# RobinBruneau/RNb-NeuS2

Measured on AMD Instinct MI355X. Metric: training rays/s + ms/step, normals-only SDF 64x800^2, higher is better.
Workload: dtype f16 storage / f32 accumulate

## Files before the change

rnb-neus2_amd/csrc/common.cuh:

```cuda
#pragma once
#include <hip/hip_runtime.h>
#include <stdint.h>
#include "../../include/rnb_neus2.h"

namespace rnb {

typedef _Float16 half_t;
typedef _Float16 h2 __attribute__((ext_vector_type(2)));
typedef _Float16 h4 __attribute__((ext_vector_type(4)));
typedef _Float16 h8 __attribute__((ext_vector_type(8)));
typedef float f4 __attribute__((ext_vector_type(4)));

constexpr uint32_t GRIDSIZE = RNB_GRIDSIZE;
constexpr uint32_t GRID_CELLS = GRIDSIZE * GRIDSIZE * GRIDSIZE;
constexpr uint32_t N_CASCADES = RNB_CASCADES;
constexpr float LOSS_SCALE = 128.f;
constexpr uint32_t N_MAX_RANDOM_SAMPLES_PER_RAY = 8;
constexpr float SQRT3 = 1.73205080757f;
constexpr float STEPSIZE = SQRT3 / 1024;
constexpr float MIN_CONE_STEPSIZE = STEPSIZE;
constexpr float MAX_CONE_STEPSIZE = STEPSIZE * (1 << (N_CASCADES - 1)) * 1024 / GRIDSIZE;
constexpr float MIN_OPTICAL_THICKNESS = 0.1f;

struct GridMeta {
// ... 220 lines not shown
}

template <bool PAIR = false>
__device__ __forceinline__ void level_issue(const LevelMeta* __restrict__ lm, const uint32_t* __restrict__ grid, const uint32_t level, const float x, const float y, const float z, uint32_t (&v)[8]) {
	const uint4 raw = reinterpret_cast<const uint4*>(lm + level)[0], raw2 = reinterpret_cast<const uint4*>(lm + level)[1];
	const uint32_t off = __builtin_amdgcn_readfirstlane(raw.x), hashmap_size = __builtin_amdgcn_readfirstlane(raw.y);
	const float scale = __uint_as_float(__builtin_amdgcn_readfirstlane(raw.w));
	const uint32_t my = __builtin_amdgcn_readfirstlane(raw2.x), mz = __builtin_amdgcn_readfirstlane(raw2.y);
	const bool dense = __builtin_amdgcn_readfirstlane(raw2.z) != 0u, pow2 = __builtin_amdgcn_readfirstlane(raw2.w) != 0u;
	const uint32_t* __restrict__ g = grid + off;
	float pos[3];
	uint32_t pg[3];
	pos_fract(x, scale, &pos[0], &pg[0]);
	pos_fract(y, scale, &pos[1], &pg[1]);
	pos_fract(z, scale, &pos[2], &pg[2]);
	const uint32_t ty0 = pg[1] * my, ty1 = ty0 + my, tz0 = pg[2] * mz, tz1 = tz0 + mz;
#pragma unroll
	for (uint32_t yz = 0; yz < 4; ++yz) {
		const uint32_t ty = (yz & 1u) ? ty1 : ty0, tz = (yz >> 1) ? tz1 : tz0;
		const uint32_t d0 = pg[0] + ty + tz, h = ty ^ tz;
		uint32_t e0 = (PAIR || dense) ? d0 : (pg[0] ^ h), e1 = (PAIR || dense) ? d0 + 1u : ((pg[0] + 1u) ^ h);
		const uint32_t w0 = e0 >= hashmap_size ? e0 - hashmap_size : e0, w1 = e1 >= hashmap_size ? e1 - hashmap_size : e1;
		e0 = pow2 ? (e0 & (hashmap_size - 1u)) : w0;
		e1 = pow2 ? (e1 & (hashmap_size - 1u)) : w1;
		if (PAIR) {
			const U2 p = *reinterpret_cast<const U2*>(g + e0);
			v[yz * 2 + 0] = p.x;
			v[yz * 2 + 1] = e1 == e0 + 1u ? p.y : g[0];
		} else {
			v[yz * 2 + 0] = g[e0];
			v[yz * 2 + 1] = g[e1];
		}
	}
}
template <bool GRAD>
__device__ __forceinline__ void level_consume(const LevelMeta* __restrict__ lm, const uint32_t level, const float x, const float y, const float z, const uint32_t (&v)[8],
                                              half_t& f0, half_t& f1, float dy0[3], float dy1[3]) {
	const float scale = __uint_as_float(__builtin_amdgcn_readfirstlane(reinterpret_cast<const uint32_t*>(lm + level)[3]));
	float pos[3];
	uint32_t pg[3];
	pos_fract(x, scale, &pos[0], &pg[0]);
	pos_fract(y, scale, &pos[1], &pg[1]);
	pos_fract(z, scale, &pos[2], &pg[2]);
	half_t r0 = (half_t)0.f, r1 = (half_t)0.f;
#pragma unroll
	for (uint32_t idx = 0; idx < 8; ++idx) {
		float weight = 1;
#pragma unroll
		for (uint32_t d = 0; d < 3; ++d) {
			if ((idx & (1u << d)) == 0) weight *= 1 - pos[d];
			else weight *= pos[d];
		}
		const h2 val = unpack_h2(v[idx]);
		r0 = r0 + f2h(weight * h2f(val[0]));
		r1 = r1 + f2h(weight * h2f(val[1]));
	}
	f0 = r0;
	f1 = r1;
	if (GRAD) {
#pragma unroll
		for (uint32_t gd = 0; gd < 3; ++gd) {
			float a0 = 0.f, a1 = 0.f;
#pragma unroll
			for (uint32_t idx = 0; idx < 4; ++idx) {
				float weight = scale;
				uint32_t corner = 0;
#pragma unroll
				for (uint32_t ngd = 0; ngd < 2; ++ngd) {
					const uint32_t d = ngd >= gd ? (ngd + 1) : ngd;
					if ((idx & (1u << ngd)) == 0) weight *= 1 - pos[d];
					else { weight *= pos[d]; corner |= (1u << d); }
				}
				const h2 vl = unpack_h2(v[corner]);
				const h2 vr = unpack_h2(v[corner | (1u << gd)]);
				a0 += weight * (h2f(vr[0]) - h2f(vl[0])) * 1.0f;
				a1 += weight * (h2f(vr[1]) - h2f(vl[1])) * 1.0f;
			}
			dy0[gd] = a0;
			dy1[gd] = a1;
		}
	}
}

struct Vec3 { float x, y, z; };
__device__ __forceinline__ Vec3 v3(float x, float y, float z) { return {x, y, z}; }
__device__ __forceinline__ Vec3 operator+(Vec3 a, Vec3 b) { return {a.x + b.x, a.y + b.y, a.z + b.z}; }
__device__ __forceinline__ Vec3 operator-(Vec3 a, Vec3 b) { return {a.x - b.x, a.y - b.y, a.z - b.z}; }
__device__ __forceinline__ Vec3 operator*(float s, Vec3 a) { return {s * a.x, s * a.y, s * a.z}; }
__device__ __forceinline__ float esum3(float x0, float x1, float x2) { return x0 + (x1 + x2); }
__device__ __forceinline__ float esum4(float x0, float x1, float x2, float x3) { return (x0 + x1) + (x2 + x3); }
__device__ __forceinline__ float dot(Vec3 a, Vec3 b) { return esum3(a.x * b.x, a.y * b.y, a.z * b.z); }
__device__ __forceinline__ Vec3 normalized(Vec3 a) { float n = sqrtf(dot(a, a)); return {a.x / n, a.y / n, a.z / n}; }

__device__ __forceinline__ int mip_from_pos(const Vec3& pos, uint32_t max_cascade = N_CASCADES - 1) {
	int exponent;
	float maxval = fmaxf(fmaxf(fabsf(pos.x - 0.5f), fabsf(pos.y - 0.5f)), fabsf(pos.z - 0.5f));
	frexpf(maxval, &exponent);
	return min((int)max_cascade, max(0, exponent + 1));
}
__device__ __forceinline__ int mip_from_dt(float dt, const Vec3& pos, uint32_t max_cascade = N_CASCADES - 1) {
	int mip = mip_from_pos(pos, max_cascade);
	dt *= 2 * GRIDSIZE;
	if (dt < 1.f) return mip;
	int exponent;
	frexpf(dt, &exponent);
	return min((int)max_cascade, max(exponent, mip));
}
__device__ __forceinline__ uint32_t cascaded_grid_idx_at(Vec3 pos, uint32_t mip) {
	float mip_scale = scalbnf(1.0f, -(int)mip);
	pos = pos - v3(0.5f, 0.5f, 0.5f);
	pos = mip_scale * pos;
	pos = pos + v3(0.5f, 0.5f, 0.5f);
	int ix = (int)(pos.x * GRIDSIZE), iy = (int)(pos.y * GRIDSIZE), iz = (int)(pos.z * GRIDSIZE);
	return morton3D((uint32_t)min(max(ix, 0), (int)GRIDSIZE - 1), (uint32_t)min(max(iy, 0), (int)GRIDSIZE - 1), (uint32_t)min(max(iz, 0), (int)GRIDSIZE - 1));
}
__device__ __forceinline__ bool density_grid_occupied_at(const Vec3& pos, const uint8_t* __restrict__ bitfield, uint32_t mip) {
	uint32_t idx = cascaded_grid_idx_at(pos, mip);
	return bitfield[idx / 8 + (GRID_CELLS * mip) / 8] & (1 << (idx % 8));
}
__device__ __forceinline__ float calc_dt(float t, float cone_angle) {
	return fminf(fmaxf(t * cone_angle, MIN_CONE_STEPSIZE), MAX_CONE_STEPSIZE);
}
__device__ __forceinline__ float warp_dt(float dt) {
	float max_stepsize = MIN_CONE_STEPSIZE * (1 << (N_CASCADES - 1));
	return (dt - MIN_CONE_STEPSIZE) / (max_stepsize - MIN_CONE_STEPSIZE);
}
__device__ __forceinline__ float unwarp_dt(float dt) {
	float max_stepsize = MIN_CONE_STEPSIZE * (1 << (N_CASCADES - 1));
	return dt * (max_stepsize - MIN_CONE_STEPSIZE) + MIN_CONE_STEPSIZE;
}
__device__ __forceinline__ float sign1(float x) { return copysignf(1.0f, x); }
__device__ __forceinline__ float distance_to_next_voxel(const Vec3& pos, const Vec3& dir, const Vec3& idir, uint32_t res) {
	Vec3 p = (float)res * pos;
	float tx = (floorf(p.x + 0.5f + 0.5f * sign1(dir.x)) - p.x) * idir.x;
	float ty = (floorf(p.y + 0.5f + 0.5f * sign1(dir.y)) - p.y) * idir.y;
	float tz = (floorf(p.z + 0.5f + 0.5f * sign1(dir.z)) - p.z) * idir.z;
	float t = fminf(fminf(tx, ty), tz);
	return fmaxf(t / res, 0.0f);
}
__device__ __forceinline__ float advance_to_next_voxel(float t, float cone_angle, const Vec3& pos, const Vec3& dir, const Vec3& idir, uint32_t res) {
	float t_target = t + distance_to_next_voxel(pos, dir, idir, res);
	do { t += calc_dt(t, cone_angle); } while (t < t_target);
	return t;
}

__device__ __forceinline__ float logistic(float x) { return 1.0f / (1.0f + expf(-x)); }
__device__ __forceinline__ float relu(float v) { return v > 0.0f ? v : 0.0f; }
__device__ __forceinline__ Vec3 warp_direction(const Vec3& d) { return {(d.x + 1.0f) * 0.5f, (d.y + 1.0f) * 0.5f, (d.z + 1.0f) * 0.5f}; }
__device__ __forceinline__ Vec3 unwarp_direction(const Vec3& d) { return {d.x * 2.0f - 1.0f, d.y * 2.0f - 1.0f, d.z * 2.0f - 1.0f}; }
__device__ __forceinline__ float loss_and_gradient(const bool l2, const float (&target)[4], const float (&prediction)[4], float (&grad)[4]) {
	float diff[4];
#pragma unroll
	for (int k = 0; k < 4; ++k) diff[k] = prediction[k] - target[k];
	if (l2) {
#pragma unroll
		for (int k = 0; k < 4; ++k) grad[k] = 2 * diff[k];
		return diff[0] * diff[0] + diff[1] * diff[1] + diff[2] * diff[2] + diff[3] * diff[3];
	}
#pragma unroll
	for (int k = 0; k < 4; ++k) grad[k] = copysignf(1.0f, diff[k]);
	return fabsf(diff[0]) + fabsf(diff[1]) + fabsf(diff[2]) + fabsf(diff[3]);
}

}
```

rnb-neus2_amd/csrc/kernels_net.cuh:

```cuda
#pragma once
#include "mlp.cuh"

namespace rnb {

constexpr int WG = 256;
constexpr int WAVES_PER_WG = 4;


__device__ __forceinline__ void write_sdf_in_row(half_t* __restrict__ tile, const int lane, const float x, const float y, const float z, const half_t (&feat)[28]) {
	half_t row[32];
	row[0] = f2h(x) - (half_t)0.5f;
	row[1] = f2h(y) - (half_t)0.5f;
	row[2] = f2h(z) - (half_t)0.5f;
#pragma unroll
	for (int k = 0; k < 28; ++k) row[3 + k] = feat[k];
	row[31] = (half_t)0.f;
#pragma unroll
	for (int q = 0; q < 4; ++q) {
		h8 v;
#pragma unroll
		for (int j = 0; j < 8; ++j) v[j] = row[q * 8 + j];
		*reinterpret_cast<h8*>(tile + lane * S32 + q * 8) = v;
	}
}

template <bool GRAD>
__device__ __forceinline__ void encode_all_lm(const LevelMeta* __restrict__ lm, const uint32_t n_levels, const uint32_t valid_level, const uint32_t* __restrict__ grid,
                                              const float x, const float y, const float z, half_t (&feat)[28], float (&dydx)[GRAD ? 28 : 1][3]) {
#pragma unroll
	for (uint32_t level = 0; level < 14; ++level) {
		half_t f0 = (half_t)0.f, f1 = (half_t)0.f;
		float d0[3] = {0.f, 0.f, 0.f}, d1[3] = {0.f, 0.f, 0.f};
		if (level < n_levels && level <= valid_level) {
			encode_level_lm<GRAD>(lm, grid, level, x, y, z, f0, f1, d0, d1);
		}
		feat[level * 2 + 0] = f0;
		feat[level * 2 + 1] = f1;
		if (GRAD) {
#pragma unroll
			for (int d = 0; d < 3; ++d) { dydx[GRAD ? level * 2 + 0 : 0][d] = d0[d]; dydx[GRAD ? level * 2 + 1 : 0][d] = d1[d]; }
		}
	}
}

template <bool GRAD, int DEPTH, int ND = 0>
__device__ __forceinline__ void encode_all_pipelined(const LevelMeta* __restrict__ lm, const uint32_t n_levels, const uint32_t valid_level, const uint32_t* __restrict__ grid,
                                                     const float x, const float y, const float z, half_t (&feat)[28], float (&dydx)[GRAD ? 28 : 1][3]) {
	const uint32_t n_live = min(n_levels, valid_level + 1u);
	uint32_t v[DEPTH][8];
	const uint32_t last = n_live ? n_live - 1u : 0u;
#pragma unroll
	for (uint32_t l = 0; l < (uint32_t)DEPTH; ++l) { if (l < (uint32_t)ND) level_issue<true>(lm, grid, min(l, last), x, y, z, v[l]); else level_issue<false>(lm, grid, min(l, last), x, y, z, v[l]); }
#pragma unroll
	for (uint32_t level = 0; level < 14; ++level) {
		half_t f0, f1;
		float d0[3], d1[3];
		const bool live = level < n_live;
		level_consume<GRAD>(lm, min(level, last), x, y, z, v[level % DEPTH], f0, f1, d0, d1);
		if (level + DEPTH < 14) { if (level + DEPTH < (uint32_t)ND) level_issue<true>(lm, grid, min(level + (uint32_t)DEPTH, last), x, y, z, v[level % DEPTH]); else level_issue<false>(lm, grid, min(level + (uint32_t)DEPTH, last), x, y, z, v[level % DEPTH]); }
		feat[level * 2 + 0] = live ? f0 : (half_t)0.f;
		feat[level * 2 + 1] = live ? f1 : (half_t)0.f;
		if (GRAD) {
#pragma unroll
			for (int d = 0; d < 3; ++d) { dydx[GRAD ? level * 2 + 0 : 0][d] = live ? d0[d] : 0.f; dydx[GRAD ? level * 2 + 1 : 0][d] = live ? d1[d] : 0.f; }
		}
	}
}

__device__ __forceinline__ half_t sdf_to_density(half_t sdf, half_t variance) {
	const half_t s = f2h(expf(h2f(variance * (half_t)10.0f)));
	const half_t sig = f2h(1.0f / (1.0f + expf(-h2f(sdf * s))));
	return (s * sig) * ((half_t)1.0f - sig);
}

struct PointArgs {
	const float* xyz;
	uint32_t n;
	half_t* out;
	const uint32_t* splat_idx;
	float* grid_tmp;
	int want_density;
	float sdf_bias;
	const uint32_t* range;
	uint32_t xcd;
};

struct FwdArgs {
	const float* coords;
	const uint32_t* n_ptr;
	uint32_t n_max;
	half_t* out;
	float sdf_bias;
	const uint32_t* idx;
	const half_t* wimg;
	half_t* cin_out;
};

__device__ __forceinline__ void copy_weight_image(half_t* __restrict__ dst, const half_t* __restrict__ src, const int n_halfs, const int tid, const int nthreads) {
	for (int i = tid * 8; i < n_halfs; i += nthreads * 8) *reinterpret_cast<h8*>(dst + i) = *reinterpret_cast<const h8*>(src + i);
}

constexpr int PQ2_WAVE_HALFS = TILE * S32 + TILE;
constexpr size_t LDS_POINT2 = (size_t)(W_S0T + WAVES_PER_WG * PQ2_WAVE_HALFS) * sizeof(half_t);
__device__ __forceinline__ void poison_lds(char* smem_raw, const size_t bytes, const int tid, const int nthreads) {
#ifdef RNB_POISON_LDS
	uint32_t* w = reinterpret_cast<uint32_t*>(smem_raw);
	for (uint32_t q = (uint32_t)tid; q < (uint32_t)(bytes / 4); q += (uint32_t)nthreads) w[q] = 0x7e007e00u;
	__syncthreads();
#else
	(void)smem_raw; (void)bytes; (void)tid; (void)nthreads;
#endif
}

template <bool EMU, int PIPE_DEPTH = 0, int ND = 0>
__device__ __forceinline__ void point_query_chained_body(const GridMeta& G, const NetW& net, const PointArgs& a, const half_t* __restrict__ wimg, char* smem_raw, LevelMeta* lm) {
	poison_lds(smem_raw, LDS_POINT2, threadIdx.x, WG);
	half_t* wts = reinterpret_cast<half_t*>(smem_raw);
	fill_level_meta(lm, G, threadIdx.x);
	const uint32_t n_levels = G.n_levels, valid_level = G.valid_level;
	if (wimg) copy_weight_image(wts, wimg, W_S0T, threadIdx.x, WG);
	else {
		for (int i = threadIdx.x; i < 64 * 32; i += WG) { int o = i >> 5, k = i & 31; wts[W_S0 + o * S32 + k] = net.sdf_w0[i]; }
		for (int i = threadIdx.x; i < 16 * 64; i += WG) { int o = i >> 6, q = i & 63; wts[W_S1 + o * S64 + q] = net.sdf_w1[o * 64 + chain_logical(q)]; }
	}
	__syncthreads();
	const int lane = threadIdx.x & 63, wave = threadIdx.x >> 6;
	half_t* X = wts + W_S0T + wave * PQ2_WAVE_HALFS;
	half_t* Z = X + TILE * S32;
	const half_t variance = net.variance[0];
	const half_t bias = f2h(a.sdf_bias);
	uint32_t s_first = 0, s_end = a.n;
	if (a.range) { s_first = a.range[0]; s_end = min(a.range[1], a.n); }
	const uint32_t n_tiles = (s_end - s_first + TILE - 1) / TILE;
	const int r16 = lane & 15, hq = lane >> 4;
	const bool by_xcd = a.xcd != 0u && (gridDim.x & 7u) == 0u;
	const uint32_t t8 = by_xcd ? (n_tiles + 7u) / 8u : n_tiles, t_base = by_xcd ? (blockIdx.x & 7u) * t8 : 0u, t_stop = min(n_tiles, t_base + t8);
	const uint32_t t_stride = (by_xcd ? gridDim.x / 8u : gridDim.x) * WAVES_PER_WG;
	for (uint32_t tile = t_base + (by_xcd ? blockIdx.x / 8u : blockIdx.x) * WAVES_PER_WG + wave; tile < t_stop; tile += t_stride) {
		const uint32_t s = s_first + tile * TILE + lane;
		const bool valid = s < s_end;
		float x = 0.5f, y = 0.5f, z = 0.5f;
		if (valid) { x = a.xyz[(size_t)s * 3 + 0]; y = a.xyz[(size_t)s * 3 + 1]; z = a.xyz[(size_t)s * 3 + 2]; }
		uint32_t cell = 0;
		if (valid && a.splat_idx) cell = a.splat_idx[s];
		half_t feat[28];
		float dummy[1][3];
		if (PIPE_DEPTH) encode_all_pipelined<false, PIPE_DEPTH ? PIPE_DEPTH : 1, ND>(lm, n_levels, valid_level, net.grid, x, y, z, feat, dummy);
		else encode_all_lm<false>(lm, n_levels, valid_level, net.grid, x, y, z, feat, dummy);
		write_sdf_in_row(X, lane, x, y, z, feat);
		wave_lds_sync();
		h8 bz[4][2];
		{
			f4 acc[4][4];
			zero_acc<4>(acc);
			mfma_layer<4, 1, EMU ? EMU_NATURAL : EMU_OFF>(wts + W_S0, S32, X, S32, acc, lane);
			chain_pack<true>(acc, bz);
		}
		f4 acc_so[1][4];
		zero_acc<1>(acc_so);
		mfma_layer_regs<1, 2, EMU ? EMU_CHAINED : EMU_OFF>(wts + W_S1, S64, bz, acc_so, lane);
		if (hq == 0) {
#pragma unroll
			for (int nt = 0; nt < 4; ++nt) Z[16 * nt + r16] = f2h(acc_so[0][nt][0]);
		}
		wave_lds_sync();
		half_t v = Z[lane] + bias;
		if (a.want_density) v = sdf_to_density(v, variance);
		if (valid) {
			if (a.out) a.out[s] = v;
			if (a.splat_idx) atomicMax(reinterpret_cast<uint32_t*>(a.grid_tmp) + cell, __float_as_uint(h2f(v)));
		}
		wave_lds_sync();
	}
}
__global__ __launch_bounds__(WG, 4) void k_point_query_chained(const GridMeta G, const NetW net, const PointArgs a, const half_t* __restrict__ wimg) {
	extern __shared__ __attribute__((aligned(16))) char smem_raw[];
	__shared__ LevelMeta lm[RNB_MAX_LEVELS];
	point_query_chained_body<false>(G, net, a, wimg, smem_raw, lm);
}
template <int DEPTH, int ND = 0>
__global__ __launch_bounds__(WG, 3) void k_point_query_chained_pipe(const GridMeta G, const NetW net, const PointArgs a, const half_t* __restrict__ wimg) {
	extern __shared__ __attribute__((aligned(16))) char smem_raw[];
	__shared__ LevelMeta lm[RNB_MAX_LEVELS];
	point_query_chained_body<false, DEPTH, ND>(G, net, a, wimg, smem_raw, lm);
}
__global__ __launch_bounds__(WG, 2) void k_point_query_chained_emul(const GridMeta G, const NetW net, const PointArgs a, const half_t* __restrict__ wimg) {
	extern __shared__ __attribute__((aligned(16))) char smem_raw[];
	__shared__ LevelMeta lm[RNB_MAX_LEVELS];
	point_query_chained_body<true>(G, net, a, wimg, smem_raw, lm);
}
template <int DEPTH, int ND = 0>
__global__ __launch_bounds__(WG, 2) void k_point_query_chained_emul_pipe(const GridMeta G, const NetW net, const PointArgs a, const half_t* __restrict__ wimg) {
	extern __shared__ __attribute__((aligned(16))) char smem_raw[];
	__shared__ LevelMeta lm[RNB_MAX_LEVELS];
	point_query_chained_body<true, DEPTH, ND>(G, net, a, wimg, smem_raw, lm);
}

constexpr int FWD2_WAVE_HALFS = TILE * S32 + TILE * 8 + TILE;
constexpr size_t LDS_FWD2 = (size_t)(W_FWD_END + WAVES_PER_WG * FWD2_WAVE_HALFS) * sizeof(half_t);

template <bool EMU, int PIPE_DEPTH = 0, int ND = 0>
__device__ __forceinline__ void forward_chained_body(const GridMeta& G, const NetW& net, const FwdArgs& a, char* smem_raw, LevelMeta* lm) {
	poison_lds(smem_raw, LDS_FWD2, threadIdx.x, WG);
	half_t* wts = reinterpret_cast<half_t*>(smem_raw);
	fill_level_meta(lm, G, threadIdx.x);
	const uint32_t n_levels = G.n_levels, valid_level = G.valid_level;
	if (a.wimg) copy_weight_image(wts, a.wimg, W_FWD_END, threadIdx.x, WG);
	else load_weights_chained(wts, net, threadIdx.x, WG);
	__syncthreads();
	const int lane = threadIdx.x & 63, wave = threadIdx.x >> 6;
	half_t* X = wts + W_FWD_END + wave * FWD2_WAVE_HALFS;
	half_t* Y = X + TILE * S32;
	half_t* Z = Y + TILE * 8;
	const half_t variance = net.variance[0];
	const half_t bias = f2h(a.sdf_bias);
	uint32_t n = a.n_max;
	if (a.n_ptr) n = min(*a.n_ptr, a.n_max);
	const uint32_t n_tiles = (n + TILE - 1) / TILE;
	const int r16 = lane & 15, hq = lane >> 4;
	for (uint32_t tile = blockIdx.x * WAVES_PER_WG + wave; tile < n_tiles; tile += gridDim.x * WAVES_PER_WG) {
		const uint32_t q_in = tile * TILE + lane;
		const bool valid = q_in < n;
		uint32_t s = q_in;
		if (a.idx && valid) s = a.idx[q_in];
		float c[7] = {0.5f, 0.5f, 0.5f, 0.f, 0.f, 0.f, 0.f};
		if (valid) {
#pragma unroll
			for (int q = 0; q < 7; ++q) c[q] = a.coords[(size_t)s * 7 + q];
		}
		half_t feat[28];
		float dydx[28][3];
		if (PIPE_DEPTH) encode_all_pipelined<true, PIPE_DEPTH ? PIPE_DEPTH : 1, ND>(lm, n_levels, valid_level, net.grid, c[0], c[1], c[2], feat, dydx);
		else encode_all_lm<true>(lm, n_levels, valid_level, net.grid, c[0], c[1], c[2], feat, dydx);
		write_sdf_in_row(X, lane, c[0], c[1], c[2], feat);
		wave_lds_sync();
		h8 bz[4][2];
		{
			f4 acc[4][4];
			zero_acc<4>(acc);
			mfma_layer<4, 1, EMU ? EMU_NATURAL : EMU_OFF>(wts + W_S0, S32, X, S32, acc, lane);
			chain_pack<true>(acc, bz);
		}
		f4 acc_so[1][4];
		zero_acc<1>(acc_so);
		mfma_layer_regs<1, 2, EMU ? EMU_CHAINED : EMU_OFF>(wts + W_S1, S64, bz, acc_so, lane);
		{
#pragma unroll
			for (int ks = 0; ks < 2; ++ks) {
				const h8 w1 = *reinterpret_cast<const h8*>(wts + W_S1 + 0 * S64 + 32 * ks + 8 * hq);
#pragma unroll
				for (int nt = 0; nt < 4; ++nt)
#pragma unroll
					for (int j = 0; j < 8; ++j) bz[nt][ks][j] = (bz[nt][ks][j] > (half_t)0.f) ? w1[j] : (half_t)0.f;
			}
		}
		wave_lds_sync();
		{
			f4 acc[2][4];
			zero_acc<2>(acc);
			mfma_layer_regs<2, 2, EMU ? EMU_CHAINED : EMU_OFF>(wts + W_S0T, S64, bz, acc, lane);
			store_acc<2, false>(acc, X, S32, 0, lane);
		}
		wave_lds_sync();
		float grad[3] = {0.f, 0.f, 0.f};
		{
			half_t din[32];
#pragma unroll
			for (int q = 0; q < 4; ++q) {
				const h8 v = *reinterpret_cast<const h8*>(X + lane * S32 + q * 8);
#pragma unroll
				for (int j = 0; j < 8; ++j) din[q * 8 + j] = v[j];
			}
#pragma unroll
			for (int k = 0; k < 28; ++k) {
				const float dl = h2f(din[3 + k]);
#pragma unroll
				for (int d = 0; d < 3; ++d) grad[d] += dl * dydx[k][d];
			}
#pragma unroll
			for (int d = 0; d < 3; ++d) grad[d] += h2f(din[d]);
		}
		{
			const h8 v = {f2h(c[0]), f2h(c[1]), f2h(c[2]), f2h(grad[0]), f2h(grad[1]), f2h(grad[2]), (half_t)0.f, (half_t)0.f};
			*reinterpret_cast<h8*>(Y + lane * 8) = v;
			if (hq == 0) {
#pragma unroll
				for (int nt = 0; nt < 4; ++nt) Z[16 * nt + r16] = f2h(acc_so[0][nt][0]);
			}
		}
		wave_lds_sync();
		const half_t sdf0 = Z[lane];
		if (a.cin_out) {
			if (valid) {
				h8* row = reinterpret_cast<h8*>(a.cin_out + (size_t)s * 32);
				row[2] = *reinterpret_cast<const h8*>(Y + lane * 8);
				row[3] = h8{(half_t)0.f, (half_t)0.f, (half_t)0.f, (half_t)0.f, (half_t)0.f, (half_t)0.f, (half_t)0.f, (half_t)0.f};
			}
#pragma unroll
			for (int nt = 0; nt < 4; ++nt) {
				const uint32_t s_nt = (uint32_t)__shfl((int)s, 16 * nt + r16, 64);
				const bool v_nt = __shfl((int)valid, 16 * nt + r16, 64) != 0;
				const h4 o = {f2h(acc_so[0][nt][0]), f2h(acc_so[0][nt][1]), f2h(acc_so[0][nt][2]), f2h(acc_so[0][nt][3])};
				if (v_nt) *reinterpret_cast<h4*>(a.cin_out + (size_t)s_nt * 32 + 4 * hq) = o;
			}
		}
		h8 bh[4][2];
		{
			h8 bin[4][1];
#pragma unroll
			for (int nt = 0; nt < 4; ++nt) {
				h4 o = {(half_t)0.f, (half_t)0.f, (half_t)0.f, (half_t)0.f};
				if (hq < 2) o = *reinterpret_cast<const h4*>(Y + (16 * nt + r16) * 8 + 4 * hq);
#pragma unroll
				for (int j = 0; j < 4; ++j) { bin[nt][0][j] = f2h(acc_so[0][nt][j]); bin[nt][0][4 + j] = o[j]; }
			}
			f4 acc[4][4];
			zero_acc<4>(acc);
			mfma_layer_regs<4, 1, EMU ? EMU_CHAINED : EMU_OFF>(wts + W_C0, S32, bin, acc, lane);
			chain_pack<true>(acc, bh);
		}
		{
			f4 acc[4][4];
			zero_acc<4>(acc);
			mfma_layer_regs<4, 2, EMU ? EMU_CHAINED : EMU_OFF>(wts + W_C1, S64, bh, acc, lane);
			chain_pack<true>(acc, bh);
		}
		{
			f4 acc[1][4];
			zero_acc<1>(acc);
			mfma_layer_regs<1, 2, EMU ? EMU_CHAINED : EMU_OFF>(wts + W_C2, S64, bh, acc, lane);
			store_acc<1, false>(acc, X, S32, 0, lane);
		}
		wave_lds_sync();
		{
			h8 o0 = *reinterpret_cast<const h8*>(X + lane * S32 + 0);
			h8 o1 = *reinterpret_cast<const h8*>(X + lane * S32 + 8);
			o0[3] = sdf0 + bias;
			o0[4] = f2h(grad[0]); o0[5] = f2h(grad[1]); o0[6] = f2h(grad[2]);
			o0[7] = variance;
			o1[0] = f2h(c[4]); o1[1] = f2h(c[5]); o1[2] = f2h(c[6]);
			if (valid) {
				h8* dst = reinterpret_cast<h8*>(a.out + (size_t)s * 16);
				dst[0] = o0;
				dst[1] = o1;
			}
		}
		wave_lds_sync();
	}
}
__global__ __launch_bounds__(WG, 2) void k_forward_chained(const GridMeta G, const NetW net, const FwdArgs a) {
	extern __shared__ __attribute__((aligned(16))) char smem_raw[];
	__shared__ LevelMeta lm[RNB_MAX_LEVELS];
	forward_chained_body<false>(G, net, a, smem_raw, lm);
}
template <int DEPTH, int ND = 0>
__global__ __launch_bounds__(WG, 2) void k_forward_chained_pipe(const GridMeta G, const NetW net, const FwdArgs a) {
	extern __shared__ __attribute__((aligned(16))) char smem_raw[];
	__shared__ LevelMeta lm[RNB_MAX_LEVELS];
	forward_chained_body<false, DEPTH, ND>(G, net, a, smem_raw, lm);
}
__global__ __launch_bounds__(WG, 2) void k_forward_chained_emul(const GridMeta G, const NetW net, const FwdArgs a) {
	extern __shared__ __attribute__((aligned(16))) char smem_raw[];
	__shared__ LevelMeta lm[RNB_MAX_LEVELS];
	forward_chained_body<true>(G, net, a, smem_raw, lm);
}
template <int DEPTH, int ND = 0>
__global__ __launch_bounds__(WG, 2) void k_forward_chained_emul_pipe(const GridMeta G, const NetW net, const FwdArgs a) {
	extern __shared__ __attribute__((aligned(16))) char smem_raw[];
	__shared__ LevelMeta lm[RNB_MAX_LEVELS];
	forward_chained_body<true, DEPTH, ND>(G, net, a, smem_raw, lm);
}


struct TrainScratch {
	half_t *h2, *h1, *cin, *z1, *sdfin, *dz1;
	half_t *dr, *dh2, *dh1, *dso, *dz, *ddin, *front;
	uint32_t* g12;
	float* srec;
	float* var_partial;
};

struct TrainArgs {
	const float* coords;
	const half_t* dout;
	uint32_t B;
	uint32_t B_global;
	float sdf_bias;
	uint32_t skip_rgb;
	const half_t* wimg;
	float *dw_w0, *dw_w0b, *dw_w1, *dw_w1b;
	const half_t* dcin;
	TrainScratch t;
};

__device__ __forceinline__ void fm_store(const half_t* __restrict__ tile, const int stride, const int width, half_t* __restrict__ dst, const uint32_t B, const uint32_t s) {
	const half_t* row = tile + (s & 63) * stride;
	for (int f = 0; f < width; f += 8) {
		const h8 v = *reinterpret_cast<const h8*>(row + f);
#pragma unroll
		for (int j = 0; j < 8; ++j) dst[(size_t)(f + j) * B + s] = v[j];
	}
}

__global__ __launch_bounds__(WG, 1) void k_fwd_bwd(const GridMeta G, const NetW net, const TrainArgs a) {
	extern __shared__ __attribute__((aligned(16))) char smem_raw[];
	half_t* wts = reinterpret_cast<half_t*>(smem_raw);
	__shared__ LevelMeta lm[RNB_MAX_LEVELS];
	fill_level_meta(lm, G, threadIdx.x);
	const uint32_t n_levels = G.n_levels, valid_level = G.valid_level;
	if (a.wimg) copy_weight_image(wts, a.wimg, W_TRAIN_END, threadIdx.x, WG);
	else load_weights<true>(wts, net, threadIdx.x, WG);
	__syncthreads();
	const int lane = threadIdx.x & 63, wave = threadIdx.x >> 6;
	half_t* tA = wts + W_TRAIN_END + wave * 3 * ACT_TILE_HALFS;
	half_t* tB = tA + ACT_TILE_HALFS;
	half_t* tC = tB + ACT_TILE_HALFS;
	const int r16 = lane & 15, hq = lane >> 4;
	const uint32_t B = a.B;
	const uint32_t n_tiles = B / TILE;
	const TrainScratch& T = a.t;
	float var_sum = 0.f;
	for (uint32_t tile = blockIdx.x * WAVES_PER_WG + wave; tile < n_tiles; tile += gridDim.x * WAVES_PER_WG) {
		const uint32_t s = tile * TILE + lane;
		float c[7];
#pragma unroll
		for (int q = 0; q < 7; ++q) c[q] = a.coords[(size_t)s * 7 + q];
		half_t dout[16];
		{
			const h8* src = reinterpret_cast<const h8*>(a.dout + (size_t)s * 16);
			const h8 d0 = src[0], d1 = src[1];
#pragma unroll
			for (int j = 0; j < 8; ++j) { dout[j] = d0[j]; dout[8 + j] = d1[j]; }
		}
		half_t feat[28];
		float dydx[28][3];
		encode_all_lm<true>(lm, n_levels, valid_level, net.grid, c[0], c[1], c[2], feat, dydx);
		write_sdf_in_row(tA, lane, c[0], c[1], c[2], feat);
		wave_lds_sync();
		fm_store(tA, S32, 32, T.sdfin, B, s);
		uint64_t m_z1;
		{
			f4 acc[4][4];
			zero_acc<4>(acc);
			mfma_layer<4, 1>(wts + W_S0, S32, tA, S32, acc, lane);
			m_z1 = store_acc<4, true>(acc, tB, S64, 0, lane);
		}
		wave_lds_sync();
		fm_store(tB, S64, 64, T.z1, B, s);
		{
			f4 acc[1][4];
			zero_acc<1>(acc);
			mfma_layer<1, 2>(wts + W_S1, S64, tB, S64, acc, lane);
			store_acc<1, false>(acc, tC, S32, 0, lane);
		}
		wave_lds_sync();
#pragma unroll
		for (int mt = 0; mt < 4; ++mt) {
			const h4 w1 = *reinterpret_cast<const h4*>(wts + W_S1 + 0 * S64 + 16 * mt + 4 * hq);
#pragma unroll
			for (int nt = 0; nt < 4; ++nt) {
				h4 v;
#pragma unroll
				for (int r = 0; r < 4; ++r) v[r] = ((m_z1 >> ((mt * 4 + nt) * 4 + r)) & 1ull) ? w1[r] : (half_t)0.f;
				*reinterpret_cast<h4*>(tA + (16 * nt + r16) * S64 + 16 * mt + 4 * hq) = v;
			}
		}
		wave_lds_sync();
		fm_store(tA, S64, 64, T.dz1, B, s);
		{
			f4 acc[2][4];
			zero_acc<2>(acc);
			mfma_layer<2, 2>(wts + W_S0T, S64, tA, S64, acc, lane);
			store_acc<2, false>(acc, tB, S32, 0, lane);
		}
// ... 153 lines not shown
			}
			dd[31] = (half_t)0.f;
#pragma unroll
			for (int q = 0; q < 4; ++q) {
				h8 v;
#pragma unroll
				for (int j = 0; j < 8; ++j) v[j] = dd[q * 8 + j];
				*reinterpret_cast<h8*>(tC + lane * S32 + q * 8) = v;
			}
		}
		wave_lds_sync();
		fm_store(tC, S32, 32, T.ddin, B, s);
		{
			f4 acc[4][4];
			zero_acc<4>(acc);
			mfma_layer<4, 1>(wts + W_S0, S32, tC, S32, acc, lane);
			wave_lds_sync();
			store_acc_masked<4>(acc, m_z1, tB, S64, 0, lane);
		}
		wave_lds_sync();
		fm_store(tB, S64, 64, T.front, B, s);
		wave_lds_sync();
		(void)m_h2;
	}
#pragma unroll
	for (int off = 32; off > 0; off >>= 1) var_sum += __shfl_down(var_sum, off, 64);
	if (lane == 0) T.var_partial[blockIdx.x * WAVES_PER_WG + wave] = var_sum;
}

constexpr int SW_S0 = 0;
constexpr int SW_S0T = SW_S0 + 64 * S32;
constexpr int SW_W1 = SW_S0T + 32 * S64;
constexpr int SW_W1N = SW_W1 + 64;
constexpr int SW_END = SW_W1N + 64;
constexpr int SW_END_PADDED = (SW_END + 7) / 8 * 8;
constexpr int FBS_WAVE_HALFS = 2 * TILE * S32 + TILE;
constexpr size_t LDS_FBS = (size_t)(SW_END + WAVES_PER_WG * FBS_WAVE_HALFS) * sizeof(half_t);
constexpr int SW_W1T = SW_END_PADDED;
constexpr int SWF_END = SW_W1T + 64 * S32;
constexpr int SO_STRIDE = 24;
constexpr int FBS_FULL_WAVE_HALFS = FBS_WAVE_HALFS + TILE * SO_STRIDE;
constexpr size_t LDS_FBS_FULL = (size_t)(SWF_END + WAVES_PER_WG * FBS_FULL_WAVE_HALFS) * sizeof(half_t);
__host__ __device__ constexpr int fbs_logical(int p) { return p < 28 ? 3 + p : (p < 31 ? p - 28 : 31); }
__host__ __device__ constexpr int fbs_logical_h(int p) { return p < 13 ? 3 + p : (p < 16 ? p - 13 : p); }
__host__ __device__ constexpr int fbs_feature_slot_h(int q) { return q < 13 ? q : q + 3; }

__device__ inline void load_weights_fbs(half_t* __restrict__ w, const NetW& net, const int tid, const int nthreads, const bool half_order = false) {
	for (int i = tid; i < 64 * 32; i += nthreads) { const int o = i >> 5, p = i & 31; w[SW_S0 + o * S32 + p] = net.sdf_w0[o * 32 + (half_order ? fbs_logical_h(p) : fbs_logical(p))]; }
	for (int i = tid; i < 32 * 64; i += nthreads) { const int q = i >> 6, p = i & 63; w[SW_S0T + q * S64 + p] = net.sdf_w0[chain_logical(p) * 32 + fbs_logical(q)]; }
	for (int i = tid; i < 64; i += nthreads) { w[SW_W1 + i] = net.sdf_w1[chain_logical(i)]; w[SW_W1N + i] = net.sdf_w1[i]; }
	for (int i = SW_END + tid; i < SW_END_PADDED; i += nthreads) w[i] = (half_t)0.f;
}
__device__ inline void load_weights_fbs_full(half_t* __restrict__ w, const NetW& net, const int tid, const int nthreads, const bool half_order = false) {
	load_weights_fbs(w, net, tid, nthreads, half_order);
	for (int i = tid; i < 64 * 32; i += nthreads) { const int u = i >> 5, o = i & 31; w[SW_W1T + u * S32 + o] = o < 16 ? net.sdf_w1[o * 64 + u] : (half_t)0.f; }
}

__device__ inline void load_weights_rgb(half_t* __restrict__ w, const NetW& net, const int tid, const int nthreads);
constexpr uint32_t WIMG_WGS = 16;
__global__ __launch_bounds__(WG) void k_prepare_weight_images(const NetW net, half_t* __restrict__ img_fwd, half_t* __restrict__ img_fbs, half_t* __restrict__ img_train, half_t* __restrict__ img_rgb, const int half_order) {
	const int tid = blockIdx.x * WG + threadIdx.x, nthreads = gridDim.x * WG;
	if (blockIdx.y == 0) load_weights_chained(img_fwd, net, tid, nthreads);
	else if (blockIdx.y == 1) load_weights_fbs_full(img_fbs, net, tid, nthreads, half_order != 0);
	else if (blockIdx.y == 2) load_weights<true>(img_train, net, tid, nthreads);
	else load_weights_rgb(img_rgb, net, tid, nthreads);
}

template <typename T>
__device__ __forceinline__ void st32(T* __restrict__ base, const uint32_t idx, const T v) { *reinterpret_cast<T*>(reinterpret_cast<char*>(base) + idx * (uint32_t)sizeof(T)) = v; }

__device__ __forceinline__ void export_frags(const h8 (&b)[4][2], half_t* __restrict__ dst, const uint32_t B, const uint32_t tile, const int lane) {
	const uint32_t r16 = lane & 15, hq = lane >> 4;
	const uint32_t lane_off = 4u * hq * B + tile * TILE + r16 * 4u;
#pragma unroll
	for (uint32_t ks = 0; ks < 2; ++ks)
#pragma unroll
		for (uint32_t j = 0; j < 8; ++j) {
			const uint32_t row_off = (16u * (2u * ks + (j >> 2)) + (j & 3u)) * B;
			const h4 v = {b[0][ks][j], b[1][ks][j], b[2][ks][j], b[3][ks][j]};
			*reinterpret_cast<h4*>(reinterpret_cast<char*>(dst) + (row_off + lane_off) * 2u) = v;
		}
}

template <bool FULL, bool EMU = false, bool SLICED = false>
__device__ __forceinline__ void fwd_bwd_sdf_body(const GridMeta& G, const NetW& net, const TrainArgs& a, char* smem_raw, LevelMeta* lm) {
	poison_lds(smem_raw, FULL ? LDS_FBS_FULL : LDS_FBS, threadIdx.x, WG);
	half_t* wts = reinterpret_cast<half_t*>(smem_raw);
	constexpr int W_END = FULL ? SWF_END : SW_END;
	fill_level_meta(lm, G, threadIdx.x);
	const uint32_t n_live = min(G.n_levels, G.valid_level + 1u);
	if (a.wimg) copy_weight_image(wts, a.wimg, W_END, threadIdx.x, WG);
	else if (FULL) load_weights_fbs_full(wts, net, threadIdx.x, WG, EMU);
	else load_weights_fbs(wts, net, threadIdx.x, WG, EMU);
	__syncthreads();
	const int lane = threadIdx.x & 63, wave = threadIdx.x >> 6;
	constexpr int WAVE_HALFS = FULL ? FBS_FULL_WAVE_HALFS : FBS_WAVE_HALFS;
	half_t* X = wts + W_END + wave * WAVE_HALFS;
	half_t* D = X + TILE * S32;
	half_t* Z = D + TILE * S32;
	half_t* SO = Z + TILE;
	const int r16 = lane & 15, hq = lane >> 4;
	const uint32_t B = a.B;
	const uint32_t n_tiles = B / TILE;
	const TrainScratch& T = a.t;
	float var_sum = 0.f;
	f4 acc_w0[4][2], acc_w0b[4][2];
	float acc_w1[4] = {0.f, 0.f, 0.f, 0.f}, acc_w1b[4] = {0.f, 0.f, 0.f, 0.f};
	f4 acc_w1f[FULL ? 4 : 1];
#pragma unroll
	for (int nt = 0; nt < (FULL ? 4 : 1); ++nt) acc_w1f[nt] = f4{0.f, 0.f, 0.f, 0.f};
#pragma unroll
	for (int mo = 0; mo < 4; ++mo)
#pragma unroll
		for (int ni = 0; ni < 2; ++ni) { acc_w0[mo][ni] = f4{0.f, 0.f, 0.f, 0.f}; acc_w0b[mo][ni] = f4{0.f, 0.f, 0.f, 0.f}; }
	for (uint32_t tile = blockIdx.x * WAVES_PER_WG + wave; tile < n_tiles; tile += gridDim.x * WAVES_PER_WG) {
		const uint32_t s = tile * TILE + lane;
		float c[3];
#pragma unroll
		for (int q = 0; q < 3; ++q) c[q] = a.coords[(size_t)s * 7 + q];
		half_t dout[16];
		{
			const h8* src = reinterpret_cast<const h8*>(a.dout + (size_t)s * 16);
			const h8 d0 = src[0], d1 = src[1];
#pragma unroll
			for (int j = 0; j < 8; ++j) { dout[j] = d0[j]; dout[8 + j] = d1[j]; }
		}
		float dn[3];
		{
			h8 a2 = {(half_t)0.f, (half_t)0.f, (half_t)0.f, (half_t)0.f, (half_t)0.f, (half_t)0.f, (half_t)0.f, (half_t)0.f};
			if (FULL) {
				const h8* row = reinterpret_cast<const h8*>(a.dcin + (size_t)s * 32);
				a2 = row[2];
				h8 o0 = row[0];
				o0[0] = o0[0] + dout[3];
				*reinterpret_cast<h8*>(SO + lane * SO_STRIDE) = o0;
				*reinterpret_cast<h8*>(SO + lane * SO_STRIDE + 8) = row[1];
			}
#pragma unroll
			for (int d = 0; d < 3; ++d) {
				float v = FULL ? h2f(a2[3 + d]) : 0.f;
				v += h2f(dout[4 + d]) / (float)a.B_global;
				v += h2f(dout[8 + d]);
				dn[d] = v;
			}
		}
		reinterpret_cast<f4*>(T.srec)[(size_t)s * 2 + 0] = f4{c[0], c[1], c[2], dn[0]};
		reinterpret_cast<f4*>(T.srec)[(size_t)s * 2 + 1] = f4{dn[1], dn[2], 0.f, 0.f};
		uint32_t* Xrow = reinterpret_cast<uint32_t*>(X + lane * S32);
		uint32_t* Drow = reinterpret_cast<uint32_t*>(D + lane * S32);
#pragma unroll 1
		for (uint32_t level = 0; level < 14; ++level) {
			half_t f0 = (half_t)0.f, f1 = (half_t)0.f;
			float d0[3] = {0.f, 0.f, 0.f}, d1[3] = {0.f, 0.f, 0.f};
			if (level < n_live) encode_level_lm<true>(lm, net.grid, level, c[0], c[1], c[2], f0, f1, d0, d1);
			float r0 = 0.f, r1 = 0.f;
#pragma unroll
			for (int d = 0; d < 3; ++d) { r0 += d0[d] * dn[d]; r1 += d1[d] * dn[d]; }
			const half_t e0 = f2h(r0), e1 = f2h(r1);
			if (EMU) {
				const uint32_t q0 = 2u * level, q1 = q0 + 1u, p0 = q0 < 13u ? q0 : q0 + 3u, p1 = q1 < 13u ? q1 : q1 + 3u;
				X[lane * S32 + p0] = f0; X[lane * S32 + p1] = f1;
				D[lane * S32 + p0] = e0; D[lane * S32 + p1] = e1;
			} else {
				Xrow[level] = pack_h2(f0, f1);
				Drow[level] = pack_h2(e0, e1);
			}
		}
		{
			const half_t px = f2h(c[0]) - (half_t)0.5f, py = f2h(c[1]) - (half_t)0.5f, pz = f2h(c[2]) - (half_t)0.5f;
			const half_t n0 = f2h(dn[0]), n1 = f2h(dn[1]), n2 = f2h(dn[2]);
			if (EMU) {
				half_t* xr = X + lane * S32; half_t* dr = D + lane * S32;
				xr[13] = px; xr[14] = py; xr[15] = pz; xr[31] = (half_t)0.f;
				dr[13] = n0; dr[14] = n1; dr[15] = n2; dr[31] = (half_t)0.f;
			} else {
				Xrow[14] = pack_h2(px, py); Xrow[15] = pack_h2(pz, (half_t)0.f);
				Drow[14] = pack_h2(n0, n1); Drow[15] = pack_h2(n2, (half_t)0.f);
			}
		}
		Z[lane] = dout[3];
		var_sum += h2f(dout[7]);
		wave_lds_sync();
		auto load_fso = [&](const int nt) {
			h8 v = {(half_t)0.f, (half_t)0.f, (half_t)0.f, (half_t)0.f, (half_t)0.f, (half_t)0.f, (half_t)0.f, (half_t)0.f};
			if (hq < 2) v = *reinterpret_cast<const h8*>(SO + (16 * nt + r16) * SO_STRIDE + 8 * hq);
			return v;
		};
		if (SLICED) {
			static_assert(!SLICED || EMU, "the sliced weight gradients belong to the half mode");
			if (!FULL) st32(T.dso, s, dout[3]);
		}
		{
			h8 fso[4];
			if (FULL) {
#pragma unroll
				for (int nt = 0; nt < 4; ++nt) fso[nt] = load_fso(nt);
			}
			h8 ain[4], add[4];
			h4 d3v[4];
#pragma unroll
			for (int mt = 0; mt < 4; ++mt) {
				ain[mt] = *reinterpret_cast<const h8*>(X + (16 * mt + r16) * S32 + 8 * hq);
				add[mt] = *reinterpret_cast<const h8*>(D + (16 * mt + r16) * S32 + 8 * hq);
				d3v[mt] = *reinterpret_cast<const h4*>(Z + 16 * mt + 4 * hq);
			}
			const f4 zero4 = {0.f, 0.f, 0.f, 0.f};
			h8 a_so[2];
			if (FULL) {
				h8 idf;
#pragma unroll
				for (int j = 0; j < 8; ++j) idf[j] = (8 * hq + j == r16) ? (half_t)1.f : (half_t)0.f;
#pragma unroll
				for (int ks = 0; ks < 2; ++ks)
#pragma unroll
					for (int h = 0; h < 2; ++h) {
						const f4 t = __builtin_amdgcn_mfma_f32_16x16x32_f16(fso[2 * ks + h], idf, zero4, 0, 0, 0);
#pragma unroll
						for (int r = 0; r < 4; ++r) a_so[ks][4 * h + r] = f2h(t[r]);
					}
				if (SLICED) {
#pragma unroll
					for (int ks = 0; ks < 2; ++ks)
#pragma unroll
						for (int h = 0; h < 2; ++h) {
							const uint32_t off = (uint32_t)r16 * B + tile * TILE + 16u * (2 * ks + h) + 4u * hq;
							st32(reinterpret_cast<h4*>(T.dso), off / 4u, h4{a_so[ks][4 * h], a_so[ks][4 * h + 1], a_so[ks][4 * h + 2], a_so[ks][4 * h + 3]});
						}
				}
			}
			h8 b_in[2][2], b_dd[2][2];
#pragma unroll
			for (int n2 = 0; n2 < 2; ++n2) {
				h8 idf;
#pragma unroll
				for (int j = 0; j < 8; ++j) idf[j] = (8 * hq + j == 16 * n2 + r16) ? (half_t)1.f : (half_t)0.f;
#pragma unroll
				for (int ks = 0; ks < 2; ++ks)
#pragma unroll
					for (int h = 0; h < 2; ++h) {
						const f4 ti = __builtin_amdgcn_mfma_f32_16x16x32_f16(ain[2 * ks + h], idf, zero4, 0, 0, 0);
						const f4 td = __builtin_amdgcn_mfma_f32_16x16x32_f16(add[2 * ks + h], idf, zero4, 0, 0, 0);
#pragma unroll
						for (int r = 0; r < 4; ++r) { b_in[n2][ks][4 * h + r] = f2h(ti[r]); b_dd[n2][ks][4 * h + r] = f2h(td[r]); }
					}
			}
			if (SLICED) {
#pragma unroll
				for (int n2 = 0; n2 < 2; ++n2) {
// ... 113 lines not shown
			}
		}
#pragma unroll
		for (int ks = 0; ks < 2; ++ks) {
			const h8 w1 = *reinterpret_cast<const h8*>(wts + SW_W1 + 32 * ks + 8 * hq);
#pragma unroll
			for (int nt = 0; nt < 4; ++nt)
#pragma unroll
				for (int j = 0; j < 8; ++j) {
					const bool on = bz[nt][ks][j] > (half_t)0.f;
					bz[nt][ks][j] = on ? w1[j] : (half_t)0.f;
					bdz[nt][ks][j] = on ? (FULL ? bdz[nt][ks][j] : f2h(h2f(w1[j]) * h2f(d3[nt]))) : (half_t)0.f;
				}
		}
		wave_lds_sync();
		{
			f4 acc[2][4];
			zero_acc<2>(acc);
			mfma_layer_regs<2, 2, EMU ? EMU_CHAINED : EMU_OFF>(wts + SW_S0T, S64, bz, acc, lane);
			store_acc<2, false>(acc, X, S32, 0, lane);
		}
		wave_lds_sync();
#pragma unroll
		for (uint32_t l = 0; l < 14; ++l) st32(T.g12, (l * B + s) * 2u + 1u, Xrow[l]);
		wave_lds_sync();
		{
			f4 acc[2][4];
			zero_acc<2>(acc);
			mfma_layer_regs<2, 2, EMU ? EMU_CHAINED : EMU_OFF>(wts + SW_S0T, S64, bdz, acc, lane);
			store_acc<2, false>(acc, X, S32, 0, lane);
		}
		wave_lds_sync();
#pragma unroll
		for (uint32_t l = 0; l < 14; ++l) st32(T.g12, (l * B + s) * 2u + 0u, Xrow[l]);
		wave_lds_sync();
	}
#pragma unroll
	for (int off = 32; off > 0; off >>= 1) var_sum += __shfl_down(var_sum, off, 64);
	if (lane == 0) T.var_partial[blockIdx.x * WAVES_PER_WG + wave] = var_sum;
	if (SLICED) return;
	float* red = reinterpret_cast<float*>(wts + W_END);
	static_assert((size_t)WAVES_PER_WG * FBS_WAVE_HALFS * sizeof(half_t) >= (size_t)WAVES_PER_WG * 64 * 32 * sizeof(float), "staging area of the weight-gradient partials");
	constexpr int N = 64 * 32;
	for (int pass = 0; pass < 2; ++pass) {
		__syncthreads();
#pragma unroll
		for (int mo = 0; mo < 4; ++mo)
#pragma unroll
			for (int ni = 0; ni < 2; ++ni)
#pragma unroll
				for (int r = 0; r < 4; ++r) red[wave * N + (16 * mo + 4 * hq + r) * 32 + (EMU ? fbs_logical_h(16 * ni + r16) : fbs_logical(16 * ni + r16))] = pass ? acc_w0b[mo][ni][r] : acc_w0[mo][ni][r];
		__syncthreads();
		float* dst = (pass ? a.dw_w0b : a.dw_w0) + (size_t)blockIdx.x * N;
		for (int q = threadIdx.x; q < N; q += WG) dst[q] = ((red[q] + red[N + q]) + red[2 * N + q]) + red[3 * N + q];
	}
	if (FULL) {
		__syncthreads();
#pragma unroll
		for (int nt = 0; nt < 4; ++nt)
#pragma unroll
			for (int r = 0; r < 4; ++r) red[wave * (16 * 64) + (4 * hq + r) * 64 + 16 * nt + r16] = acc_w1f[nt][r];
		__syncthreads();
		float* dst = a.dw_w1 + (size_t)blockIdx.x * (16 * 64);
		for (int q = threadIdx.x; q < 16 * 64; q += WG) dst[q] = ((red[q] + red[16 * 64 + q]) + red[2 * 16 * 64 + q]) + red[3 * 16 * 64 + q];
	}
	for (int pass = FULL ? 1 : 0; pass < 2; ++pass) {
		__syncthreads();
#pragma unroll
		for (int nt = 0; nt < 4; ++nt) red[(wave * 4 + hq) * 64 + 16 * nt + r16] = pass ? acc_w1b[nt] : acc_w1[nt];
		__syncthreads();
		float* dst = (pass ? a.dw_w1b : a.dw_w1) + (size_t)blockIdx.x * (16 * 64);
		for (int q = threadIdx.x; q < 16 * 64; q += WG) {
			float v = 0.f;
			if (q < 64) for (int g = 0; g < 16; ++g) v += red[g * 64 + q];
			dst[q] = v;
		}
	}
}

__global__ __launch_bounds__(WG, 2) void k_fwd_bwd_sdf(const GridMeta G, const NetW net, const TrainArgs a) {
	extern __shared__ __attribute__((aligned(16))) char smem_raw[];
	__shared__ LevelMeta lm[RNB_MAX_LEVELS];
	fwd_bwd_sdf_body<false>(G, net, a, smem_raw, lm);
}
__global__ __launch_bounds__(WG, 2) void k_fwd_bwd_sdf_full(const GridMeta G, const NetW net, const TrainArgs a) {
	extern __shared__ __attribute__((aligned(16))) char smem_raw[];
	__shared__ LevelMeta lm[RNB_MAX_LEVELS];
	fwd_bwd_sdf_body<true>(G, net, a, smem_raw, lm);
}
__global__ __launch_bounds__(WG, 2) void k_fwd_bwd_sdf_h(const GridMeta G, const NetW net, const TrainArgs a) {
	extern __shared__ __attribute__((aligned(16))) char smem_raw[];
	__shared__ LevelMeta lm[RNB_MAX_LEVELS];
	fwd_bwd_sdf_body<false, true>(G, net, a, smem_raw, lm);
}
__global__ __launch_bounds__(WG, 2) void k_fwd_bwd_sdf_hs(const GridMeta G, const NetW net, const TrainArgs a) {
	extern __shared__ __attribute__((aligned(16))) char smem_raw[];
	__shared__ LevelMeta lm[RNB_MAX_LEVELS];
	fwd_bwd_sdf_body<false, true, true>(G, net, a, smem_raw, lm);
}
__global__ __launch_bounds__(WG, 2) void k_fwd_bwd_sdf_full_hs(const GridMeta G, const NetW net, const TrainArgs a) {
	extern __shared__ __attribute__((aligned(16))) char smem_raw[];
	__shared__ LevelMeta lm[RNB_MAX_LEVELS];
	fwd_bwd_sdf_body<true, true, true>(G, net, a, smem_raw, lm);
}
__global__ __launch_bounds__(WG, 2) void k_fwd_bwd_sdf_full_h(const GridMeta G, const NetW net, const TrainArgs a) {
	extern __shared__ __attribute__((aligned(16))) char smem_raw[];
	__shared__ LevelMeta lm[RNB_MAX_LEVELS];
	fwd_bwd_sdf_body<true, true>(G, net, a, smem_raw, lm);
}

constexpr int RW_C0 = 0;
constexpr int RW_C1 = RW_C0 + 64 * S32;
constexpr int RW_C1T = RW_C1 + 64 * S64;
constexpr int RW_C0T = RW_C1T + 64 * S64;
constexpr int RW_C2T = RW_C0T + 32 * S64;
constexpr int RW_END = RW_C2T + 64 * S32;
static_assert(RW_END % 8 == 0, "16-byte copies of the image");
constexpr size_t LDS_RGB = std::max((size_t)RW_END * sizeof(half_t), (size_t)WAVES_PER_WG * 64 * 64 * sizeof(float));

__device__ inline void load_weights_rgb(half_t* __restrict__ w, const NetW& net, const int tid, const int nthreads) {
	auto col = [](int c) { return c < 16 ? c : c + 16; };
	for (int i = tid; i < 64 * 32; i += nthreads) {
		const int o = i >> 5, c = i & 31;
		w[RW_C0 + o * S32 + c] = net.rgb_w0[o * 48 + col(c)];
		w[RW_C2T + o * S32 + c] = c < 16 ? net.rgb_w2[c * 64 + o] : (half_t)0.f;
	}
	for (int i = tid; i < 64 * 64; i += nthreads) {
		const int o = i >> 6, p = i & 63;
		w[RW_C1 + o * S64 + p] = net.rgb_w1[o * 64 + chain_logical(p)];
		w[RW_C1T + o * S64 + p] = net.rgb_w1[chain_logical(p) * 64 + o];
	}
	for (int i = tid; i < 32 * 64; i += nthreads) { const int c = i >> 6, p = i & 63; w[RW_C0T + c * S64 + p] = net.rgb_w0[chain_logical(p) * 48 + col(c)]; }
}

struct RgbArgs {
	const half_t* cin;
	const uint32_t* src_slot;
	const half_t* dout;
	half_t* dcin;
	uint32_t B;
	const half_t* wimg;
	float *dw_c0, *dw_c1, *dw_c2;
	TrainScratch t;
};

template <int KS>
__device__ __forceinline__ void transpose_frags(const h8 (&in)[4][KS], h8 (&out)[2 * KS][2], const int r16, const int hq) {
	const f4 zero4 = {0.f, 0.f, 0.f, 0.f};
#pragma unroll
	for (int n2 = 0; n2 < 2; ++n2) {
		h8 idf;
#pragma unroll
		for (int j = 0; j < 8; ++j) idf[j] = (8 * hq + j == 16 * n2 + r16) ? (half_t)1.f : (half_t)0.f;
#pragma unroll
		for (int ks = 0; ks < KS; ++ks)
#pragma unroll
			for (int ms = 0; ms < 4; ++ms) {
				const f4 t = __builtin_amdgcn_mfma_f32_16x16x32_f16(in[ms][ks], idf, zero4, 0, 0, 0);
#pragma unroll
				for (int r = 0; r < 4; r += 2) {
					out[2 * ks + n2][ms >> 1][4 * (ms & 1) + r] = f2h(t[r]);
					out[2 * ks + n2][ms >> 1][4 * (ms & 1) + r + 1] = f2h(t[r + 1]);
				}
			}
	}
}
// ... 1200 lines not shown
```

rnb-neus2_amd/csrc/rnb_neus2_hip.hip:

```cpp
#include "kernels_net.cuh"
#include "kernels_ray.cuh"
#include "kernels_mesh.cuh"
#include "kernels_render.cuh"
#include "kernels_mesh_sparse.cuh"
#include "kernels_mesh_clean.cuh"
#include "kernels_mesh_simplify.cuh"
#include "../host/mesh.hpp"

#include <hip/hip_ext.h>

#include <algorithm>
#include <atomic>
#include <chrono>
#include <cmath>
#include <cstdio>
#include <cstdlib>
#include <cstring>
#include <functional>
#include <limits>
#include <new>
#include <stdexcept>
#include <random>
#include <string>
#include <vector>
// ... 69 lines not shown
			float ms = 0.f;
			if (hipEventElapsedTime(&ms, ev[i - 1], ev[i]) == hipSuccess) {
				total_ms[ids[i]] += ms; ++launches[ids[i]];
				if (ids[i] == P_SCATTER_LDS || ids[i] == P_SCATTER_RL || ids[i] == P_SCATTER_QUAD) { total_ms[P_SCATTER] += ms; if (ids[i] == P_SCATTER_QUAD) ++launches[P_SCATTER]; }
			}
		}
		n = 0;
	}
	void reset() { for (int i = 0; i < P_COUNT; ++i) { total_ms[i] = 0; launches[i] = 0; units[i] = 0; } n = 0; }
	void destroy() { for (auto e : ev) (void)hipEventDestroy(e); ev.clear(); ids.clear(); n = 0; }
};

static inline uint32_t ilog2(uint32_t v) { uint32_t r = 0; while (v > 1) { v >>= 1; ++r; } return r; }

struct rnb_ctx {
	rnb_config cfg;
	Profiler prof;
	GridMeta grid;
	uint64_t n_grid_params = 0, n_params = 0;
	uint32_t n_dense_lead = 0;
	uint64_t off_sdf = 0, off_rgb = 0, off_grid = 0, off_var = 0;
	SceneAabb aabb;
	int n_cus = 256;

	DevBuf<float> params_fp32, grads, adam_m, adam_v;
	DevBuf<half_t> params_fp16, params_ema;
	DevBuf<half_t> grads16;
	bool half_acc() const { return cfg.accumulate == RNB_ACCUM_HALF; }
	DevBuf<unsigned long long> grads_fixed;
	bool fixed_acc() const { return cfg.deterministic != 0; }
	size_t grad_elem() const { return half_acc() ? sizeof(half_t) : sizeof(float); }
	char* grad_ptr(uint64_t i) const { return half_acc() ? reinterpret_cast<char*>(grads16.p + i) : reinterpret_cast<char*>(grads.p + i); }
	DevBuf<uint32_t> adam_steps;
	DevBuf<float> opt_rec;
	bool opt_plain_current = true, opt_rec_current = false;
	DevBuf<float> adam_lr_table;
	float lr_table_beta1 = -1.f, lr_table_beta2 = -1.f;
	DevBuf<float> density_grid, density_grid_tmp, density_grid_tmp_alt, density_mean;
	bool tmp_alt_clear = false;
	rnb_grid_exchange_fn grid_exchange = nullptr;
	void* grid_exchange_user = nullptr;
	bool bitfield_foreign = false;
	DevBuf<double> mean_partial, loss_sums;
	DevBuf<uint8_t> bitfield;
	DevBuf<unsigned long long> march_stats;
	DevBuf<uint32_t> coarse_bits, coarse_count;
	bool coarse_valid = false;
	uint32_t* host_coarse = nullptr;
	uint32_t* host_coarse_dev = nullptr;
	DevBuf<float> grid_sample_pos;
	DevBuf<uint32_t> grid_sample_idx;
	uint32_t n_grid_samples = 0;
	struct { bool valid = false; uint32_t ema_step = 0, n_uniform = 0, n_nonuniform = 0; uint64_t rng_state = 0, rng_inc = 0; } gs_pre;
	bool last_update_sorted = false;
	struct { bool pending = false; uint32_t n_uniform = 0, n_nonuniform = 0; } gs_todo;
	DevBuf<float> gs_sorted_pos, gs_stage_pos, gs_eval_pos;
	DevBuf<uint32_t> gs_sorted_idx, gs_stage_idx, gs_eval_idx, gs_hist, gs_range;
	hipEvent_t ev_grid = nullptr, ev_gs = nullptr;

	uint32_t n_views = 0;
	DevBuf<ViewDev> views;
	DevBuf<uint16_t> pixels;
	float light_dirs[9];

	DevBuf<uint32_t> ray_indices, numsteps, counters;
	DevBuf<float> rays, coords, coords_compacted, loss;
	float *ek_loss = nullptr, *mask_loss = nullptr;
	DevBuf<half_t> mlp_out, dloss_dout;
	DevBuf<double> wg_partial;
	bool loss_reduced = false;
	DevBuf<float> ray_grad; DevBuf<uint32_t> ray_of, slot_of;
	DevBuf<float> chain_rec;
	DevBuf<float> ray_setup, ray_dunnorm, ray_t;
	DevBuf<double> loss_partial;
	DevBuf<uint32_t> ray_steps, ray_base, ray_slot, ncomp, cbase, scan_tiles;
	DevBuf<uint32_t> ray_base1, idx1, idx2, fwd_counts;
	DevBuf<unsigned long long> scan_words;
	uint32_t scan_ticket = 0;
	DevBuf<half_t> wimg_fwd, wimg_fbs, wimg_train, wimg_rgb;
	DevBuf<half_t> cin_eval, dcin, rgb_out_scratch;
	DevBuf<uint32_t> src_slot;
	bool cin_flow = false;
	bool rgb_split() const { return !cfg.apply_no_albedo && !knobs.fwd_bwd_generic; }
	bool wimg_valid = false;
	DevBuf<float> ray_const;
	DevBuf<uint32_t> unfinished;
	uint32_t fwd_k1 = 48;
	bool fwd_k1_fixed = false;
	bool gen_split = false;
	uint32_t gen_k1 = 0, cur_k1 = 0;
	struct Knobs {
		bool march_narrow = false, fwd_bwd_generic = false, loss_wave_per_ray = false;
		int scatter_wg_per_cu = -1;
		uint32_t fbs_wg_per_cu = 2;
		bool march_running_sums = false;
		bool march_late = false;
		uint32_t march_narrow_from = 18432;
		bool dp_order = false;
		bool scan_chain = true;
		uint32_t march_wave_per_ray_below = 4096;
		int scatter_order = -1;
		bool scatter_c_side = false;
		bool unsafe_skip_joins = false;
		bool join_fold = false;
		bool defer_tail = true;
		bool poll_loss = true;
		bool fused_update = true;
		bool loss_scan_fused_always = false;
		bool loss_scan_fused = true;
		bool loss_flat = true;
		bool loss_chain_records = true;
		int ray_const_dense = 2;
		int march_write_split = -1;
		bool scatter_plain = false;
		int dbg_scatter_lo = -1, dbg_scatter_hi = -1;
		bool scatter_c_early = false;
		int scatter_rl_staged = -1;
		bool march_skip_narrow = false;
		uint32_t march_narrow_wgs = 128;
		int march_wgs = 1024;
		int march_skip = 1;
		bool dw_late = false;
		int march_bbox = 1;
		int march_prio = 0;
		int scatter_prio = 0;
		bool scatter_share = true;
		int scatter_kmin = 0, scatter_rl_upto = 0;
		bool scatter_anyorder = true;
		int encode_depth = 4;
		int march_write_wg = 256;
		bool chain_plain = true;
		bool point_xcd = true;
		bool dw_sliced = true;
		bool encode_pair = false;
		bool grid_presort = true;
	} knobs;
	DevBuf<RayLoss> ray_loss;
	DevBuf<McTable> mc_table;
	uint32_t render_cap = 0;
	DevBuf<RenderRay> render_rays[2];
	DevBuf<uint32_t> render_keep, render_scan, render_counts;
	DevBuf<float> render_res, render_coords;
	DevBuf<half_t> render_out;
	DevBuf<half_t> fm;
	DevBuf<uint32_t> g12;
	DevBuf<float> srec, var_partial, dw_partial;
	TrainScratch ts;
	uint32_t dw_nwg = 0, dw_chunk = 0;
	uint32_t fwd_grid = 0;
	bool grads_clean = true;

	Pcg32 rng, density_grid_rng, trainer_rng;
	uint32_t density_grid_ema_step = 0;
	uint32_t training_step = 0, valid_level = 0, rays_per_batch = 0;
	uint32_t measured_batch_size = 0, measured_batch_size_before_compaction = 0, n_rays_total = 0;
	uint32_t optimizer_step_count = 0;
	float lr_factor = 1.f;
	uint32_t cur_n_rays = 0, cur_n_rays_total = 0, local_measured_before = 0, cur_step = 0;
	bool grid_updated = false;
	float prep_ms = 0.f;
	std::chrono::steady_clock::time_point step_start;

	hipStream_t s_march = nullptr, s_dw = nullptr, s_adam = nullptr;
	bool tail_pending = false;
	bool join_pending = false;
	hipEvent_t ev_join = nullptr;
	hipEvent_t ev_loss = nullptr, ev_march = nullptr, ev_fb = nullptr, ev_dw = nullptr, ev_adam = nullptr, ev_tail = nullptr, ev_march_rest = nullptr, ev_all = nullptr, ev_sc[4] = {nullptr, nullptr, nullptr, nullptr};
	struct { bool valid = false, exchanged = false, dp = false, sharded = false, all_final_recorded = false, dw_joined = true, c_early = false; uint64_t split[2] = {0, 0}, split_mid = 0; int order = 0;
	         bool c_side = false; hipEvent_t c_after = nullptr; std::function<void(hipStream_t, hipEvent_t)> c_launch; } sc;
	struct ScatterGroups { uint32_t e_c = 0, l_fine = 0, Ks[RNB_MAX_LEVELS] = {}; uint64_t k_log2 = 0; } sg;
	hipStream_t backward_stream = nullptr;
	hipStream_t step_stream = nullptr;
	uint64_t dp_split = 0, dp_mid = 0;
	uint64_t param_capacity = 0;
	bool dp_order() const { return cfg.world_size > 1 || knobs.dp_order; }
	struct { bool begun = false, early_done = false; AdamArgs args; } opt;
	struct { bool valid = false, loss_cleared = false; uint32_t n_rays = 0, n_rays_total = 0, max_inference = 0, k1 = 0; bool split = false, march_joined = false; } pre;
	struct Readback { double sums[3]; uint32_t counters[4]; uint32_t fwd[2]; uint32_t seq, pad; }* host_rb = nullptr;
	uint32_t rb_seq = 0;
	bool loss_polled = true;
	bool poll_loss() const { return overlap() && !dp_order() && knobs.poll_loss; }
	void* host_rb_dev = nullptr;
	bool overlap() const { return cfg.overlap != 0 && !prof.on && s_march != nullptr; }

	NetW net(bool inference) const {
		const half_t* p = inference ? params_ema.p : params_fp16.p;
		NetW n;
		n.sdf_w0 = p + off_sdf;
		n.sdf_w1 = n.sdf_w0 + 64 * 32;
		n.rgb_w0 = p + off_rgb;
		n.rgb_w1 = n.rgb_w0 + 64 * 48;
		n.rgb_w2 = n.rgb_w1 + 64 * 64;
		n.grid = reinterpret_cast<const uint32_t*>(p + off_grid);
		n.variance = p + off_var;
		return n;
	}
	GridMeta meta() const { GridMeta g = grid; g.valid_level = valid_level; return g; }
};

static void discard_premarch(rnb_ctx* c);
static bool prep_due(uint32_t step) {
	const uint32_t n_prep_to_skip = std::min(std::max(step / 16u, 1u), 16u);
	return step % n_prep_to_skip == 0;
}
static void flush_c_side(rnb_ctx* c, hipStream_t s) {
	if (!c->sc.c_side) return;
	c->sc.c_side = false;
	c->sc.c_launch(s, nullptr);
}
static void join_tail_host(rnb_ctx* c) {
	if (c->join_pending) { (void)hipEventSynchronize(c->ev_join); c->join_pending = false; }
	if (c->tail_pending) { (void)hipEventSynchronize(c->ev_tail); c->tail_pending = false; }
}

static int check_scan_errors(rnb_ctx* c) {
	const bool rays = c->host_coarse[5] != 0, compact = c->host_coarse[6] != 0;
	if (!rays && !compact) return RNB_OK;
// ... 191 lines not shown
	HIP_TRY(hipGetLastError());
	HIP_TRY(hipEventRecord(c->ev_gs, s));
	c->gs_pre.valid = true; c->gs_pre.ema_step = c->density_grid_ema_step; c->gs_pre.n_uniform = n_uniform; c->gs_pre.n_nonuniform = n_nonuniform;
	return RNB_OK;
}

int update_density_grid_front(rnb_ctx* c, hipStream_t s, uint32_t n_uniform, uint32_t n_nonuniform, bool shard) {
	const uint32_t n_elements = GRID_CELLS * (c->aabb.max_cascade + 1);
	const uint32_t n_samples = n_uniform + n_nonuniform;
	c->prof.mark(s, P_NONE);
	if (c->training_step == 0) {
		c->density_grid_ema_step = 0;
		HIP_TRY(hipMemsetAsync(c->density_grid.p, 0, sizeof(float) * n_elements, s));
		c->gs_pre.valid = false;
	}
	const bool sorted = c->gs_pre.valid && c->gs_pre.ema_step == c->density_grid_ema_step && c->gs_pre.n_uniform == n_uniform && c->gs_pre.n_nonuniform == n_nonuniform &&
	                    c->gs_pre.rng_state == c->density_grid_rng.state && c->gs_pre.rng_inc == c->density_grid_rng.inc;
	c->gs_pre.valid = false;
	c->last_update_sorted = sorted;
	if (sorted && c->tmp_alt_clear) std::swap(c->density_grid_tmp, c->density_grid_tmp_alt);
	else HIP_TRY(hipMemsetAsync(c->density_grid_tmp.p, 0, sizeof(float) * n_elements, s));
	c->tmp_alt_clear = false;
	if (sorted) {
		HIP_TRY(hipStreamWaitEvent(s, c->ev_gs, 0));
		std::swap(c->grid_sample_pos, c->gs_stage_pos);
		std::swap(c->grid_sample_idx, c->gs_stage_idx);
		std::swap(c->gs_sorted_pos, c->gs_eval_pos);
		std::swap(c->gs_sorted_idx, c->gs_eval_idx);
		c->density_grid_rng.advance();
		c->density_grid_rng.advance();
	} else {
		int rc = launch_grid_samples(c, s, c->density_grid_rng, c->density_grid_ema_step, n_uniform, n_nonuniform, c->grid_sample_pos.p, c->grid_sample_idx.p, nullptr, 0);
		if (rc != RNB_OK) return rc;
	}
	c->prof.mark(s, P_GRID_SAMPLES);
	c->n_grid_samples = n_samples;
	int rc;
	const uint64_t W = shard ? c->cfg.world_size : 1u, r = shard ? c->cfg.rank : 0u;
	if (sorted) {
		rc = launch_point_query(c, s, c->gs_eval_pos.p, n_samples, nullptr, c->gs_eval_idx.p, c->density_grid_tmp.p, 1, false, W > 1 ? c->gs_range.p : nullptr);
	} else {
		const uint32_t lo = (uint32_t)((uint64_t)n_samples * r / W), hi = (uint32_t)((uint64_t)n_samples * (r + 1) / W);
		rc = launch_point_query(c, s, c->grid_sample_pos.p + (size_t)lo * 3, hi - lo, nullptr, c->grid_sample_idx.p + lo, c->density_grid_tmp.p, 1, false);
	}
	if (rc != RNB_OK) return rc;
	c->prof.mark(s, P_POINT_QUERY);
	c->prof.units[P_POINT_QUERY] += n_samples / W;
	c->gs_todo.n_uniform = n_uniform; c->gs_todo.n_nonuniform = n_nonuniform;
	return RNB_OK;
}

int update_density_grid_back(rnb_ctx* c, hipStream_t s) {
	const uint32_t n_elements = GRID_CELLS * (c->aabb.max_cascade + 1);
	int rc;
	if (c->knobs.fused_update) hipLaunchKernelGGL(k_ema_mean, dim3(n_elements / 2048), dim3(256), 0, s, n_elements, c->cfg.density_grid_decay, c->density_grid.p, c->density_grid_tmp.p, c->mean_partial.p);
	else hipLaunchKernelGGL(k_ema_grid, dim3((n_elements + 127) / 128), dim3(128), 0, s, n_elements, c->cfg.density_grid_decay, c->density_grid.p, c->density_grid_tmp.p);
	HIP_TRY(hipGetLastError());
	++c->density_grid_ema_step;
	rc = update_bitfield(c, s, !c->overlap(), c->knobs.fused_update);
	c->prof.mark(s, P_EMA_BITFIELD);
	c->gs_todo.pending = true;
	return rc;
}

int training_prep_front(rnb_ctx* c, hipStream_t s, bool shard) {
	const uint32_t n_cascades = c->aabb.max_cascade + 1;
	if (c->training_step < 256) return update_density_grid_front(c, s, GRID_CELLS * n_cascades, 0, shard);
	return update_density_grid_front(c, s, GRID_CELLS / 4 * n_cascades, GRID_CELLS / 4 * n_cascades, shard);
}
int training_prep(rnb_ctx* c, hipStream_t s) {
	const bool shard = c->grid_exchange != nullptr && c->dp_order();
	int rc = training_prep_front(c, s, shard);
	if (rc != RNB_OK) return rc;
	if (shard) {
		const int xrc = c->grid_exchange(c->grid_exchange_user, c->density_grid_tmp.p, (uint64_t)GRID_CELLS * (c->aabb.max_cascade + 1), (void*)s);
		if (xrc != 0) return fail(RNB_ERR_INVALID, "the occupancy grid exchange (rnb_set_grid_exchange) failed");
	}
	return update_density_grid_back(c, s);
}

static int ensure_rgb_buffers(rnb_ctx* c) {
	if (c->cin_eval.p) return RNB_OK;
	const size_t B = c->cfg.target_batch_size;
	if (c->cin_eval.alloc(B * 16 * 32) != hipSuccess || c->dcin.alloc(B * 32) != hipSuccess || c->rgb_out_scratch.alloc(B * 16) != hipSuccess || c->src_slot.alloc(B) != hipSuccess)
		return fail(RNB_ERR_NOMEM, "hipMalloc failed for the colour-MLP training buffers");
	return RNB_OK;
}

int launch_forward(rnb_ctx* c, hipStream_t s, const float* coords, const uint32_t* n_ptr, uint32_t n_max, half_t* out, bool inference, const uint32_t* idx = nullptr, half_t* cin_out = nullptr) {
	if (n_max == 0) return RNB_OK;
	join_tail_host(c);
	FwdArgs a;
	a.coords = coords; a.n_ptr = n_ptr; a.n_max = n_max; a.out = out; a.sdf_bias = c->cfg.sdf_bias; a.idx = idx; a.cin_out = cin_out;
	a.wimg = (!inference && c->wimg_valid) ? c->wimg_fwd.p : nullptr;
	const uint32_t n_tiles = (n_max + TILE - 1) / TILE;
	const uint32_t grid = std::min<uint32_t>((n_tiles + WAVES_PER_WG - 1) / WAVES_PER_WG, (uint32_t)c->n_cus * 2);
	if (c->half_acc() && c->knobs.encode_depth) hipLaunchKernelGGL(k_forward_chained_emul_pipe<4>, dim3(grid), dim3(WG), LDS_FWD2, s, c->meta(), c->net(inference), a);
	else if (c->half_acc()) hipLaunchKernelGGL(k_forward_chained_emul, dim3(grid), dim3(WG), LDS_FWD2, s, c->meta(), c->net(inference), a);
	else if (c->knobs.encode_depth == 2) hipLaunchKernelGGL(k_forward_chained_pipe<2>, dim3(grid), dim3(WG), LDS_FWD2, s, c->meta(), c->net(inference), a);
	else if (c->knobs.encode_depth == 4 && c->knobs.encode_pair && c->n_dense_lead >= 5) hipLaunchKernelGGL((k_forward_chained_pipe<4, 5>), dim3(grid), dim3(WG), LDS_FWD2, s, c->meta(), c->net(inference), a);
	else if (c->knobs.encode_depth == 4) hipLaunchKernelGGL(k_forward_chained_pipe<4>, dim3(grid), dim3(WG), LDS_FWD2, s, c->meta(), c->net(inference), a);
	else if (c->knobs.encode_depth == 7) hipLaunchKernelGGL(k_forward_chained_pipe<7>, dim3(grid), dim3(WG), LDS_FWD2, s, c->meta(), c->net(inference), a);
	else hipLaunchKernelGGL(k_forward_chained, dim3(grid), dim3(WG), LDS_FWD2, s, c->meta(), c->net(inference), a);
	HIP_TRY(hipGetLastError());
	return RNB_OK;
}

static LossFlags loss_flags(const rnb_ctx* c) {
	LossFlags F;
	F.apply_L2 = c->cfg.apply_L2; F.apply_rgbplus = c->cfg.apply_rgbplus; F.apply_no_albedo = c->cfg.apply_no_albedo; F.apply_light_opti = c->cfg.apply_light_opti;
	F.apply_relu = c->cfg.apply_relu; F.apply_bce = c->cfg.apply_bce; F.snap = c->cfg.snap_to_pixel_centers;
	F.mask_loss_weight = c->cfg.mask_loss_weight; F.ek_loss_weight = c->cfg.ek_loss_weight;
	return F;
}

static uint32_t k1_for(const rnb_ctx* c, uint32_t n_rays) {
	if (c->fwd_k1 == 0 || c->fwd_k1_fixed) return c->fwd_k1;
	const float k = 8.f + 3.f * (float)c->cfg.target_batch_size / (float)std::max(1u, n_rays);
	const uint32_t k8 = (uint32_t)std::min(48.f, std::max(16.f, k) + 4.f) / 8u * 8u;
	return std::min(c->fwd_k1, std::max(16u, k8));
}

static bool lattice_is_linear() {
	const volatile float C = STEPSIZE;
	for (int e = -1; e <= 3; ++e) {
		const float base = std::ldexp(0.5f, e), ulp = std::ldexp(1.0f, e - 1 - 23);
		const volatile float d0 = (base + C) - base;
		for (const float t : {base, base + ulp, base + 2 * ulp, base + 3 * ulp, std::ldexp(1.0f, e) - 64 * d0, std::ldexp(1.0f, e) - 64 * d0 + ulp}) {
			const volatile float sum = t + C;
			if (sum - t != d0) return false;
		}
	}
	return true;
}

MarchArgs march_args(rnb_ctx* c, uint32_t n_rays, uint32_t n_rays_total, uint32_t max_samples) {
	MarchArgs a;
	static const bool linear = lattice_is_linear();
	a.lattice_ok = (linear && !c->knobs.march_running_sums) ? 1u : 0u;
	a.n_rays = n_rays;
	a.n_rays_global = n_rays * c->cfg.world_size;
	a.ray_offset = c->cfg.rank * n_rays;
	a.n_rays_total = n_rays_total;
	a.max_samples = max_samples;
	a.n_images = c->n_views;
	a.snap = c->cfg.snap_to_pixel_centers;
	a.rng = c->rng;
	a.A = c->aabb;
	a.views = c->views.p;
	a.bitfield = c->bitfield.p; a.coarse = c->coarse_bits.p;
	{
		const uint32_t seen = *reinterpret_cast<volatile uint32_t*>(c->host_coarse);
		const uint32_t budget = seen == 0xffffffffu ? 0u : (seen + seen / 8 + 64 + 63) / 64 * 64;
		a.n_blocks_lds = seen <= COARSE_MAX_BLOCKS ? std::min(budget, COARSE_MAX_BLOCKS) : 0u;
	}
	a.setup = c->ray_setup.p; a.ray_t = c->ray_t.p; a.d_unnorm = c->ray_dunnorm.p; a.steps = c->ray_steps.p; a.base = c->ray_base.p; a.slot = c->ray_slot.p;
	a.ray_indices = c->ray_indices.p; a.rays = c->rays.p; a.numsteps = c->numsteps.p; a.coords = c->coords.p; a.counters = c->counters.p;
	a.base1 = c->ray_base1.p; a.idx1 = c->idx1.p; a.k1 = k1_for(c, n_rays);
	a.F = loss_flags(c);
	for (int k = 0; k < 9; ++k) a.light_dirs[k] = c->light_dirs[k];
	a.ray_const = c->ray_const.p;
	a.part = 0;
	a.stats = c->march_stats.p;
	a.prio = (uint32_t)c->knobs.march_prio;
	a.use_bbox = (uint32_t)c->knobs.march_bbox;
	return a;
}

int generate_training_samples(rnb_ctx* c, hipStream_t s, uint32_t n_rays, uint32_t n_rays_total, uint32_t max_samples, hipEvent_t done = nullptr, hipEvent_t wait_before_write = nullptr, hipEvent_t rest_done = nullptr, hipEvent_t wait_before_scans = nullptr) {
	if (!c->coarse_valid) { const int rc0 = rebuild_coarse(c, s); if (rc0 != RNB_OK) return rc0; }
	MarchArgs a = march_args(c, n_rays, n_rays_total, max_samples);
	c->gen_k1 = a.k1;
	const uint32_t blocks = (n_rays + 127) / 128;
	c->prof.mark(s, P_NONE);
	const bool sc = c->aabb.cone_angle == 0.f && c->aabb.max_cascade == 0;
	const size_t march_lds = sc ? (size_t)(2 * COARSE_WORDS + 2 * a.n_blocks_lds) * sizeof(uint32_t) : 0;
	if (c->knobs.march_narrow || n_rays >= c->knobs.march_narrow_from) {
		if (sc && c->knobs.march_skip && c->knobs.march_skip_narrow && a.lattice_ok) {
			if (c->knobs.march_skip == 2) a.lattice_ok |= 2u;
			hipLaunchKernelGGL(k_march_count_skip_narrow, dim3(blocks), dim3(128), march_lds + COARSE_WORDS * sizeof(uint32_t), s, a);
			a.lattice_ok &= 1u;
		} else if (sc && c->knobs.march_bbox >= 2 && a.lattice_ok) {
			if (c->knobs.march_skip == 2) a.lattice_ok |= 2u;
			hipLaunchKernelGGL(k_march_count_bbox, dim3(blocks), dim3(128), march_lds, s, a);
			a.lattice_ok &= 1u;
		} else if (sc) hipLaunchKernelGGL(k_march_count<true>, dim3((n_rays + c->knobs.march_narrow_wgs - 1) / c->knobs.march_narrow_wgs), dim3(c->knobs.march_narrow_wgs), march_lds, s, a);
		else hipLaunchKernelGGL(k_march_count<false>, dim3(blocks), dim3(128), 0, s, a);
	} else if (sc && n_rays <= c->knobs.march_wave_per_ray_below) {
		hipLaunchKernelGGL((k_march_count_wide<64, true, 256>), dim3((n_rays + 3) / 4), dim3(256), march_lds, s, a);
	} else {
		const dim3 grid((n_rays + 15) / 16);
		if (sc && c->knobs.march_skip && a.lattice_ok) {
			if (c->knobs.march_skip == 2) a.lattice_ok |= 2u;
			if (c->knobs.march_wgs == 512) hipLaunchKernelGGL((k_march_count_skip<512>), dim3((n_rays + 31) / 32), dim3(512), march_lds + COARSE_WORDS * sizeof(uint32_t), s, a);
			else if (c->knobs.march_wgs == 1024) hipLaunchKernelGGL((k_march_count_skip<1024>), dim3((n_rays + 63) / 64), dim3(1024), march_lds + COARSE_WORDS * sizeof(uint32_t), s, a);
			else hipLaunchKernelGGL((k_march_count_skip<256>), grid, dim3(256), march_lds + COARSE_WORDS * sizeof(uint32_t), s, a);
			a.lattice_ok &= 1u;
		} else if (sc) hipLaunchKernelGGL((k_march_count_wide<16, true>), grid, dim3(256), march_lds, s, a);
		else hipLaunchKernelGGL((k_march_count_wide<16, false>), grid, dim3(256), 0, s, a);
	}
	c->prof.mark(s, P_MARCH_COUNT);
	if (wait_before_scans) HIP_TRY(hipStreamWaitEvent(s, wait_before_scans, 0));
	const uint32_t n_scan_tiles = (n_rays + SCAN_TILE - 1) / SCAN_TILE;
	if (c->knobs.scan_chain && n_scan_tiles <= 64) {
		ScanChainArgs q;
		q.n = n_rays; q.max_samples = max_samples; q.k1 = a.k1; q.steps = c->ray_steps.p; q.base = c->ray_base.p; q.slot = c->ray_slot.p; q.base1 = c->ray_base1.p;
		q.counters = c->counters.p; q.fwd_counts = c->fwd_counts.p; q.words = c->scan_words.p; q.words2 = c->scan_words.p + 2 * 64 * 4; q.ticket = ++c->scan_ticket; q.error = c->host_coarse_dev + 5; q.plain = c->knobs.chain_plain ? 1u : 0u;
		hipLaunchKernelGGL(k_scan_rays_chain, dim3(n_scan_tiles), dim3(SCAN_WG), 0, s, q);
	} else if (n_rays >= c->knobs.march_narrow_from) {
		const uint32_t n_tiles = (n_rays + SCAN_TILE - 1) / SCAN_TILE;
		hipLaunchKernelGGL(k_scan_rays_sums, dim3(n_tiles), dim3(SCAN_WG), 0, s, n_rays, c->ray_steps.p, c->scan_tiles.p);
		hipLaunchKernelGGL(k_scan_rays_base, dim3(n_tiles), dim3(SCAN_WG), 0, s, n_rays, max_samples, a.k1, c->ray_steps.p, c->scan_tiles.p, c->ray_base.p, c->scan_tiles.p + 64, c->counters.p);
		hipLaunchKernelGGL(k_scan_rays_slots, dim3(n_tiles), dim3(SCAN_WG), 0, s, n_rays, max_samples, a.k1, c->ray_steps.p, c->ray_base.p, c->scan_tiles.p + 64, c->ray_slot.p, c->ray_base1.p, c->counters.p, c->fwd_counts.p);
	} else
		hipLaunchKernelGGL(k_scan_rays, dim3(1), dim3(1024), 0, s, n_rays, max_samples, c->ray_steps.p, c->ray_base.p, c->ray_slot.p, c->counters.p, a.k1, c->ray_base1.p, c->fwd_counts.p);
	c->prof.mark(s, P_SCAN_RAYS);
	if (wait_before_write) HIP_TRY(hipStreamWaitEvent(s, wait_before_write, 0));
	const bool dense_const = c->knobs.ray_const_dense != 0;
	float* const ray_const = a.ray_const;
	if (dense_const) a.ray_const = nullptr;
	c->gen_split = rest_done != nullptr && a.k1 != 0 && (c->knobs.ray_const_dense == 1 ? false : (c->knobs.march_write_split < 0 ? n_rays < 65536u : c->knobs.march_write_split != 0));
	for (uint32_t part = c->gen_split ? 1u : 0u; part <= (c->gen_split ? 2u : 0u); ++part) {
		a.part = part;
		hipEvent_t ev = part == 2 ? rest_done : done;
		if (dense_const && part != 1) ev = nullptr;
		if (c->knobs.march_write_wg == 1024) {
			if (n_rays >= c->knobs.march_narrow_from) LAUNCH_EV((k_march_write<16, 1024>), dim3((n_rays + 63) / 64), dim3(1024), 0, s, ev, a);
			else LAUNCH_EV((k_march_write<64, 1024>), dim3((n_rays + 15) / 16), dim3(1024), 0, s, ev, a);
		} else if (c->knobs.march_write_wg == 64) {
			if (n_rays >= c->knobs.march_narrow_from) LAUNCH_EV((k_march_write<16, 64>), dim3((n_rays + 3) / 4), dim3(64), 0, s, ev, a);
			else LAUNCH_EV((k_march_write<64, 64>), dim3(n_rays), dim3(64), 0, s, ev, a);
		} else if (c->knobs.march_write_wg == 128) {
			if (n_rays >= c->knobs.march_narrow_from) LAUNCH_EV((k_march_write<16, 128>), dim3((n_rays + 7) / 8), dim3(128), 0, s, ev, a);
			else LAUNCH_EV((k_march_write<64, 128>), dim3((n_rays + 1) / 2), dim3(128), 0, s, ev, a);
		} else if (n_rays >= c->knobs.march_narrow_from) LAUNCH_EV((k_march_write<16, 256>), dim3((n_rays + 15) / 16), dim3(256), 0, s, ev, a);
		else LAUNCH_EV((k_march_write<64, 256>), dim3((n_rays + 3) / 4), dim3(256), 0, s, ev, a);
	}
	if (dense_const) LAUNCH_EV(k_ray_constants, dim3((n_rays + 63) / 64), dim3(64), 0, s, c->gen_split ? rest_done : done, a, ray_const);
	c->prof.mark(s, P_MARCH_WRITE);
	c->prof.units[P_MARCH_COUNT] += n_rays;
	HIP_TRY(hipGetLastError());
	return RNB_OK;
}

int compute_loss(rnb_ctx* c, hipStream_t s, uint32_t n_rays, uint32_t n_rays_total, uint32_t two_round_n_max = 0, bool defer_rollover = false, bool reduce_too = false) {
	LossArgs a;
	a.n_rays = n_rays; a.n_rays_global = n_rays * c->cfg.world_size; a.ray_offset = c->cfg.rank * n_rays; a.n_rays_total = n_rays_total;
	a.n_images = c->n_views; a.B = c->cfg.target_batch_size;
	a.rng = c->rng; a.A = c->aabb;
	a.F = loss_flags(c);
	a.ray_const = two_round_n_max ? c->ray_const.p : nullptr;
	for (int k = 0; k < 9; ++k) a.light_dirs[k] = c->light_dirs[k];
	a.views = c->views.p; a.counters = c->counters.p; a.ray_indices = c->ray_indices.p; a.rays = c->rays.p; a.numsteps = c->numsteps.p;
	a.coords = c->coords.p; a.mlp_out = c->mlp_out.p; a.ray_loss = c->ray_loss.p; a.ncomp = c->ncomp.p; a.cbase = c->cbase.p;
	a.coords_compacted = c->coords_compacted.p; a.dloss = c->dloss_dout.p; a.loss = c->loss.p; a.ek_loss = c->ek_loss; a.mask_loss = c->mask_loss;
	a.src_slot = c->cin_flow ? c->src_slot.p : nullptr;
	a.chain_rec = c->knobs.loss_chain_records ? c->chain_rec.p : nullptr;
	a.ray_grad = c->ray_grad.p; a.ray_of = c->ray_of.p; a.slot_of = c->slot_of.p;
	a.scan_words = nullptr; a.scan_ticket = 0; a.scan_error = nullptr; a.scan_total = nullptr;
	a.wg_partial = c->wg_partial.p; a.red_out = nullptr; a.red_host_out = nullptr; a.red_host_seq = 0;
	c->loss_reduced = false;
	if (!c->pre.loss_cleared && !defer_rollover) HIP_TRY(hipMemsetAsync(c->loss.p, 0, c->loss.bytes(), s));
	c->pre.loss_cleared = false;
	const uint32_t blocks = (n_rays + 3) / 4;
	const bool rows = n_rays >= c->knobs.march_narrow_from && !c->knobs.loss_wave_per_ray;
	const uint32_t blocks_heads = rows ? (n_rays + LOSS1_WG / 16 - 1) / (LOSS1_WG / 16) : (n_rays + LOSS1_WG / 64 - 1) / (LOSS1_WG / 64);
	auto launch_heads = [&]() {
		if (rows) hipLaunchKernelGGL(k_loss_pass1_heads<16>, dim3(blocks_heads), dim3(LOSS1_WG), 0, s, a);
		else hipLaunchKernelGGL(k_loss_pass1_heads<64>, dim3(blocks_heads), dim3(LOSS1_WG), 0, s, a);
	};
	a.cap = 0xffffffffu; a.phase = 0; a.unfinished = c->unfinished.p; a.idx2 = c->idx2.p; a.fwd_counts = c->fwd_counts.p;
	c->prof.mark(s, P_NONE);
	if (two_round_n_max) {
		a.cap = c->cur_k1;
		launch_heads();
		c->prof.mark(s, P_LOSS_PASS1);
		int rc = launch_forward(c, s, c->coords.p, c->fwd_counts.p + 2, two_round_n_max, c->mlp_out.p, false, c->idx2.p, c->cin_flow ? c->cin_eval.p : nullptr);
		if (rc != RNB_OK) return rc;
		c->prof.mark(s, P_FORWARD);
		a.phase = 1;
	}
	if (a.phase) hipLaunchKernelGGL(k_loss_pass1, dim3(std::min(blocks, 1024u)), dim3(256), 0, s, a);
	else launch_heads();
	c->prof.mark(s, P_LOSS_PASS1);
	const bool flat = a.chain_rec && c->knobs.loss_flat;
	if (flat && c->knobs.loss_scan_fused && (n_rays + SCAN_TILE - 1) / SCAN_TILE <= (c->knobs.loss_scan_fused_always ? 64u : 8u)) {
		a.scan_words = c->scan_words.p + 64 * 4; a.scan_ticket = ++c->scan_ticket; a.scan_error = c->host_coarse_dev + 6; a.scan_total = c->counters.p + 1;
	} else if (n_rays >= c->knobs.march_narrow_from && c->knobs.scan_chain && (n_rays + SCAN_TILE - 1) / SCAN_TILE <= 64) {
		hipLaunchKernelGGL(k_scan_compact_chain, dim3((n_rays + SCAN_TILE - 1) / SCAN_TILE), dim3(SCAN_WG), 0, s, n_rays, c->ncomp.p, c->cbase.p, c->counters.p,
		                   c->scan_words.p + 64 * 4, ++c->scan_ticket, c->host_coarse_dev + 6);
	} else if (n_rays >= c->knobs.march_narrow_from) {
		const uint32_t n_tiles = (n_rays + SCAN_TILE - 1) / SCAN_TILE;
		hipLaunchKernelGGL(k_scan_compact_sums, dim3(n_tiles), dim3(SCAN_WG), 0, s, n_rays, c->ncomp.p, c->scan_tiles.p + 256);
		hipLaunchKernelGGL(k_scan_compact_offsets, dim3(n_tiles), dim3(SCAN_WG), 0, s, n_rays, c->ncomp.p, c->scan_tiles.p + 256, c->cbase.p, c->counters.p);
	} else
		hipLaunchKernelGGL(k_scan_compact, dim3(1), dim3(1024), 0, s, n_rays, c->ncomp.p, c->cbase.p, c->counters.p);
	c->prof.mark(s, P_SCAN_COMPACT);
	if (flat) {
		hipLaunchKernelGGL(k_loss_pass2_rays<16>, dim3((n_rays + 15) / 16), dim3(256), 0, s, a);
		hipEvent_t ev = nullptr;
		if (reduce_too) {
			const bool poll = c->poll_loss();
			if (poll) { if (++c->rb_seq == 0) ++c->rb_seq; c->loss_polled = false; }
			a.red_out = c->loss_sums.p; a.red_host_out = reinterpret_cast<double*>(c->host_rb_dev); a.red_host_seq = poll ? c->rb_seq : 0u;
			ev = poll ? nullptr : c->ev_loss;
			c->loss_reduced = true;
		}
		LAUNCH_EV(k_loss_pass2_samples, dim3(1 + (a.B + 255) / 256), dim3(256), 0, s, ev, a);
		c->prof.mark(s, P_LOSS_PASS2);
		HIP_TRY(hipGetLastError());
		return RNB_OK;
	} else if (a.chain_rec) {
		if (rows) hipLaunchKernelGGL((k_loss_pass2<16, true>), dim3((n_rays + 15) / 16), dim3(256), 0, s, a);
		else hipLaunchKernelGGL((k_loss_pass2<64, true>), dim3(blocks), dim3(256), 0, s, a);
	} else {
		if (rows) hipLaunchKernelGGL((k_loss_pass2<16, false>), dim3((n_rays + 15) / 16), dim3(256), 0, s, a);
		else hipLaunchKernelGGL((k_loss_pass2<64, false>), dim3(blocks), dim3(256), 0, s, a);
	}
	if (!defer_rollover) hipLaunchKernelGGL(k_rollover, dim3(1024), dim3(256), 0, s, c->cfg.target_batch_size, c->counters.p, c->dloss_dout.p, c->coords_compacted.p, a.src_slot);
	c->prof.mark(s, P_LOSS_PASS2);
	HIP_TRY(hipGetLastError());
	return RNB_OK;
}

int forward_backward(rnb_ctx* c, hipStream_t s, bool join_dw = true) {
	const uint32_t B = c->cfg.target_batch_size;
	const rnb_ctx::ScatterGroups& sg = c->sg;
	const uint32_t L = c->cfg.n_levels;
	const uint32_t e_c = sg.e_c, l_fine = sg.l_fine;
	join_tail_host(c);
	const bool half = c->half_acc();
	if (!c->grads_clean) HIP_TRY(hipMemsetAsync(c->grad_ptr(0), 0, c->n_params * c->grad_elem(), s));
	c->grads_clean = false;
	c->sc.valid = false; c->sc.exchanged = false; c->sc.sharded = false; c->sc.all_final_recorded = false; c->sc.dw_joined = true; c->sc.c_early = false; c->sc.c_side = false;
	TrainArgs a;
	a.coords = c->coords_compacted.p; a.dout = c->dloss_dout.p; a.B = B; a.B_global = B * c->cfg.world_size; a.sdf_bias = c->cfg.sdf_bias; a.t = c->ts; a.skip_rgb = c->cfg.apply_no_albedo ? 1u : 0u;
	const bool split = c->rgb_split();
	a.wimg = !c->wimg_valid ? nullptr : (!c->knobs.fwd_bwd_generic) ? c->wimg_fbs.p : c->wimg_train.p;
	const bool sdf_only = (a.skip_rgb && !c->knobs.fwd_bwd_generic) || split;
	const uint32_t fb_grid = sdf_only ? std::min<uint32_t>((B / TILE + WAVES_PER_WG - 1) / WAVES_PER_WG, (uint32_t)c->n_cus * c->knobs.fbs_wg_per_cu) : c->fwd_grid;
	const bool sliced = half && sdf_only && c->knobs.dw_sliced;
	const uint32_t n_slices = (B + DW_SLICE - 1) / DW_SLICE;
	const size_t slab = sliced ? (size_t)n_slices : sdf_only ? (size_t)fb_grid : (size_t)c->dw_nwg;
	float* p_rgb2; float* p_rgb1; float* p_rgb0; float* p_sdf1; float* p_sdf0; float* p_sdf0b; float* p_sdf1b;
	{
		float* p = c->dw_partial.p;
		p_rgb2 = p;  p += slab * 16 * 64;
		p_rgb1 = p;  p += slab * 64 * 64;
		p_rgb0 = p;  p += slab * 64 * 32;
		p_sdf1 = p;  p += slab * 16 * 64;
		p_sdf0 = p;  p += slab * 64 * 32;
		p_sdf0b = p; p += slab * 64 * 32;
		p_sdf1b = p; p += slab * 16 * 64;
	}
	a.dw_w0 = p_sdf0; a.dw_w0b = p_sdf0b; a.dw_w1 = p_sdf1; a.dw_w1b = p_sdf1b;
	const bool side_streams = c->overlap();
	c->prof.mark(s, P_NONE);
	hipEvent_t ev_fb = side_streams ? c->ev_fb : nullptr;
	if (split) {
		int rc = ensure_rgb_buffers(c);
		if (rc != RNB_OK) return rc;
		const bool flow = c->cin_flow;
		c->cin_flow = false;
		if (!flow) {
			rc = launch_forward(c, s, c->coords_compacted.p, nullptr, B, c->rgb_out_scratch.p, false, nullptr, c->cin_eval.p);
			if (rc != RNB_OK) return rc;
		}
		RgbArgs r;
		r.cin = c->cin_eval.p; r.src_slot = flow ? c->src_slot.p : nullptr; r.dout = c->dloss_dout.p; r.dcin = c->dcin.p; r.B = B;
		r.wimg = c->wimg_valid ? c->wimg_rgb.p : nullptr;
		r.dw_c0 = p_rgb0; r.dw_c1 = p_rgb1; r.dw_c2 = p_rgb2;
		r.t = c->ts;
		if (half && sliced) hipLaunchKernelGGL(k_rgb_fwd_bwd_hs, dim3(fb_grid), dim3(WG), LDS_RGB, s, c->net(false), r);
		else if (half) hipLaunchKernelGGL(k_rgb_fwd_bwd_h, dim3(fb_grid), dim3(WG), LDS_RGB, s, c->net(false), r);
		else hipLaunchKernelGGL(k_rgb_fwd_bwd, dim3(fb_grid), dim3(WG), LDS_RGB, s, c->net(false), r);
		a.dcin = c->dcin.p;
		if (half && sliced) LAUNCH_EV(k_fwd_bwd_sdf_full_hs, dim3(fb_grid), dim3(WG), LDS_FBS_FULL, s, ev_fb, c->meta(), c->net(false), a);
		else if (half) LAUNCH_EV(k_fwd_bwd_sdf_full_h, dim3(fb_grid), dim3(WG), LDS_FBS_FULL, s, ev_fb, c->meta(), c->net(false), a);
		else LAUNCH_EV(k_fwd_bwd_sdf_full, dim3(fb_grid), dim3(WG), LDS_FBS_FULL, s, ev_fb, c->meta(), c->net(false), a);
	} else if (sdf_only && half && sliced) LAUNCH_EV(k_fwd_bwd_sdf_hs, dim3(fb_grid), dim3(WG), LDS_FBS, s, ev_fb, c->meta(), c->net(false), a);
	else if (sdf_only && half) LAUNCH_EV(k_fwd_bwd_sdf_h, dim3(fb_grid), dim3(WG), LDS_FBS, s, ev_fb, c->meta(), c->net(false), a);
	else if (sdf_only) LAUNCH_EV(k_fwd_bwd_sdf, dim3(fb_grid), dim3(WG), LDS_FBS, s, ev_fb, c->meta(), c->net(false), a);
	else LAUNCH_EV(k_fwd_bwd, dim3(fb_grid), dim3(WG), LDS_TRAIN, s, ev_fb, c->meta(), c->net(false), a);
	c->prof.mark(s, P_FWD_BWD);
	c->prof.units[P_FWD_BWD] += B;
	const TrainScratch& T = c->ts;

	auto launch_dw = [&](hipStream_t sd, hipEvent_t done) {
		const uint32_t nwg = c->dw_nwg, chunk = c->dw_chunk;
		DwAllArgs d;
		d.n = 0; d.nwg = nwg; d.B = B; d.chunk = chunk;
		auto add = [&](uint32_t kind, const half_t* yt, const half_t* xt, float* part) { d.kind[d.n] = kind; d.YT[d.n] = yt; d.XT[d.n] = xt; d.partial[d.n] = part; ++d.n; };
		if (!a.skip_rgb) {
			add(DW_4x4, T.dh2, T.h1, p_rgb1);
			add(DW_4x2, T.dh1, T.cin, p_rgb0);
			add(DW_1x4, T.dr, T.h2, p_rgb2);
		}
		add(DW_4x2, T.dz, T.sdfin, p_sdf0);
		add(DW_4x2, T.dz1, T.ddin, p_sdf0b);
		add(DW_1x4, T.dso, T.z1, p_sdf1);
		add(DW_1x4_ONES, nullptr, T.front, p_sdf1b);
		for (uint32_t q = d.n; q < 7; ++q) { d.kind[q] = DW_1x4; d.YT[q] = nullptr; d.XT[q] = nullptr; d.partial[q] = nullptr; }
		if (!sdf_only) hipLaunchKernelGGL(k_dw_all, dim3(nwg * d.n), dim3(WG), 0, sd, d);
		if (sliced) {
			DwSlicedArgs q;
			q.n = 0; q.B = B; q.n_slices = n_slices;
			uint32_t wgs = 0;
			auto add_sliced = [&](const half_t* yt, const half_t* xt, float* out, uint32_t n_out, uint32_t n_live, uint32_t n_in, uint32_t ones) {
				q.YT[q.n] = yt; q.XT[q.n] = xt; q.out[q.n] = out; q.n_out[q.n] = n_out; q.n_out_live[q.n] = n_live; q.n_in[q.n] = n_in; q.ones[q.n] = ones;
				q.first_wg[q.n] = wgs; wgs += n_slices * ((n_out * n_in / 4 + 255) / 256); ++q.n;
			};
			if (!a.skip_rgb) {
				add_sliced(T.dh2, T.h1, p_rgb1, 64, 64, 64, 0);
				add_sliced(T.dh1, T.cin, p_rgb0, 64, 64, 32, 0);
				add_sliced(T.dr, T.h2, p_rgb2, 16, 3, 64, 0);
			}
			add_sliced(T.dz, T.sdfin, p_sdf0, 64, 64, 32, 0);
			add_sliced(T.dz1, T.ddin, p_sdf0b, 64, 64, 32, 0);
			add_sliced(T.dso, T.z1, p_sdf1, 16, split ? 16 : 1, 64, 0);
			add_sliced(nullptr, T.front, p_sdf1b, 16, 1, 64, 1);
			for (uint32_t g = q.n; g < 7; ++g) { q.YT[g] = nullptr; q.XT[g] = nullptr; q.out[g] = nullptr; q.n_out[g] = 0; q.n_out_live[g] = 0; q.n_in[g] = 4; q.ones[g] = 0; }
			for (uint32_t g = q.n; g < 8; ++g) q.first_wg[g] = wgs;
			hipLaunchKernelGGL(k_dw_sliced, dim3(wgs), dim3(256), 0, sd, q);
		}
		DwFinishArgs f;
		f.partial[0] = p_rgb2; f.partial[1] = p_rgb1; f.partial[2] = p_rgb0; f.partial[3] = p_sdf1; f.partial[4] = p_sdf0; f.partial[5] = p_sdf0b; f.partial[6] = p_sdf1b;
		f.n_partials = (uint32_t)slab; f.sliced = sliced ? 1u : 0u;
		f.var_partial = c->var_partial.p; f.n_var_partials = fb_grid * WAVES_PER_WG;
		f.grads = c->grads.p; f.grads16 = half ? c->grads16.p : nullptr; f.off_sdf = (uint32_t)c->off_sdf; f.off_rgb = (uint32_t)c->off_rgb; f.off_var = (uint32_t)c->off_var; f.skip_rgb = a.skip_rgb;
		const uint32_t n_fin_blocks = (RNB_N_SDF_MLP_PARAMS + (a.skip_rgb ? 0 : RNB_N_RGB_MLP_PARAMS)) / DWF_PARAMS + 1;
		LAUNCH_EV(k_dw_finish, dim3(n_fin_blocks), dim3(DWF_WG), 0, sd, done, f);
	};

	const uint32_t scatter_cap = c->knobs.scatter_wg_per_cu >= 0 ? (uint32_t)c->knobs.scatter_wg_per_cu : ((sdf_only && !split) ? 0u : 2u);
	ScatterArgs sa;
	sa.g12 = T.g12; sa.srec = T.srec; sa.B = B; sa.grid_grad = half ? nullptr : c->grads.p + c->off_grid;
	sa.grid_grad16 = half ? reinterpret_cast<uint32_t*>(c->grads16.p + c->off_grid) : nullptr;
	const bool fixed = c->fixed_acc();
	sa.grid_fixed = fixed ? c->grads_fixed.p : nullptr;
	sa.prio = side_streams ? (uint32_t)c->knobs.scatter_prio : 0u;
	auto narrow = [&](hipStream_t st, hipEvent_t done, uint32_t l0, uint32_t l1) {
		const uint64_t lo = (uint64_t)c->grid.offsets[l0] * 2, hi = (uint64_t)c->grid.offsets[l1] * 2;
		if (hi <= lo) { if (done) (void)hipEventRecord(done, st); return; }
		const uint32_t blocks = (uint32_t)std::min<uint64_t>(2048, ((hi - lo) / 2 + 255) / 256);
		LAUNCH_EV(k_fixed_narrow, dim3(blocks), dim3(256), 0, st, done, c->grads_fixed.p, half ? nullptr : c->grads.p + c->off_grid, half ? c->grads16.p + c->off_grid : nullptr, lo, hi);
	};
	const bool dbg_levels = c->prof.on && c->knobs.dbg_scatter_lo >= 0;
	bool sc_first = true;
	auto sc_flags = [&]() -> uint32_t { const bool any = c->knobs.scatter_anyorder && side_streams && !sc_first; sc_first = false; return any ? (uint32_t)hipExtAnyOrderLaunch : 0u; };
	auto launch_a = [&](hipStream_t st, hipEvent_t done, uint32_t l0, uint32_t l1) {
		if (dbg_levels) { l0 = std::max(l0, (uint32_t)c->knobs.dbg_scatter_lo); l1 = std::max(l0, std::min(l1, (uint32_t)c->knobs.dbg_scatter_hi)); }
		const uint32_t n_vb = (B * 4 + 255) / 256, cap = scatter_cap ? std::max(1u, (uint32_t)c->n_cus * scatter_cap / std::max(1u, l1 - l0)) : n_vb;
		if (l1 > l0 && fixed) {
			LAUNCH_EVF(k_grid_scatter_quad_fixed, dim3(std::min(n_vb, cap), l1 - l0), dim3(256), 0, st, nullptr, sc_flags(), c->meta(), sa, l0, n_vb);
			narrow(st, done, l0, l1);
		} else if (l1 > l0 && half && c->knobs.scatter_plain) LAUNCH_EVF(k_grid_scatter_quad_h_per_addend, dim3(std::min(n_vb, cap), l1 - l0), dim3(256), 0, st, done, sc_flags(), c->meta(), sa, l0, n_vb);
		else if (l1 > l0 && half) LAUNCH_EVF(k_grid_scatter_quad_h, dim3(std::min(n_vb, cap), l1 - l0), dim3(256), 0, st, done, sc_flags(), c->meta(), sa, l0, n_vb);
		else if (l1 > l0) LAUNCH_EVF(k_grid_scatter_quad, dim3(std::min(n_vb, cap), l1 - l0), dim3(256), 0, st, done, sc_flags(), c->meta(), sa, l0, n_vb);
		else if (done) (void)hipEventRecord(done, st);
	};
	auto launch_b = [&](hipStream_t st, hipEvent_t done) {
		uint32_t e_c = sg.e_c, l_fine = sg.l_fine;
		if (dbg_levels) { e_c = std::max(e_c, (uint32_t)c->knobs.dbg_scatter_lo); l_fine = std::min(l_fine, (uint32_t)c->knobs.dbg_scatter_hi); }
		if (l_fine <= e_c) { if (done) (void)hipEventRecord(done, st); return; }
// ... 277 lines not shown
		if (!c->knobs.unsafe_skip_joins) HIP_TRY(hipStreamWaitEvent(s, c->ev_adam, 0));
	} else {
		adam_launch(c, s, 0, c->n_params);
	}
	return optimizer_finish(c, s, images_done);
}

int optimizer_step_shard(rnb_ctx* c, uint32_t part, hipStream_t st) {
	rnb_shard_part parts[RNB_MAX_SHARD_PARTS];
	uint32_t n = 0;
	shard_layout(c, parts, &n);
	if (part >= n) return fail(RNB_ERR_INVALID, "rnb_train_step_apply_shard: no such block");
	const rnb_shard_part& p = parts[part];
	{ const int rc = optimizer_begin(c); if (rc != RNB_OK) return rc; }
	if (!c->sc.dw_joined) HIP_TRY(hipStreamWaitEvent(st, c->ev_dw, 0));
	if (p.own_lo > p.lo) HIP_TRY(hipMemsetAsync(c->grad_ptr(p.lo), 0, (p.own_lo - p.lo) * c->grad_elem(), st));
	if (p.hi > p.own_hi) HIP_TRY(hipMemsetAsync(c->grad_ptr(p.own_hi), 0, (p.hi - p.own_hi) * c->grad_elem(), st));
	adam_launch(c, st, std::min<uint64_t>(p.own_lo, c->n_params), std::min<uint64_t>(p.own_hi, c->n_params));
	HIP_TRY(hipGetLastError());
	return RNB_OK;
}

hipStream_t as_stream(void* s) { return reinterpret_cast<hipStream_t>(s); }

static int update_config_common(rnb_config& dst, const rnb_config* cfg) {
	if (cfg->abi_version != RNB_ABI_VERSION) return fail(RNB_ERR_INVALID, "abi_version mismatch");
	if (cfg->n_levels != dst.n_levels || cfg->log2_hashmap_size != dst.log2_hashmap_size || cfg->base_resolution != dst.base_resolution ||
	    cfg->per_level_scale != dst.per_level_scale || cfg->target_batch_size != dst.target_batch_size || cfg->max_rays_per_batch != dst.max_rays_per_batch ||
	    cfg->aabb_scale != dst.aabb_scale || cfg->seed != dst.seed || cfg->world_size != dst.world_size || cfg->rank != dst.rank || cfg->accumulate != dst.accumulate || cfg->deterministic != dst.deterministic)
		return fail(RNB_ERR_INVALID, "rnb_update_config: geometry fields differ from the context's");
	dst = *cfg;
	return RNB_OK;
}


}

extern "C" {
#define RNB_GUARD                                                                                                   \
	catch (const std::bad_alloc&) { return fail(RNB_ERR_NOMEM, "out of host memory (std::bad_alloc)"); }                \
	catch (const std::exception& e_) { return fail(RNB_ERR_INVALID, std::string("exception: ") + e_.what()); }          \
	catch (...) { return fail(RNB_ERR_INVALID, "unknown exception"); }

const char* rnb_last_error(void) { return g_err.c_str(); }
uint32_t rnb_abi_version(void) { return RNB_ABI_VERSION; }

int rnb_default_config(rnb_config* cfg) try {
	if (!cfg) return fail(RNB_ERR_INVALID, "cfg is null");
	std::memset(cfg, 0, sizeof(*cfg));
	cfg->abi_version = RNB_ABI_VERSION;
	cfg->n_levels = 14; cfg->log2_hashmap_size = 19; cfg->base_resolution = 16;
	cfg->per_level_scale = std::exp(std::log(2048.0f * 1.0f / 16.0f) / (14 - 1));
	cfg->valid_level_scale = 0.02f; cfg->base_valid_level_scale = 0.2f; cfg->base_training_step = 100;
	cfg->sdf_bias = -0.1f;
	cfg->target_batch_size = 1u << 18; cfg->initial_rays_per_batch = 1u << 12; cfg->max_rays_per_batch = 1u << 18;
	cfg->aabb_scale = 1; cfg->seed = 1337;
	cfg->mask_loss_weight = 1.0f; cfg->ek_loss_weight = 0.01f;
	cfg->apply_L2 = 1; cfg->apply_rgbplus = 1; cfg->apply_no_albedo = 0; cfg->apply_light_opti = 0;
	cfg->apply_supernormal = 0; cfg->apply_relu = 0; cfg->apply_bce = 0; cfg->snap_to_pixel_centers = 1;
	cfg->learning_rate = 1e-3f; cfg->beta1 = 0.9f; cfg->beta2 = 0.99f; cfg->epsilon = 1e-15f; cfg->l2_reg = 1e-6f;
	cfg->ema_decay = 0.95f; cfg->lr_decay_start = 20000; cfg->lr_decay_interval = 10000; cfg->lr_decay_base = 0.33f;
	cfg->density_grid_decay = 0.95f;
	cfg->world_size = 1; cfg->rank = 0;
	cfg->overlap = 1;
	return RNB_OK;
} RNB_GUARD

int rnb_destroy(rnb_ctx* c) try {
	if (!c) return RNB_OK;
	if (c->march_stats.p) {
		unsigned long long h[8] = {0, 0, 0, 0, 0, 0, 0, 0};
		(void)hipDeviceSynchronize();
		if (hipMemcpy(h, c->march_stats.p, sizeof(h), hipMemcpyDeviceToHost) == hipSuccess && h[0])
			fprintf(stderr, "k_march_count_skip: %llu wavefronts, %.2f loop iterations each; %llu rays: %.3f skipped at least once, %.3f ended early, %.5f start-overs per ray, %.3f rounds per ray looking for a re-entry cell\n",
			        h[0], (double)h[1] / h[0], h[2], (double)h[3] / h[2], (double)h[6] / h[2], (double)h[4] / h[2], (double)h[5] / h[2]);
		c->march_stats.free();
	}
	c->opt_rec.free(); c->params_fp32.free(); c->grads.free(); c->grads16.free(); c->grads_fixed.free(); c->adam_m.free(); c->adam_v.free(); c->params_fp16.free(); c->params_ema.free(); c->adam_steps.free(); c->adam_lr_table.free();
	c->density_grid.free(); c->density_grid_tmp.free(); c->density_grid_tmp_alt.free(); c->density_mean.free(); c->mean_partial.free(); c->loss_sums.free(); c->bitfield.free(); c->coarse_bits.free(); c->coarse_count.free();
	c->grid_sample_pos.free(); c->grid_sample_idx.free(); c->views.free(); c->pixels.free();
	c->gs_sorted_pos.free(); c->gs_sorted_idx.free(); c->gs_stage_pos.free(); c->gs_stage_idx.free(); c->gs_hist.free(); c->gs_range.free(); c->gs_eval_pos.free(); c->gs_eval_idx.free();
	c->ray_indices.free(); c->numsteps.free(); c->counters.free(); c->rays.free(); c->coords.free(); c->coords_compacted.free();
	c->loss.free(); c->mlp_out.free(); c->chain_rec.free(); c->ray_grad.free(); c->ray_of.free(); c->slot_of.free(); c->wg_partial.free(); c->dloss_dout.free();
	c->wimg_fwd.free(); c->wimg_fbs.free(); c->wimg_train.free(); c->wimg_rgb.free(); c->cin_eval.free(); c->dcin.free(); c->rgb_out_scratch.free(); c->src_slot.free(); c->ray_const.free(); c->ray_base1.free(); c->scan_words.free(); c->idx1.free(); c->idx2.free(); c->fwd_counts.free(); c->unfinished.free();
	c->ray_setup.free(); c->ray_t.free(); c->ray_dunnorm.free(); c->ray_steps.free(); c->ray_base.free(); c->ray_slot.free(); c->ncomp.free(); c->cbase.free(); c->scan_tiles.free(); c->loss_partial.free(); c->ray_loss.free();
	c->render_rays[0].free(); c->render_rays[1].free(); c->render_keep.free(); c->render_scan.free(); c->render_counts.free(); c->render_res.free(); c->render_coords.free(); c->render_out.free();
	c->mc_table.free(); c->fm.free(); c->g12.free(); c->srec.free(); c->var_partial.free(); c->dw_partial.free();
	c->prof.destroy();
	if (c->s_march) { (void)hipStreamSynchronize(c->s_march); (void)hipStreamDestroy(c->s_march); }
	for (hipStream_t st : {c->s_dw, c->s_adam}) if (st) { (void)hipStreamSynchronize(st); (void)hipStreamDestroy(st); }
	for (hipEvent_t e : {c->ev_join, c->ev_loss, c->ev_march, c->ev_fb, c->ev_dw, c->ev_adam, c->ev_tail, c->ev_march_rest, c->ev_all, c->ev_grid, c->ev_gs, c->ev_sc[0], c->ev_sc[1], c->ev_sc[2], c->ev_sc[3]}) if (e) (void)hipEventDestroy(e);
	if (c->host_rb) (void)hipHostFree(c->host_rb);
	if (c->host_coarse) (void)hipHostFree(c->host_coarse);
	delete c;
	return RNB_OK;
} RNB_GUARD

int rnb_create(const rnb_config* cfg, rnb_ctx** out) try {
	if (!cfg || !out) return fail(RNB_ERR_INVALID, "null argument");
	if (cfg->abi_version != RNB_ABI_VERSION) return fail(RNB_ERR_INVALID, "abi_version mismatch");
	if (cfg->n_levels == 0 || cfg->n_levels > 14) return fail(RNB_ERR_INVALID, "n_levels must be in [1,14]");
	if (cfg->base_resolution < 2) return fail(RNB_ERR_INVALID, "base_resolution must be >= 2");
	if (cfg->aabb_scale == 0 || (cfg->aabb_scale & (cfg->aabb_scale - 1)) != 0 || cfg->aabb_scale > 128) return fail(RNB_ERR_INVALID, "aabb_scale must be a power of two <= 128");
	if (cfg->target_batch_size == 0 || cfg->target_batch_size % 128 != 0) return fail(RNB_ERR_INVALID, "target_batch_size must be a positive multiple of 128");
	if (cfg->max_rays_per_batch == 0 || cfg->max_rays_per_batch > (1u << 18)) return fail(RNB_ERR_INVALID, "max_rays_per_batch must be in [1, 2^18]");
	if (cfg->world_size == 0 || cfg->rank >= cfg->world_size) return fail(RNB_ERR_INVALID, "bad rank/world_size");
	if (cfg->accumulate > RNB_ACCUM_HALF) return fail(RNB_ERR_INVALID, "accumulate must be RNB_ACCUM_FP32 or RNB_ACCUM_HALF");
	if (cfg->deterministic > 1) return fail(RNB_ERR_INVALID, "deterministic must be 0 or 1");
	if (cfg->accumulate == RNB_ACCUM_HALF && getenv("RNB_FWD_BWD_GENERIC")) return fail(RNB_ERR_INVALID, "RNB_FWD_BWD_GENERIC (the generic training kernel of rounds 1-3) has no half-accumulate form");
	int dev = 0;
	HIP_TRY(hipGetDevice(&dev));
	hipDeviceProp_t prop;
	HIP_TRY(hipGetDeviceProperties(&prop, dev));
	if (std::string(prop.gcnArchName).find("gfx950") == std::string::npos) return fail(RNB_ERR_DEVICE, std::string("librnb_neus2_hip targets gfx950 (MI355X); found ") + prop.gcnArchName);
	rnb_ctx* c = new rnb_ctx();
#define HIP_TRY_C(expr)                                                                                                  \
	do {                                                                                                                 \
		hipError_t e_ = (expr);                                                                                          \
		if (e_ != hipSuccess) { rnb_destroy(c); return fail(RNB_ERR_DEVICE, std::string(#expr) + ": " + hipGetErrorString(e_)); } \
	} while (0)
	c->cfg = *cfg;
	if (const char* e = getenv("RNB_DETERMINISTIC")) c->cfg.deterministic = atoi(e) != 0 ? 1u : 0u;
	c->n_cus = prop.multiProcessorCount;
	build_grid_tables(c);
	c->off_sdf = 0;
	c->off_rgb = RNB_N_SDF_MLP_PARAMS;
	c->off_grid = c->off_rgb + RNB_N_RGB_MLP_PARAMS;
	c->off_var = c->off_grid + c->n_grid_params;
	c->n_params = c->off_var + RNB_N_VARIANCE_PARAMS;
	c->aabb.mn = 0.5f - 0.5f * std::min(1u << (N_CASCADES - 1), cfg->aabb_scale);
	c->aabb.mx = 0.5f + 0.5f * std::min(1u << (N_CASCADES - 1), cfg->aabb_scale);
	c->aabb.max_cascade = 0;
	while ((1u << c->aabb.max_cascade) < cfg->aabb_scale) ++c->aabb.max_cascade;
	c->aabb.cone_angle = cfg->aabb_scale <= 1 ? 0.0f : (1.0f / 256.0f);
	const uint32_t B = cfg->target_batch_size, maxr = cfg->max_rays_per_batch;
	const uint32_t n_grid = GRID_CELLS * (c->aabb.max_cascade + 1);
#define ALLOC(buf, count)                                                                                              \
	do {                                                                                                               \
		if ((buf).alloc(count) != hipSuccess) { rnb_destroy(c); return fail(RNB_ERR_NOMEM, "hipMalloc failed for " #buf); } \
	} while (0)
	{
		const uint64_t q = 4ull * std::max(1u, cfg->world_size);
		c->param_capacity = (c->n_params + q - 1) / q * q;
	}
#define ALLOC_P(buf)                                                                                                   \
	do {                                                                                                               \
		if ((buf).alloc_padded(c->n_params, c->param_capacity) != hipSuccess) { rnb_destroy(c); return fail(RNB_ERR_NOMEM, "hipMalloc failed for " #buf); } \
	} while (0)
	if (getenv("RNB_MARCH_STATS")) { if (c->march_stats.alloc_padded(8, 8) != hipSuccess) { rnb_destroy(c); return fail(RNB_ERR_NOMEM, "hipMalloc failed"); } }
	ALLOC(c->adam_lr_table, ADAM_LR_TABLE_N);
	ALLOC(c->opt_rec, c->param_capacity * 4);
	if (cfg->accumulate == RNB_ACCUM_HALF) ALLOC_P(c->grads16); else ALLOC_P(c->grads);
	if (c->cfg.deterministic) {
		if (c->grads_fixed.alloc_padded(c->n_grid_params, c->n_grid_params) != hipSuccess) { rnb_destroy(c); return fail(RNB_ERR_NOMEM, "hipMalloc failed for the fixed-point gradient accumulators"); }
	}
	ALLOC_P(c->params_fp32); ALLOC_P(c->adam_m); ALLOC_P(c->adam_v); ALLOC_P(c->params_fp16); ALLOC_P(c->params_ema); ALLOC_P(c->adam_steps);
#undef ALLOC_P
	ALLOC(c->density_grid, n_grid); ALLOC(c->density_grid_tmp, n_grid); ALLOC(c->density_grid_tmp_alt, n_grid); ALLOC(c->density_mean, 1); ALLOC(c->mean_partial, 1024); ALLOC(c->loss_sums, 16);
	ALLOC(c->bitfield, (size_t)GRID_CELLS / 8 * N_CASCADES); ALLOC(c->coarse_bits, COARSE_BUF_WORDS); ALLOC(c->coarse_count, 1);
	ALLOC(c->grid_sample_pos, (size_t)n_grid * 3); ALLOC(c->grid_sample_idx, n_grid);
	ALLOC(c->ray_indices, maxr); ALLOC(c->numsteps, (size_t)maxr * 2); ALLOC(c->counters, 4); ALLOC(c->rays, (size_t)maxr * 6);
	ALLOC(c->coords, (size_t)B * 16 * 7); ALLOC(c->mlp_out, (size_t)B * 16 * 16); ALLOC(c->chain_rec, (size_t)B * 16 * CHAIN_REC_FLOATS); ALLOC(c->ray_grad, (size_t)maxr * 16); ALLOC(c->ray_of, B); ALLOC(c->slot_of, B); ALLOC(c->wg_partial, ((size_t)maxr + 15) / 16 * 3); ALLOC(c->dloss_dout, (size_t)B * 16); ALLOC(c->coords_compacted, (size_t)B * 7);
	ALLOC(c->loss, (size_t)maxr * 3); c->ek_loss = c->loss.p + maxr; c->mask_loss = c->loss.p + (size_t)maxr * 2;
	ALLOC(c->ray_setup, (size_t)maxr * 8); ALLOC(c->ray_t, (size_t)maxr * RNB_MAX_STEPS); ALLOC(c->ray_dunnorm, (size_t)maxr * 3); ALLOC(c->ray_steps, maxr); ALLOC(c->ray_base, maxr); ALLOC(c->ray_slot, maxr);
	ALLOC(c->scan_tiles, 256 + 64); ALLOC(c->loss_partial, 64 * 3);
	ALLOC(c->ncomp, maxr); ALLOC(c->cbase, maxr); ALLOC(c->ray_loss, maxr);
	ALLOC(c->wimg_fwd, W_FWD_END); ALLOC(c->wimg_fbs, SWF_END); ALLOC(c->wimg_train, W_TRAIN_END); ALLOC(c->wimg_rgb, RW_END);
// ... 28 lines not shown
	HIP_TRY_C(hipMemset(c->density_grid.p, 0, c->density_grid.bytes()));
	HIP_TRY_C(hipMemset(c->density_grid_tmp.p, 0, c->density_grid_tmp.bytes()));
	HIP_TRY_C(hipMemset(c->bitfield.p, 0, c->bitfield.bytes()));
	HIP_TRY_C(hipMemset(c->counters.p, 0, c->counters.bytes()));
	HIP_TRY_C(hipMemset(c->density_mean.p, 0, 4));
	HIP_TRY_C(hipMemset(c->coords.p, 0, c->coords.bytes()));
	HIP_TRY_C(hipMemset(c->coords_compacted.p, 0, c->coords_compacted.bytes()));
	HIP_TRY_C(hipMemset(c->dloss_dout.p, 0, c->dloss_dout.bytes()));
	HIP_TRY_C(hipMemset(c->mlp_out.p, 0, c->mlp_out.bytes()));
	int rc = reset_optimizer_state(c);
	if (rc != RNB_OK) { rnb_destroy(c); return rc; }
	HIP_TRY_C(hipFuncSetAttribute(reinterpret_cast<const void*>(k_forward_chained), hipFuncAttributeMaxDynamicSharedMemorySize, (int)LDS_FWD2));
	HIP_TRY_C(hipFuncSetAttribute(reinterpret_cast<const void*>(k_forward_chained_emul), hipFuncAttributeMaxDynamicSharedMemorySize, (int)LDS_FWD2));
	HIP_TRY_C(hipFuncSetAttribute(reinterpret_cast<const void*>(k_forward_chained_emul_pipe<4>), hipFuncAttributeMaxDynamicSharedMemorySize, (int)LDS_FWD2));
	HIP_TRY_C(hipFuncSetAttribute(reinterpret_cast<const void*>(k_forward_chained_pipe<2>), hipFuncAttributeMaxDynamicSharedMemorySize, (int)LDS_FWD2));
	HIP_TRY_C(hipFuncSetAttribute(reinterpret_cast<const void*>(k_forward_chained_pipe<4>), hipFuncAttributeMaxDynamicSharedMemorySize, (int)LDS_FWD2));
	HIP_TRY_C(hipFuncSetAttribute(reinterpret_cast<const void*>(k_forward_chained_pipe<7>), hipFuncAttributeMaxDynamicSharedMemorySize, (int)LDS_FWD2));
	HIP_TRY_C(hipFuncSetAttribute(reinterpret_cast<const void*>(k_forward_chained_pipe<4, 5>), hipFuncAttributeMaxDynamicSharedMemorySize, (int)LDS_FWD2));
	HIP_TRY_C(hipFuncSetAttribute(reinterpret_cast<const void*>(k_fwd_bwd), hipFuncAttributeMaxDynamicSharedMemorySize, (int)LDS_TRAIN));
	HIP_TRY_C(hipFuncSetAttribute(reinterpret_cast<const void*>(k_fwd_bwd_sdf), hipFuncAttributeMaxDynamicSharedMemorySize, (int)LDS_FBS));
	HIP_TRY_C(hipFuncSetAttribute(reinterpret_cast<const void*>(k_fwd_bwd_sdf_full), hipFuncAttributeMaxDynamicSharedMemorySize, (int)LDS_FBS_FULL));
	HIP_TRY_C(hipFuncSetAttribute(reinterpret_cast<const void*>(k_rgb_fwd_bwd), hipFuncAttributeMaxDynamicSharedMemorySize, (int)LDS_RGB));
	HIP_TRY_C(hipFuncSetAttribute(reinterpret_cast<const void*>(k_fwd_bwd_sdf_h), hipFuncAttributeMaxDynamicSharedMemorySize, (int)LDS_FBS));
	HIP_TRY_C(hipFuncSetAttribute(reinterpret_cast<const void*>(k_fwd_bwd_sdf_hs), hipFuncAttributeMaxDynamicSharedMemorySize, (int)LDS_FBS));
	HIP_TRY_C(hipFuncSetAttribute(reinterpret_cast<const void*>(k_fwd_bwd_sdf_full_hs), hipFuncAttributeMaxDynamicSharedMemorySize, (int)LDS_FBS_FULL));
	HIP_TRY_C(hipFuncSetAttribute(reinterpret_cast<const void*>(k_rgb_fwd_bwd_hs), hipFuncAttributeMaxDynamicSharedMemorySize, (int)LDS_RGB));
	HIP_TRY_C(hipFuncSetAttribute(reinterpret_cast<const void*>(k_fwd_bwd_sdf_full_h), hipFuncAttributeMaxDynamicSharedMemorySize, (int)LDS_FBS_FULL));
	HIP_TRY_C(hipFuncSetAttribute(reinterpret_cast<const void*>(k_rgb_fwd_bwd_h), hipFuncAttributeMaxDynamicSharedMemorySize, (int)LDS_RGB));
	HIP_TRY_C(hipFuncSetAttribute(reinterpret_cast<const void*>(k_grid_scatter_lds_h), hipFuncAttributeMaxDynamicSharedMemorySize, 150 * 1024));
	{
		const int march_lds_max = (int)((2 * COARSE_WORDS + 2 * COARSE_MAX_BLOCKS) * sizeof(uint32_t));
		HIP_TRY_C(hipFuncSetAttribute(reinterpret_cast<const void*>(k_march_count<true>), hipFuncAttributeMaxDynamicSharedMemorySize, march_lds_max));
		HIP_TRY_C(hipFuncSetAttribute(reinterpret_cast<const void*>(k_march_count_wide<16, true>), hipFuncAttributeMaxDynamicSharedMemorySize, march_lds_max));
		HIP_TRY_C(hipFuncSetAttribute(reinterpret_cast<const void*>(k_march_count_wide<64, true, 256>), hipFuncAttributeMaxDynamicSharedMemorySize, march_lds_max));
		HIP_TRY_C(hipFuncSetAttribute(reinterpret_cast<const void*>(k_march_count_skip<256>), hipFuncAttributeMaxDynamicSharedMemorySize, march_lds_max + (int)(COARSE_WORDS * sizeof(uint32_t))));
		HIP_TRY_C(hipFuncSetAttribute(reinterpret_cast<const void*>(k_march_count_skip<512>), hipFuncAttributeMaxDynamicSharedMemorySize, march_lds_max + (int)(COARSE_WORDS * sizeof(uint32_t))));
		HIP_TRY_C(hipFuncSetAttribute(reinterpret_cast<const void*>(k_march_count_skip<1024>), hipFuncAttributeMaxDynamicSharedMemorySize, march_lds_max + (int)(COARSE_WORDS * sizeof(uint32_t))));
		HIP_TRY_C(hipFuncSetAttribute(reinterpret_cast<const void*>(k_march_count_skip_narrow), hipFuncAttributeMaxDynamicSharedMemorySize, march_lds_max + (int)(COARSE_WORDS * sizeof(uint32_t))));
		HIP_TRY_C(hipFuncSetAttribute(reinterpret_cast<const void*>(k_march_count_bbox), hipFuncAttributeMaxDynamicSharedMemorySize, march_lds_max));
	}
HIP_TRY_C(hipFuncSetAttribute(reinterpret_cast<const void*>(k_grid_scatter_lds), hipFuncAttributeMaxDynamicSharedMemorySize, 150 * 1024));
	HIP_TRY_C(hipFuncSetAttribute(reinterpret_cast<const void*>(k_grid_scatter_lds_fixed), hipFuncAttributeMaxDynamicSharedMemorySize, 150 * 1024));
	c->rng = Pcg32{cfg->seed};
	c->density_grid_rng = Pcg32{c->rng.next_uint()};
	(void)c->rng.next_uint();
	c->rays_per_batch = std::min(cfg->initial_rays_per_batch, cfg->max_rays_per_batch);
	c->training_step = 0;
	c->valid_level = compute_valid_level(c->cfg, 0);
	build_light_dirs(c);
	if (const char* e = getenv("RNB_FWD_K1")) { c->fwd_k1 = (uint32_t)atoi(e); c->fwd_k1_fixed = true; }
	{
		rnb_ctx::Knobs& k = c->knobs;
		k.march_narrow = getenv("RNB_MARCH_NARROW") != nullptr; k.fwd_bwd_generic = getenv("RNB_FWD_BWD_GENERIC") != nullptr;
		k.loss_wave_per_ray = getenv("RNB_LOSS_WAVE_PER_RAY") != nullptr;
		k.dp_order = getenv("RNB_DP_FORCE_COLLECTIVES") != nullptr;
		k.march_late = getenv("RNB_MARCH_LATE") != nullptr;
		k.march_running_sums = getenv("RNB_MARCH_RUNNING_SUMS") != nullptr;
		if (const char* e = getenv("RNB_MARCH_NARROW_FROM")) k.march_narrow_from = (uint32_t)atoi(e);
		if (const char* e = getenv("RNB_SCATTER_WG_PER_CU")) k.scatter_wg_per_cu = std::max(0, atoi(e));
		if (const char* e = getenv("RNB_FBS_WG_PER_CU")) k.fbs_wg_per_cu = (uint32_t)std::max(1, std::min(2, atoi(e)));
		if (const char* e = getenv("RNB_GRID_PRESORT")) k.grid_presort = atoi(e) != 0;
		if (const char* e = getenv("RNB_FUSED_UPDATE")) k.fused_update = atoi(e) != 0;
		if (const char* e = getenv("RNB_POLL_LOSS")) k.poll_loss = atoi(e) != 0;
		if (const char* e = getenv("RNB_DEFER_TAIL")) k.defer_tail = atoi(e) != 0;
		if (const char* e = getenv("RNB_JOIN_FOLD")) k.join_fold = atoi(e) != 0;
		if (const char* e = getenv("RNB_SCATTER_C_SIDE")) k.scatter_c_side = atoi(e) != 0;
		if (const char* e = getenv("RNB_UNSAFE_SKIP_JOINS")) k.unsafe_skip_joins = atoi(e) != 0;
		if (const char* e = getenv("RNB_MARCH_WAVE_PER_RAY_BELOW")) k.march_wave_per_ray_below = (uint32_t)atoi(e);
		if (const char* e = getenv("RNB_SCATTER_ORDER")) k.scatter_order = std::max(-1, std::min(2, atoi(e)));
		if (const char* e = getenv("RNB_SCAN_CHAIN")) k.scan_chain = atoi(e) != 0;
		if (const char* e = getenv("RNB_LOSS_SCAN_FUSED")) { k.loss_scan_fused = atoi(e) != 0; k.loss_scan_fused_always = atoi(e) == 2; }
		if (const char* e = getenv("RNB_LOSS_FLAT")) k.loss_flat = atoi(e) != 0;
		if (const char* e = getenv("RNB_LOSS_CHAIN_RECORDS")) k.loss_chain_records = atoi(e) != 0;
		if (const char* e = getenv("RNB_RAY_CONST_DENSE")) k.ray_const_dense = atoi(e);
		if (const char* e = getenv("RNB_MARCH_WRITE_SPLIT")) k.march_write_split = atoi(e) != 0 ? 1 : 0;
		if (const char* e = getenv("RNB_SCATTER_PLAIN")) k.scatter_plain = atoi(e) != 0;
		if (const char* e = getenv("RNB_MARCH_NARROW_WGS")) { const int w = atoi(e); k.march_narrow_wgs = (w == 64 || w == 256 || w == 512) ? (uint32_t)w : 128u; }
		if (const char* e = getenv("RNB_MARCH_WGS")) { const int w = atoi(e); k.march_wgs = (w == 256 || w == 512) ? w : 1024; }
		if (const char* e = getenv("RNB_MARCH_WRITE_WG")) { const int w = atoi(e); k.march_write_wg = (w == 1024 || w == 128 || w == 64) ? w : 256; }
		if (const char* e = getenv("RNB_CHAIN_PLAIN")) k.chain_plain = atoi(e) != 0;
		if (const char* e = getenv("RNB_POINT_XCD")) k.point_xcd = atoi(e) != 0;
		if (const char* e = getenv("RNB_DW_SLICED")) k.dw_sliced = atoi(e) != 0;
		if (const char* e = getenv("RNB_ENCODE_PAIR")) k.encode_pair = atoi(e) != 0;
		if (const char* e = getenv("RNB_ENCODE_DEPTH")) { const int d = atoi(e); k.encode_depth = (d == 0 || d == 2 || d == 4 || d == 7) ? d : 4; }
		if (const char* e = getenv("RNB_DEBUG_SCATTER_LEVELS")) { int lo = -1, hi = -1; if (sscanf(e, "%d,%d", &lo, &hi) == 2 && lo >= 0 && hi > lo) { k.dbg_scatter_lo = lo; k.dbg_scatter_hi = hi; } }
		if (const char* e = getenv("RNB_SCATTER_C_EARLY")) k.scatter_c_early = atoi(e) != 0;
		if (const char* e = getenv("RNB_SCATTER_RL_STAGED")) k.scatter_rl_staged = atoi(e) != 0 ? 1 : 0;
		if (const char* e = getenv("RNB_SCATTER_ANYORDER")) k.scatter_anyorder = atoi(e) != 0;
		if (const char* e = getenv("RNB_SCATTER_SHARE")) k.scatter_share = atoi(e) != 0;
		if (const char* e = getenv("RNB_MARCH_SKIP")) k.march_skip = std::max(0, std::min(2, atoi(e)));
		if (const char* e = getenv("RNB_MARCH_SKIP_NARROW")) k.march_skip_narrow = atoi(e) != 0;
		if (const char* e = getenv("RNB_SCATTER_PRIO")) k.scatter_prio = std::max(0, std::min(3, atoi(e)));
		if (const char* e = getenv("RNB_MARCH_PRIO")) k.march_prio = std::max(0, std::min(3, atoi(e)));
		if (const char* e = getenv("RNB_MARCH_BBOX")) k.march_bbox = std::max(0, std::min(2, atoi(e)));
		if (const char* e = getenv("RNB_DW_LATE")) k.dw_late = atoi(e) != 0;
		if (const char* e = getenv("RNB_SCATTER_KMIN")) k.scatter_kmin = std::max(0, std::min(16, atoi(e)));
		if (const char* e = getenv("RNB_SCATTER_RL_UPTO")) k.scatter_rl_upto = std::max(0, std::min(14, atoi(e)));
	}
	plan_scatter_groups(c);
	{
		int pr[3] = {0, 0, 0};
		if (const char* e = getenv("RNB_STREAM_PRIO")) sscanf(e, "%d,%d,%d", &pr[0], &pr[1], &pr[2]);
		hipStream_t* st[3] = {&c->s_march, &c->s_dw, &c->s_adam};
		for (int i = 0; i < 3; ++i) {
			if (pr[i] == 0) HIP_TRY_C(hipStreamCreateWithFlags(st[i], hipStreamNonBlocking));
			else HIP_TRY_C(hipStreamCreateWithPriority(st[i], hipStreamNonBlocking, pr[i]));
		}
	}
	HIP_TRY_C(hipEventCreateWithFlags(&c->ev_loss, hipEventDisableTiming));
	const unsigned dev_flags = hipEventDisableTiming | (unsigned)hipEventDisableSystemFence;
	for (hipEvent_t* e : {&c->ev_join, &c->ev_march, &c->ev_fb, &c->ev_dw, &c->ev_adam, &c->ev_tail, &c->ev_march_rest, &c->ev_all, &c->ev_grid, &c->ev_gs, &c->ev_sc[0], &c->ev_sc[1], &c->ev_sc[2], &c->ev_sc[3]}) HIP_TRY_C(hipEventCreateWithFlags(e, dev_flags));
	HIP_TRY_C(hipHostMalloc(reinterpret_cast<void**>(&c->host_rb), sizeof(*c->host_rb), hipHostMallocMapped));
	std::memset(c->host_rb, 0, sizeof(*c->host_rb));
	HIP_TRY_C(hipHostGetDevicePointer(&c->host_rb_dev, c->host_rb, 0));
	HIP_TRY_C(hipHostMalloc(reinterpret_cast<void**>(&c->host_coarse), 64, hipHostMallocMapped));
	std::memset(c->host_coarse, 0, 64);
	*c->host_coarse = 0xffffffffu;
	HIP_TRY_C(hipMemset(c->scan_words.p, 0, c->scan_words.bytes()));
	HIP_TRY_C(hipHostGetDevicePointer(reinterpret_cast<void**>(&c->host_coarse_dev), c->host_coarse, 0));
	*out = c;
	return RNB_OK;
#undef HIP_TRY_C
} RNB_GUARD

int rnb_update_config(rnb_ctx* c, const rnb_config* cfg) try {
	if (!c || !cfg) return fail(RNB_ERR_INVALID, "null argument");
	discard_premarch(c);
	int rc = update_config_common(c->cfg, cfg);
	if (rc != RNB_OK) return rc;
	build_light_dirs(c);
	return RNB_OK;
} RNB_GUARD

uint64_t rnb_n_params(const rnb_ctx* c) { return c ? c->n_params : 0; }

int rnb_param_layout(const rnb_ctx* c, uint64_t offsets[5]) try {
	if (!c || !offsets) return fail(RNB_ERR_INVALID, "null argument");
	offsets[0] = c->off_sdf; offsets[1] = c->off_rgb; offsets[2] = c->off_grid; offsets[3] = c->off_var; offsets[4] = c->n_params;
	return RNB_OK;
} RNB_GUARD

int rnb_grid_tables(const rnb_ctx* c, uint32_t* offsets, uint32_t* resolution, float* scale) try {
	if (!c) return fail(RNB_ERR_INVALID, "null ctx");
	for (uint32_t i = 0; i <= c->cfg.n_levels; ++i) if (offsets) offsets[i] = c->grid.offsets[i];
	for (uint32_t i = 0; i < c->cfg.n_levels; ++i) { if (resolution) resolution[i] = c->grid.resolution[i]; if (scale) scale[i] = c->grid.scale[i]; }
	return RNB_OK;
} RNB_GUARD

int rnb_init_params(rnb_ctx* c, const float* sdf_w) try {
	if (!c || !sdf_w) return fail(RNB_ERR_INVALID, "null argument");
	discard_premarch(c);
	HIP_TRY(hipDeviceSynchronize());
	std::seed_seq seq{c->cfg.seed};
	std::vector<uint32_t> seeds(2);
	seq.generate(std::begin(seeds), std::end(seeds));
	Pcg32 rnd{seeds.front()};
	std::vector<float> mlp(RNB_N_SDF_MLP_PARAMS + RNB_N_RGB_MLP_PARAMS, 0.f);
	auto xavier = [&](float* dst, int rows, int cols) {
		float scale = 1.f;
		scale *= std::sqrt(6.0f / (float)(cols + rows));
		for (int i = 0; i < rows * cols; ++i) dst[i] = (float)(rnd.next_float() * 2.0f * scale - scale);
	};
	xavier(mlp.data(), 64, 32);
	xavier(mlp.data() + 64 * 32, 16, 64);
	std::memcpy(mlp.data(), sdf_w, sizeof(float) * RNB_N_SDF_MLP_PARAMS);
	float* rgb = mlp.data() + RNB_N_SDF_MLP_PARAMS;
// ... 252 lines not shown
	uint64_t total = 0;
	do { n = (n + 1023) / 1024; total += n; } while (n > 1);
	return total;
}
int scan_exclusive(uint32_t* data, uint64_t n, hipStream_t s, uint32_t* total_out, uint32_t* scratch) {
	std::vector<uint32_t*> levels{data};
	std::vector<uint64_t> sizes{n};
	while (true) {
		const uint64_t nb = (sizes.back() + 1023) / 1024;
		uint32_t* sums = scratch;
		scratch += nb;
		hipLaunchKernelGGL(k_scan_blocks, dim3((uint32_t)nb), dim3(1024), 0, s, levels.back(), sizes.back(), sums);
		levels.push_back(sums); sizes.push_back(nb);
		if (nb == 1) break;
	}
	HIP_TRY(hipGetLastError());
	HIP_TRY(hipMemcpyAsync(total_out, levels.back(), 4, hipMemcpyDeviceToHost, s));
	for (size_t k = levels.size() - 1; k >= 2; --k) {
		hipLaunchKernelGGL(k_scan_add, dim3((uint32_t)sizes[k - 1]), dim3(1024), 0, s, levels[k - 2], sizes[k - 2], levels[k - 1]);
	}
	HIP_TRY(hipGetLastError());
	HIP_TRY(hipStreamSynchronize(s));
	return RNB_OK;
}
}

static int ensure_mc_table(rnb_ctx* c) {
	if (c->mc_table.p) return RNB_OK;
	static const mesh::Tables T;
	std::vector<McTable> h(1);
	for (int m = 0; m < 256; ++m) {
		int k = 0;
		for (; T.tri[m][k] >= 0; ++k) h[0].tri[m][k] = T.tri[m][k];
		h[0].n[m] = (uint8_t)k;
		for (; k < 40; ++k) h[0].tri[m][k] = -1;
	}
	if (c->mc_table.alloc(1) != hipSuccess) return fail(RNB_ERR_NOMEM, "hipMalloc failed for the case table");
	HIP_TRY(hipMemcpy(c->mc_table.p, h.data(), sizeof(McTable), hipMemcpyHostToDevice));
	return RNB_OK;
}

int rnb_marching_cubes(rnb_ctx* c, void* stream, const float* density, const uint32_t res[3], const float aabb_min[3], const float aabb_max[3], float thresh,
                       float** verts_out, uint32_t** indices_out, uint32_t* n_verts, uint32_t* n_indices) try {
	if (!c || !density || !res || !aabb_min || !aabb_max || !verts_out || !indices_out || !n_verts || !n_indices) return fail(RNB_ERR_INVALID, "null argument");
	*verts_out = nullptr; *indices_out = nullptr; *n_verts = 0; *n_indices = 0;
	const uint64_t res3 = (uint64_t)res[0] * res[1] * res[2];
	if (res3 == 0 || res3 >= (1ull << 32)) return fail(RNB_ERR_INVALID, "lattice must hold 1 .. 2^32-1 points");
	hipStream_t s = as_stream(stream);
	if (int rc = ensure_mc_table(c); rc != RNB_OK) return rc;
	McArgs a;
	a.density = density; a.rx = res[0]; a.ry = res[1]; a.rz = res[2]; a.thresh = thresh;
	for (int d = 0; d < 3; ++d) { a.sc[d] = (aabb_max[d] - aabb_min[d]) / (float)res[d]; a.mn[d] = aabb_min[d]; }
	const uint64_t n_wg64 = (res3 + MC_WG - 1) / MC_WG;
	const uint32_t n_wg = (uint32_t)n_wg64;
	uint32_t* wg = nullptr;
	uint32_t* scan_scratch = nullptr;
	int32_t* vidx = nullptr;
	float* verts = nullptr;
	uint32_t* indices = nullptr;
	auto cleanup = [&](int rc) { if (wg) (void)hipFree(wg); if (scan_scratch) (void)hipFree(scan_scratch); if (vidx) (void)hipFree(vidx); if (rc != RNB_OK) { if (verts) (void)hipFree(verts); if (indices) (void)hipFree(indices); } return rc; };
	if (hipMalloc((void**)&wg, (size_t)n_wg * 4) != hipSuccess || hipMalloc((void**)&scan_scratch, scan_scratch_elems(n_wg) * 4) != hipSuccess || hipMalloc((void**)&vidx, (size_t)res3 * 3 * 4) != hipSuccess) return cleanup(fail(RNB_ERR_NOMEM, "hipMalloc failed for the marching-cubes scratch (12 bytes per lattice point)"));
	uint32_t nv = 0, ni = 0;
	hipLaunchKernelGGL(k_mc_verts<false>, dim3(n_wg), dim3(MC_WG), 0, s, a, wg, (const uint32_t*)nullptr, (float*)nullptr, (int32_t*)nullptr);
	int rc = scan_exclusive(wg, n_wg, s, &nv, scan_scratch);
	if (rc != RNB_OK) return cleanup(rc);
	if (nv && hipMalloc((void**)&verts, (size_t)nv * 12) != hipSuccess) return cleanup(fail(RNB_ERR_NOMEM, "hipMalloc failed for the vertices"));
	hipLaunchKernelGGL(k_mc_verts<true>, dim3(n_wg), dim3(MC_WG), 0, s, a, (uint32_t*)nullptr, wg, verts, vidx);
	hipLaunchKernelGGL(k_mc_faces<false>, dim3(n_wg), dim3(MC_WG), 0, s, a, c->mc_table.p, wg, (const uint32_t*)nullptr, vidx, (uint32_t*)nullptr);
	rc = scan_exclusive(wg, n_wg, s, &ni, scan_scratch);
	if (rc != RNB_OK) return cleanup(rc);
	if (ni && hipMalloc((void**)&indices, (size_t)ni * 4) != hipSuccess) return cleanup(fail(RNB_ERR_NOMEM, "hipMalloc failed for the indices"));
	hipLaunchKernelGGL(k_mc_faces<true>, dim3(n_wg), dim3(MC_WG), 0, s, a, c->mc_table.p, (uint32_t*)nullptr, wg, vidx, indices);
	if (hipStreamSynchronize(s) != hipSuccess || hipGetLastError() != hipSuccess) return cleanup(fail(RNB_ERR_DEVICE, "rnb_marching_cubes: kernel failure"));
	*verts_out = verts; *indices_out = indices; *n_verts = nv; *n_indices = ni;
	return cleanup(RNB_OK);
} RNB_GUARD

int rnb_generate_training_samples(rnb_ctx* c, void* stream, uint32_t n_rays, uint32_t n_rays_total, uint32_t max_samples) try {
	if (!c) return fail(RNB_ERR_INVALID, "null ctx");
	discard_premarch(c);
	if (c->n_views == 0) return fail(RNB_ERR_INVALID, "no dataset");
	if (n_rays == 0 || n_rays > c->cfg.max_rays_per_batch) return fail(RNB_ERR_INVALID, "n_rays out of range");
	if (max_samples > c->cfg.target_batch_size * 16) return fail(RNB_ERR_INVALID, "max_samples exceeds 16*target_batch_size");
	c->cin_flow = false;
	return generate_training_samples(c, as_stream(stream), n_rays, n_rays_total, max_samples);
} RNB_GUARD

int rnb_compute_loss(rnb_ctx* c, void* stream, uint32_t n_rays, uint32_t n_rays_total) try {
	if (!c) return fail(RNB_ERR_INVALID, "null ctx");
	if (c->n_views == 0) return fail(RNB_ERR_INVALID, "no dataset");
	if (n_rays == 0 || n_rays > c->cfg.max_rays_per_batch) return fail(RNB_ERR_INVALID, "n_rays out of range");
	c->cin_flow = false;
	return compute_loss(c, as_stream(stream), n_rays, n_rays_total);
} RNB_GUARD

int rnb_forward_backward(rnb_ctx* c, void* stream) try {
	if (!c) return fail(RNB_ERR_INVALID, "null ctx");
	c->cin_flow = false;
	return forward_backward(c, as_stream(stream));
} RNB_GUARD

int rnb_optimizer_step(rnb_ctx* c, void* stream) try {
	if (!c) return fail(RNB_ERR_INVALID, "null ctx");
	return optimizer_step(c, as_stream(stream));
} RNB_GUARD

static void discard_premarch(rnb_ctx* c) {
	c->pre.march_joined = false;
	if (!c->pre.valid) return;
	(void)hipStreamSynchronize(c->s_march);
	c->n_rays_total = c->pre.n_rays_total;
	c->pre.valid = false;
	c->pre.loss_cleared = false;
}

static uint32_t next_max_inference(rnb_ctx* c) {
	const uint32_t max_samples = c->cfg.target_batch_size * 16;
	if (c->measured_batch_size_before_compaction == 0) { c->measured_batch_size_before_compaction = max_samples; return max_samples; }
	return next_multiple_u32(std::min(c->measured_batch_size_before_compaction, max_samples), 128u);
}


static int step_front(rnb_ctx* c, hipStream_t s) {
	c->valid_level = compute_valid_level(c->cfg, (int)c->training_step);
	const bool joined = c->join_pending;
	if (c->join_pending) { HIP_TRY(hipStreamWaitEvent(s, c->ev_join, 0)); c->join_pending = false; }
	if (c->tail_pending) { HIP_TRY(hipStreamWaitEvent(s, c->ev_tail, 0)); c->tail_pending = false; }
	c->grid_updated = false;
	c->prep_ms = 0.f;
	int rc;
	if (prep_due(c->training_step)) {
		discard_premarch(c);
		const uint32_t n_prep_to_skip = std::min(std::max(c->training_step / 16u, 1u), 16u);
		auto t0 = std::chrono::steady_clock::now();
		rc = training_prep(c, s);
		if (rc != RNB_OK) return rc;
		if (!c->overlap()) HIP_TRY(hipStreamSynchronize(s));
		c->grid_updated = true;
		c->prep_ms = std::chrono::duration<float, std::milli>(std::chrono::steady_clock::now() - t0).count() / n_prep_to_skip;
	}
	c->step_start = std::chrono::steady_clock::now();
	const uint32_t max_inference = next_max_inference(c);
	if (c->training_step == 0) { discard_premarch(c); c->n_rays_total = 0; }
	const uint32_t n_rays = c->rays_per_batch;
	if (c->pre.valid && (c->pre.n_rays != n_rays || c->pre.max_inference != max_inference)) discard_premarch(c);
	uint32_t n_rays_total;
	bool join_rest = false;
	if (c->pre.valid) {
		n_rays_total = c->pre.n_rays_total;
		c->pre.valid = false;
		c->cur_k1 = c->pre.k1;
		join_rest = c->pre.split;
		if (!joined && !c->pre.march_joined && !c->knobs.unsafe_skip_joins) HIP_TRY(hipStreamWaitEvent(s, c->ev_march, 0));
		c->pre.march_joined = false;
	} else {
		n_rays_total = c->n_rays_total;
		c->n_rays_total += n_rays * c->cfg.world_size;
		rc = generate_training_samples(c, s, n_rays, n_rays_total, max_inference);
		if (rc != RNB_OK) return rc;
		c->cur_k1 = c->gen_k1;
	}
	c->cur_n_rays = n_rays;
	c->cur_n_rays_total = n_rays_total;
	c->prof.mark(s, P_NONE);
	const bool two_round = c->cur_k1 != 0;
	c->cin_flow = c->rgb_split();
	if (c->cin_flow) { rc = ensure_rgb_buffers(c); if (rc != RNB_OK) return rc; }
	half_t* cin_out = c->cin_flow ? c->cin_eval.p : nullptr;
	if (two_round) rc = launch_forward(c, s, c->coords.p, c->fwd_counts.p, max_inference, c->mlp_out.p, false, c->idx1.p, cin_out);
	else rc = launch_forward(c, s, c->coords.p, c->counters.p + 3, max_inference, c->mlp_out.p, false, nullptr, cin_out);
	if (rc != RNB_OK) return rc;
	c->prof.mark(s, P_FORWARD);
	if (join_rest) HIP_TRY(hipStreamWaitEvent(s, c->ev_march_rest, 0));
	rc = compute_loss(c, s, n_rays, n_rays_total, two_round ? max_inference : 0, true, true);
	if (rc != RNB_OK) return rc;
	return pregenerate_grid_samples(c, s);
}

static int step_back(rnb_ctx* c, hipStream_t s) {
	int rc = forward_backward(c, s, false);
	if (rc != RNB_OK) return rc;
	c->rng.advance();
	return RNB_OK;
}

static int wait_loss_readback(rnb_ctx* c, hipStream_t s) {
	if (c->loss_polled) return RNB_OK;
	const volatile uint32_t* seq = &c->host_rb->seq;
	const auto t0 = std::chrono::steady_clock::now();
	for (uint64_t spins = 0; *seq != c->rb_seq; ++spins) {
		if ((spins & 0xffff) == 0xffff && std::chrono::steady_clock::now() - t0 > std::chrono::seconds(30)) {
			HIP_TRY(hipStreamSynchronize(s));
			if (*seq != c->rb_seq) return fail(RNB_ERR_DEVICE, "the loss readback of the step did not arrive");
		}
	}
	std::atomic_thread_fence(std::memory_order_acquire);
	c->loss_polled = true;
	return RNB_OK;
}

static int launch_reduce_losses(rnb_ctx* c, hipStream_t s) {
	if (c->loss_reduced) return RNB_OK;
	c->prof.mark(s, P_NONE);
	const bool tiled = c->cur_n_rays >= c->knobs.march_narrow_from;
	const uint32_t n_tiles = (c->cur_n_rays + SCAN_TILE - 1) / SCAN_TILE;
	if (tiled) hipLaunchKernelGGL(k_reduce_losses_tiles, dim3(n_tiles), dim3(1024), 0, s, c->cur_n_rays, c->counters.p, c->loss.p, c->ek_loss, c->mask_loss, c->loss_partial.p);
	const bool poll = c->poll_loss();
	if (poll) { if (++c->rb_seq == 0) ++c->rb_seq; c->loss_polled = false; }
	LAUNCH_EV(k_reduce_losses_rollover, dim3(1 + 255), dim3(1024), 0, s, poll ? nullptr : c->ev_loss, c->cur_n_rays, c->counters.p, c->loss.p, c->ek_loss, c->mask_loss, c->loss_sums.p, c->fwd_counts.p,
	          reinterpret_cast<double*>(c->host_rb_dev), tiled ? c->loss_partial.p : nullptr, n_tiles, c->cfg.target_batch_size, c->dloss_dout.p, c->coords_compacted.p, c->cin_flow ? c->src_slot.p : nullptr,
	          poll ? c->rb_seq : 0u);
	c->prof.mark(s, P_REDUCE);
	HIP_TRY(hipGetLastError());
	return RNB_OK;
}

static int launch_premarch(rnb_ctx* c) {
	if (!c->overlap() || c->pre.valid || prep_due(c->cur_step + 1)) return RNB_OK;
	const uint32_t n_rays = c->rays_per_batch, max_inference = next_max_inference(c), n_rays_total = c->n_rays_total;
	if (c->poll_loss()) { const int rc0 = wait_loss_readback(c, c->step_stream); if (rc0 != RNB_OK) return rc0; }
	else HIP_TRY(hipStreamWaitEvent(c->s_march, c->ev_loss, 0));
	if (c->knobs.march_late || c->rgb_split()) HIP_TRY(hipStreamWaitEvent(c->s_march, c->ev_fb, 0));
	int rc = generate_training_samples(c, c->s_march, n_rays, n_rays_total, max_inference, c->ev_march, c->tail_pending ? c->ev_tail : nullptr, c->ev_march_rest,
	                                   c->loss_reduced ? c->ev_fb : nullptr);
	if (rc != RNB_OK) return rc;
	c->tail_pending = false;
	c->pre.loss_cleared = true;
	c->n_rays_total += n_rays * c->cfg.world_size;
	c->pre.march_joined = false;
	c->pre.valid = true; c->pre.n_rays = n_rays; c->pre.n_rays_total = n_rays_total; c->pre.max_inference = max_inference; c->pre.k1 = c->gen_k1; c->pre.split = c->gen_split;
	return RNB_OK;
}

int rnb_train_step_begin(rnb_ctx* c, void* stream) try {
	if (!c) return fail(RNB_ERR_INVALID, "null ctx");
	if (c->n_views == 0) return fail(RNB_ERR_INVALID, "no dataset");
	hipStream_t s = as_stream(stream);
	c->cur_step = c->training_step;
	c->step_stream = s;
	int rc = step_front(c, s);
	if (rc != RNB_OK) { c->cin_flow = false; return rc; }
	rc = launch_reduce_losses(c, s);
	if (rc != RNB_OK) return rc;
	return step_back(c, s);
} RNB_GUARD

int rnb_train_step_apply(rnb_ctx* c, void* stream) try {
	if (!c) return fail(RNB_ERR_INVALID, "null ctx");
	hipStream_t s = as_stream(stream);
	int rc = optimizer_step(c, s);
	if (rc != RNB_OK) return rc;
	++c->training_step;
	return RNB_OK;
} RNB_GUARD

int rnb_train_step_local(rnb_ctx* c, void* stream, uint64_t counters_out[4], double loss_sums_out[3]) try {
	if (!c || !counters_out || !loss_sums_out) return fail(RNB_ERR_INVALID, "null argument");
	if (c->poll_loss()) { const int rc = wait_loss_readback(c, as_stream(stream)); if (rc != RNB_OK) return rc; }
	else if (c->overlap()) HIP_TRY(hipEventSynchronize(c->ev_loss));
	else HIP_TRY(hipStreamSynchronize(as_stream(stream)));
	{ const int rc = check_scan_errors(c); if (rc != RNB_OK) return rc; }
	const uint32_t* counters = c->host_rb->counters;
	if (c->prof.on) { c->prof.collect(); c->prof.units[P_FORWARD] += c->cur_k1 ? c->host_rb->fwd[0] + c->host_rb->fwd[1] : counters[3]; }
	for (int k = 0; k < 4; ++k) counters_out[k] = counters[k];
	for (int k = 0; k < 3; ++k) loss_sums_out[k] = c->host_rb->sums[k];
	c->local_measured_before = counters[0];
	return RNB_OK;
} RNB_GUARD

int rnb_train_step_finish(rnb_ctx* c, const uint64_t counters[4], const double sums[3], rnb_step_stats* stats) try {
	if (!c || !counters || !sums) return fail(RNB_ERR_INVALID, "null argument");
	const uint64_t Bg = (uint64_t)c->cfg.target_batch_size * c->cfg.world_size;
	const uint32_t n_rays = c->cur_n_rays;
	c->measured_batch_size = 0;
	c->measured_batch_size_before_compaction = 0;
	float loss_scalar = 0.f, ek_scalar = 0.f, mask_scalar = 0.f;
	uint32_t next_rays = c->rays_per_batch;
	int rc = RNB_OK;
	if (counters[0] == 0 || counters[1] == 0) {
		rc = RNB_ERR_NO_SAMPLES;
		g_err = "Nerf training generated 0 samples.";
	} else {
		c->measured_batch_size_before_compaction = c->local_measured_before;
		c->measured_batch_size = (uint32_t)(counters[1] / c->cfg.world_size);
		const float measured = (float)counters[1], target = (float)Bg;
		loss_scalar = (float)sums[0] * measured / target;
		ek_scalar = (float)sums[1] * measured / target;
		mask_scalar = (float)sums[2] * measured / target;
		next_rays = (uint32_t)((float)c->rays_per_batch * target / measured);
		next_rays = std::min(next_multiple_u32(next_rays, 128u), c->cfg.max_rays_per_batch);
	}
	if (stats) {
		stats->training_step = c->cur_step + 1;
		stats->rays_per_batch = n_rays;
		stats->next_rays_per_batch = next_rays;
		stats->measured_batch_size = (uint32_t)(counters[1] / c->cfg.world_size);
		stats->measured_batch_size_before_compaction = (uint32_t)(counters[0] / c->cfg.world_size);
		stats->n_rays_kept = (uint32_t)(counters[2] / c->cfg.world_size);
		stats->density_grid_updated = c->grid_updated ? 1 : 0;
		stats->loss = loss_scalar; stats->ek_loss = ek_scalar; stats->mask_loss = mask_scalar;
		stats->prep_ms = c->prep_ms;
		stats->step_ms = std::chrono::duration<float, std::milli>(std::chrono::steady_clock::now() - c->step_start).count();
	}
	c->rays_per_batch = next_rays;
	if (rc != RNB_OK) return rc;
	return launch_premarch(c);
} RNB_GUARD

int rnb_train_step_end(rnb_ctx* c, void* stream, rnb_step_stats* stats) try {
	if (c && c->overlap()) {
		uint64_t counters[4];
		double sums[3];
		int rc = rnb_train_step_local(c, stream, counters, sums);
		if (rc != RNB_OK) return rc;
		const int rc_finish = rnb_train_step_finish(c, counters, sums, stats);
		rc = rnb_train_step_apply(c, stream);
		return rc != RNB_OK ? rc : rc_finish;
	}
	int rc = rnb_train_step_apply(c, stream);
	if (rc != RNB_OK) return rc;
	uint64_t counters[4];
	double sums[3];
	rc = rnb_train_step_local(c, stream, counters, sums);
	if (rc != RNB_OK) return rc;
// ... 715 lines not shown
```

Measured before the change: 52.12 million.

## Reuse hash-grid encodings from forward pass in SDF fwd/bwd kernel

During the training forward pass, the pipelined encode now writes each sample's per-level features and dy/dx into a per-level global record buffer using nontemporal stores. The sdf-only fwd/bwd kernel then reads these records back through the compaction slot map instead of recomputing the multiresolution hash-grid encoding and its gradient. This trades repeated hash-grid gathers and interpolation for extra global memory traffic (7 dwords per level per sample written and read) and a large new buffer. It is enabled by default only for normals-only, non-half-accumulate runs with encode depth 4.

```diff
diff --git a/rnb-neus2_amd/csrc/common.cuh b/rnb-neus2_amd/csrc/common.cuh
--- a/rnb-neus2_amd/csrc/common.cuh
+++ b/rnb-neus2_amd/csrc/common.cuh
@@ -326,6 +326,26 @@
 	}
 }
 
+constexpr uint32_t ENC_REC_DWORDS = 7;
+__host__ __device__ __forceinline__ size_t enc_level_dwords(const uint32_t n_slots) { return ((size_t)n_slots + 1u) * ENC_REC_DWORDS; }
+__device__ __forceinline__ void enc_store(uint32_t* __restrict__ level_base, const uint32_t slot, const half_t f0, const half_t f1, const float (&d0)[3], const float (&d1)[3]) {
+	uint32_t* r = level_base + slot * ENC_REC_DWORDS;
+	__builtin_nontemporal_store(pack_h2(f0, f1), r + 0);
+#pragma unroll
+	for (int d = 0; d < 3; ++d) { __builtin_nontemporal_store(__float_as_uint(d0[d]), r + 1 + d); __builtin_nontemporal_store(__float_as_uint(d1[d]), r + 4 + d); }
+}
+__device__ __forceinline__ void enc_load(const uint32_t* __restrict__ level_base, const uint32_t slot, uint32_t (&v)[ENC_REC_DWORDS]) {
+	const uint32_t* r = level_base + slot * ENC_REC_DWORDS;
+#pragma unroll
+	for (uint32_t q = 0; q < ENC_REC_DWORDS; ++q) v[q] = __builtin_nontemporal_load(r + q);
+}
+__device__ __forceinline__ void enc_unpack(const uint32_t (&v)[ENC_REC_DWORDS], half_t& f0, half_t& f1, float (&d0)[3], float (&d1)[3]) {
+	const h2 f = unpack_h2(v[0]);
+	f0 = f[0]; f1 = f[1];
+#pragma unroll
+	for (int d = 0; d < 3; ++d) { d0[d] = __uint_as_float(v[1 + d]); d1[d] = __uint_as_float(v[4 + d]); }
+}
+
 struct Vec3 { float x, y, z; };
 __device__ __forceinline__ Vec3 v3(float x, float y, float z) { return {x, y, z}; }
 __device__ __forceinline__ Vec3 operator+(Vec3 a, Vec3 b) { return {a.x + b.x, a.y + b.y, a.z + b.z}; }
diff --git a/rnb-neus2_amd/csrc/kernels_net.cuh b/rnb-neus2_amd/csrc/kernels_net.cuh
--- a/rnb-neus2_amd/csrc/kernels_net.cuh
+++ b/rnb-neus2_amd/csrc/kernels_net.cuh
@@ -43,9 +43,11 @@
 	}
 }
 
-template <bool GRAD, int DEPTH, int ND = 0>
+template <bool GRAD, int DEPTH, int ND = 0, bool EXPORT = false>
 __device__ __forceinline__ void encode_all_pipelined(const LevelMeta* __restrict__ lm, const uint32_t n_levels, const uint32_t valid_level, const uint32_t* __restrict__ grid,
-                                                     const float x, const float y, const float z, half_t (&feat)[28], float (&dydx)[GRAD ? 28 : 1][3]) {
+                                                     const float x, const float y, const float z, half_t (&feat)[28], float (&dydx)[GRAD ? 28 : 1][3],
+                                                     uint32_t* __restrict__ enc_out = nullptr, const uint32_t enc_slots = 0, const uint32_t enc_slot = 0) {
+	static_assert(!EXPORT || GRAD, "the exported record holds dy/dx");
 	const uint32_t n_live = min(n_levels, valid_level + 1u);
 	uint32_t v[DEPTH][8];
 	const uint32_t last = n_live ? n_live - 1u : 0u;
@@ -64,6 +66,7 @@
 #pragma unroll
 			for (int d = 0; d < 3; ++d) { dydx[GRAD ? level * 2 + 0 : 0][d] = live ? d0[d] : 0.f; dydx[GRAD ? level * 2 + 1 : 0][d] = live ? d1[d] : 0.f; }
 		}
+		if (EXPORT) enc_store(enc_out + level * enc_level_dwords(enc_slots), enc_slot, feat[level * 2 + 0], feat[level * 2 + 1], dydx[GRAD ? level * 2 + 0 : 0], dydx[GRAD ? level * 2 + 1 : 0]);
 	}
 }
 
@@ -94,6 +97,8 @@
 	const uint32_t* idx;
 	const half_t* wimg;
 	half_t* cin_out;
+	uint32_t* enc_out;
+	uint32_t enc_slots;
 };
 
 __device__ __forceinline__ void copy_weight_image(half_t* __restrict__ dst, const half_t* __restrict__ src, const int n_halfs, const int tid, const int nthreads) {
@@ -199,7 +204,7 @@
 constexpr int FWD2_WAVE_HALFS = TILE * S32 + TILE * 8 + TILE;
 constexpr size_t LDS_FWD2 = (size_t)(W_FWD_END + WAVES_PER_WG * FWD2_WAVE_HALFS) * sizeof(half_t);
 
-template <bool EMU, int PIPE_DEPTH = 0, int ND = 0>
+template <bool EMU, int PIPE_DEPTH = 0, int ND = 0, bool EXPORT = false>
 __device__ __forceinline__ void forward_chained_body(const GridMeta& G, const NetW& net, const FwdArgs& a, char* smem_raw, LevelMeta* lm) {
 	poison_lds(smem_raw, LDS_FWD2, threadIdx.x, WG);
 	half_t* wts = reinterpret_cast<half_t*>(smem_raw);
@@ -230,7 +235,8 @@
 		}
 		half_t feat[28];
 		float dydx[28][3];
-		if (PIPE_DEPTH) encode_all_pipelined<true, PIPE_DEPTH ? PIPE_DEPTH : 1, ND>(lm, n_levels, valid_level, net.grid, c[0], c[1], c[2], feat, dydx);
+		static_assert(!EXPORT || PIPE_DEPTH, "the export belongs to the pipelined encode");
+		if (PIPE_DEPTH) encode_all_pipelined<true, PIPE_DEPTH ? PIPE_DEPTH : 1, ND, EXPORT>(lm, n_levels, valid_level, net.grid, c[0], c[1], c[2], feat, dydx, a.enc_out, a.enc_slots, (valid && s < a.enc_slots) ? s : a.enc_slots);
 		else encode_all_lm<true>(lm, n_levels, valid_level, net.grid, c[0], c[1], c[2], feat, dydx);
 		write_sdf_in_row(X, lane, c[0], c[1], c[2], feat);
 		wave_lds_sync();
@@ -359,6 +365,12 @@
 	__shared__ LevelMeta lm[RNB_MAX_LEVELS];
 	forward_chained_body<false, DEPTH, ND>(G, net, a, smem_raw, lm);
 }
+template <int DEPTH, int ND = 0>
+__global__ __launch_bounds__(WG, 2) void k_forward_chained_pipe_enc(const GridMeta G, const NetW net, const FwdArgs a) {
+	extern __shared__ __attribute__((aligned(16))) char smem_raw[];
+	__shared__ LevelMeta lm[RNB_MAX_LEVELS];
+	forward_chained_body<false, DEPTH, ND, true>(G, net, a, smem_raw, lm);
+}
 __global__ __launch_bounds__(WG, 2) void k_forward_chained_emul(const GridMeta G, const NetW net, const FwdArgs a) {
 	extern __shared__ __attribute__((aligned(16))) char smem_raw[];
 	__shared__ LevelMeta lm[RNB_MAX_LEVELS];
@@ -390,6 +402,9 @@
 	const half_t* wimg;
 	float *dw_w0, *dw_w0b, *dw_w1, *dw_w1b;
 	const half_t* dcin;
+	const uint32_t* enc;
+	const uint32_t* src_slot;
+	uint32_t enc_slots;
 	TrainScratch t;
 };
 
@@ -709,7 +724,7 @@
 		}
 }
 
-template <bool FULL, bool EMU = false, bool SLICED = false>
+template <bool FULL, bool EMU = false, bool SLICED = false, bool REUSE = false>
 __device__ __forceinline__ void fwd_bwd_sdf_body(const GridMeta& G, const NetW& net, const TrainArgs& a, char* smem_raw, LevelMeta* lm) {
 	poison_lds(smem_raw, FULL ? LDS_FBS_FULL : LDS_FBS, threadIdx.x, WG);
 	half_t* wts = reinterpret_cast<half_t*>(smem_raw);
@@ -775,11 +790,7 @@
 		reinterpret_cast<f4*>(T.srec)[(size_t)s * 2 + 1] = f4{dn[1], dn[2], 0.f, 0.f};
 		uint32_t* Xrow = reinterpret_cast<uint32_t*>(X + lane * S32);
 		uint32_t* Drow = reinterpret_cast<uint32_t*>(D + lane * S32);
-#pragma unroll 1
-		for (uint32_t level = 0; level < 14; ++level) {
-			half_t f0 = (half_t)0.f, f1 = (half_t)0.f;
-			float d0[3] = {0.f, 0.f, 0.f}, d1[3] = {0.f, 0.f, 0.f};
-			if (level < n_live) encode_level_lm<true>(lm, net.grid, level, c[0], c[1], c[2], f0, f1, d0, d1);
+		auto put_level = [&](const uint32_t level, const half_t f0, const half_t f1, const float (&d0)[3], const float (&d1)[3]) {
 			float r0 = 0.f, r1 = 0.f;
 #pragma unroll
 			for (int d = 0; d < 3; ++d) { r0 += d0[d] * dn[d]; r1 += d1[d] * dn[d]; }
@@ -791,6 +802,29 @@
 			} else {
 				Xrow[level] = pack_h2(f0, f1);
 				Drow[level] = pack_h2(e0, e1);
+			}
+		};
+		if (REUSE) {
+			const uint32_t slot = min(a.src_slot[s], a.enc_slots);
+			constexpr uint32_t DEPTH = 4;
+			uint32_t v[DEPTH][ENC_REC_DWORDS];
+#pragma unroll
+			for (uint32_t l = 0; l < DEPTH; ++l) enc_load(a.enc + l * enc_level_dwords(a.enc_slots), slot, v[l]);
+#pragma unroll
+			for (uint32_t level = 0; level < 14; ++level) {
+				half_t f0, f1;
+				float d0[3], d1[3];
+				enc_unpack(v[level % DEPTH], f0, f1, d0, d1);
+				if (level + DEPTH < 14) enc_load(a.enc + (level + DEPTH) * enc_level_dwords(a.enc_slots), slot, v[level % DEPTH]);
+				put_level(level, f0, f1, d0, d1);
+			}
+		} else {
+#pragma unroll 1
+			for (uint32_t level = 0; level < 14; ++level) {
+				half_t f0 = (half_t)0.f, f1 = (half_t)0.f;
+				float d0[3] = {0.f, 0.f, 0.f}, d1[3] = {0.f, 0.f, 0.f};
+				if (level < n_live) encode_level_lm<true>(lm, net.grid, level, c[0], c[1], c[2], f0, f1, d0, d1);
+				put_level(level, f0, f1, d0, d1);
 			}
 		}
 		{
@@ -1070,6 +1104,11 @@
 	extern __shared__ __attribute__((aligned(16))) char smem_raw[];
 	__shared__ LevelMeta lm[RNB_MAX_LEVELS];
 	fwd_bwd_sdf_body<false>(G, net, a, smem_raw, lm);
+}
+__global__ __launch_bounds__(WG, 2) void k_fwd_bwd_sdf_enc(const GridMeta G, const NetW net, const TrainArgs a) {
+	extern __shared__ __attribute__((aligned(16))) char smem_raw[];
+	__shared__ LevelMeta lm[RNB_MAX_LEVELS];
+	fwd_bwd_sdf_body<false, false, false, true>(G, net, a, smem_raw, lm);
 }
 __global__ __launch_bounds__(WG, 2) void k_fwd_bwd_sdf_full(const GridMeta G, const NetW net, const TrainArgs a) {
 	extern __shared__ __attribute__((aligned(16))) char smem_raw[];
diff --git a/rnb-neus2_amd/csrc/rnb_neus2_hip.hip b/rnb-neus2_amd/csrc/rnb_neus2_hip.hip
--- a/rnb-neus2_amd/csrc/rnb_neus2_hip.hip
+++ b/rnb-neus2_amd/csrc/rnb_neus2_hip.hip
@@ -175,6 +175,11 @@
 	DevBuf<uint32_t> src_slot;
 	bool cin_flow = false;
 	bool rgb_split() const { return !cfg.apply_no_albedo && !knobs.fwd_bwd_generic; }
+	DevBuf<uint32_t> enc_eval;
+	uint32_t enc_slots = 0;
+	bool enc_flow = false, enc_alloc_failed = false;
+	bool enc_mode() const { return knobs.encode_reuse && !enc_alloc_failed && cfg.apply_no_albedo && !knobs.fwd_bwd_generic && !half_acc() && knobs.encode_depth == 4; }
+	uint32_t* flow_slots() const { return (cin_flow || enc_flow) ? src_slot.p : nullptr; }
 	bool wimg_valid = false;
 	DevBuf<float> ray_const;
 	DevBuf<uint32_t> unfinished;
@@ -226,6 +231,7 @@
 		bool point_xcd = true;
 		bool dw_sliced = true;
 		bool encode_pair = false;
+		bool encode_reuse = true;
 		bool grid_presort = true;
 	} knobs;
 	DevBuf<RayLoss> ray_loss;
@@ -583,21 +589,37 @@
 static int ensure_rgb_buffers(rnb_ctx* c) {
 	if (c->cin_eval.p) return RNB_OK;
 	const size_t B = c->cfg.target_batch_size;
-	if (c->cin_eval.alloc(B * 16 * 32) != hipSuccess || c->dcin.alloc(B * 32) != hipSuccess || c->rgb_out_scratch.alloc(B * 16) != hipSuccess || c->src_slot.alloc(B) != hipSuccess)
+	if (c->cin_eval.alloc(B * 16 * 32) != hipSuccess || c->dcin.alloc(B * 32) != hipSuccess || c->rgb_out_scratch.alloc(B * 16) != hipSuccess || (!c->src_slot.p && c->src_slot.alloc(B) != hipSuccess))
 		return fail(RNB_ERR_NOMEM, "hipMalloc failed for the colour-MLP training buffers");
 	return RNB_OK;
 }
 
-int launch_forward(rnb_ctx* c, hipStream_t s, const float* coords, const uint32_t* n_ptr, uint32_t n_max, half_t* out, bool inference, const uint32_t* idx = nullptr, half_t* cin_out = nullptr) {
+static bool ensure_enc_buffers(rnb_ctx* c) {
+	if (c->enc_eval.p) return true;
+	const uint32_t n_slots = c->cfg.target_batch_size * 16;
+	if ((!c->src_slot.p && c->src_slot.alloc(c->cfg.target_batch_size) != hipSuccess) || c->enc_eval.alloc(14 * enc_level_dwords(n_slots)) != hipSuccess) {
+		(void)hipGetLastError();
+		c->enc_eval.p = nullptr; c->enc_eval.n = 0;
+		c->enc_alloc_failed = true;
+		return false;
+	}
+	c->enc_slots = n_slots;
+	return true;
+}
+
+int launch_forward(rnb_ctx* c, hipStream_t s, const float* coords, const uint32_t* n_ptr, uint32_t n_max, half_t* out, bool inference, const uint32_t* idx = nullptr, half_t* cin_out = nullptr, bool enc_export = false) {
 	if (n_max == 0) return RNB_OK;
 	join_tail_host(c);
 	FwdArgs a;
 	a.coords = coords; a.n_ptr = n_ptr; a.n_max = n_max; a.out = out; a.sdf_bias = c->cfg.sdf_bias; a.idx = idx; a.cin_out = cin_out;
+	a.enc_out = enc_export ? c->enc_eval.p : nullptr; a.enc_slots = enc_export ? c->enc_slots : 0u;
 	a.wimg = (!inference && c->wimg_valid) ? c->wimg_fwd.p : nullptr;
 	const uint32_t n_tiles = (n_max + TILE - 1) / TILE;
 	const uint32_t grid = std::min<uint32_t>((n_tiles + WAVES_PER_WG - 1) / WAVES_PER_WG, (uint32_t)c->n_cus * 2);
 	if (c->half_acc() && c->knobs.encode_depth) hipLaunchKernelGGL(k_forward_chained_emul_pipe<4>, dim3(grid), dim3(WG), LDS_FWD2, s, c->meta(), c->net(inference), a);
 	else if (c->half_acc()) hipLaunchKernelGGL(k_forward_chained_emul, dim3(grid), dim3(WG), LDS_FWD2, s, c->meta(), c->net(inference), a);
+	else if (enc_export && c->knobs.encode_pair && c->n_dense_lead >= 5) hipLaunchKernelGGL((k_forward_chained_pipe_enc<4, 5>), dim3(grid), dim3(WG), LDS_FWD2, s, c->meta(), c->net(inference), a);
+	else if (enc_export) hipLaunchKernelGGL(k_forward_chained_pipe_enc<4>, dim3(grid), dim3(WG), LDS_FWD2, s, c->meta(), c->net(inference), a);
 	else if (c->knobs.encode_depth == 2) hipLaunchKernelGGL(k_forward_chained_pipe<2>, dim3(grid), dim3(WG), LDS_FWD2, s, c->meta(), c->net(inference), a);
 	else if (c->knobs.encode_depth == 4 && c->knobs.encode_pair && c->n_dense_lead >= 5) hipLaunchKernelGGL((k_forward_chained_pipe<4, 5>), dim3(grid), dim3(WG), LDS_FWD2, s, c->meta(), c->net(inference), a);
 	else if (c->knobs.encode_depth == 4) hipLaunchKernelGGL(k_forward_chained_pipe<4>, dim3(grid), dim3(WG), LDS_FWD2, s, c->meta(), c->net(inference), a);
@@ -755,7 +777,7 @@
 	a.views = c->views.p; a.counters = c->counters.p; a.ray_indices = c->ray_indices.p; a.rays = c->rays.p; a.numsteps = c->numsteps.p;
 	a.coords = c->coords.p; a.mlp_out = c->mlp_out.p; a.ray_loss = c->ray_loss.p; a.ncomp = c->ncomp.p; a.cbase = c->cbase.p;
 	a.coords_compacted = c->coords_compacted.p; a.dloss = c->dloss_dout.p; a.loss = c->loss.p; a.ek_loss = c->ek_loss; a.mask_loss = c->mask_loss;
-	a.src_slot = c->cin_flow ? c->src_slot.p : nullptr;
+	a.src_slot = c->flow_slots();
 	a.chain_rec = c->knobs.loss_chain_records ? c->chain_rec.p : nullptr;
 	a.ray_grad = c->ray_grad.p; a.ray_of = c->ray_of.p; a.slot_of = c->slot_of.p;
 	a.scan_words = nullptr; a.scan_ticket = 0; a.scan_error = nullptr; a.scan_total = nullptr;
@@ -776,7 +798,7 @@
 		a.cap = c->cur_k1;
 		launch_heads();
 		c->prof.mark(s, P_LOSS_PASS1);
-		int rc = launch_forward(c, s, c->coords.p, c->fwd_counts.p + 2, two_round_n_max, c->mlp_out.p, false, c->idx2.p, c->cin_flow ? c->cin_eval.p : nullptr);
+		int rc = launch_forward(c, s, c->coords.p, c->fwd_counts.p + 2, two_round_n_max, c->mlp_out.p, false, c->idx2.p, c->cin_flow ? c->cin_eval.p : nullptr, c->enc_flow);
 		if (rc != RNB_OK) return rc;
 		c->prof.mark(s, P_FORWARD);
 		a.phase = 1;
@@ -838,6 +860,9 @@
 	a.coords = c->coords_compacted.p; a.dout = c->dloss_dout.p; a.B = B; a.B_global = B * c->cfg.world_size; a.sdf_bias = c->cfg.sdf_bias; a.t = c->ts; a.skip_rgb = c->cfg.apply_no_albedo ? 1u : 0u;
 	const bool split = c->rgb_split();
 	a.wimg = !c->wimg_valid ? nullptr : (!c->knobs.fwd_bwd_generic) ? c->wimg_fbs.p : c->wimg_train.p;
+	const bool enc_flow = c->enc_flow && c->enc_mode();
+	c->enc_flow = false;
+	a.enc = enc_flow ? c->enc_eval.p : nullptr; a.src_slot = enc_flow ? c->src_slot.p : nullptr; a.enc_slots = enc_flow ? c->enc_slots : 0u;
 	const bool sdf_only = (a.skip_rgb && !c->knobs.fwd_bwd_generic) || split;
 	const uint32_t fb_grid = sdf_only ? std::min<uint32_t>((B / TILE + WAVES_PER_WG - 1) / WAVES_PER_WG, (uint32_t)c->n_cus * c->knobs.fbs_wg_per_cu) : c->fwd_grid;
 	const bool sliced = half && sdf_only && c->knobs.dw_sliced;
@@ -881,6 +906,7 @@
 		else LAUNCH_EV(k_fwd_bwd_sdf_full, dim3(fb_grid), dim3(WG), LDS_FBS_FULL, s, ev_fb, c->meta(), c->net(false), a);
 	} else if (sdf_only && half && sliced) LAUNCH_EV(k_fwd_bwd_sdf_hs, dim3(fb_grid), dim3(WG), LDS_FBS, s, ev_fb, c->meta(), c->net(false), a);
 	else if (sdf_only && half) LAUNCH_EV(k_fwd_bwd_sdf_h, dim3(fb_grid), dim3(WG), LDS_FBS, s, ev_fb, c->meta(), c->net(false), a);
+	else if (sdf_only && enc_flow) LAUNCH_EV(k_fwd_bwd_sdf_enc, dim3(fb_grid), dim3(WG), LDS_FBS, s, ev_fb, c->meta(), c->net(false), a);
 	else if (sdf_only) LAUNCH_EV(k_fwd_bwd_sdf, dim3(fb_grid), dim3(WG), LDS_FBS, s, ev_fb, c->meta(), c->net(false), a);
 	else LAUNCH_EV(k_fwd_bwd, dim3(fb_grid), dim3(WG), LDS_TRAIN, s, ev_fb, c->meta(), c->net(false), a);
 	c->prof.mark(s, P_FWD_BWD);
@@ -1324,7 +1350,7 @@
 	c->gs_sorted_pos.free(); c->gs_sorted_idx.free(); c->gs_stage_pos.free(); c->gs_stage_idx.free(); c->gs_hist.free(); c->gs_range.free(); c->gs_eval_pos.free(); c->gs_eval_idx.free();
 	c->ray_indices.free(); c->numsteps.free(); c->counters.free(); c->rays.free(); c->coords.free(); c->coords_compacted.free();
 	c->loss.free(); c->mlp_out.free(); c->chain_rec.free(); c->ray_grad.free(); c->ray_of.free(); c->slot_of.free(); c->wg_partial.free(); c->dloss_dout.free();
-	c->wimg_fwd.free(); c->wimg_fbs.free(); c->wimg_train.free(); c->wimg_rgb.free(); c->cin_eval.free(); c->dcin.free(); c->rgb_out_scratch.free(); c->src_slot.free(); c->ray_const.free(); c->ray_base1.free(); c->scan_words.free(); c->idx1.free(); c->idx2.free(); c->fwd_counts.free(); c->unfinished.free();
+	c->wimg_fwd.free(); c->wimg_fbs.free(); c->wimg_train.free(); c->wimg_rgb.free(); c->cin_eval.free(); c->enc_eval.free(); c->dcin.free(); c->rgb_out_scratch.free(); c->src_slot.free(); c->ray_const.free(); c->ray_base1.free(); c->scan_words.free(); c->idx1.free(); c->idx2.free(); c->fwd_counts.free(); c->unfinished.free();
 	c->ray_setup.free(); c->ray_t.free(); c->ray_dunnorm.free(); c->ray_steps.free(); c->ray_base.free(); c->ray_slot.free(); c->ncomp.free(); c->cbase.free(); c->scan_tiles.free(); c->loss_partial.free(); c->ray_loss.free();
 	c->render_rays[0].free(); c->render_rays[1].free(); c->render_keep.free(); c->render_scan.free(); c->render_counts.free(); c->render_res.free(); c->render_coords.free(); c->render_out.free();
 	c->mc_table.free(); c->fm.free(); c->g12.free(); c->srec.free(); c->var_partial.free(); c->dw_partial.free();
@@ -1519,6 +1545,7 @@
 		if (const char* e = getenv("RNB_POINT_XCD")) k.point_xcd = atoi(e) != 0;
 		if (const char* e = getenv("RNB_DW_SLICED")) k.dw_sliced = atoi(e) != 0;
 		if (const char* e = getenv("RNB_ENCODE_PAIR")) k.encode_pair = atoi(e) != 0;
+		if (const char* e = getenv("RNB_ENCODE_REUSE")) k.encode_reuse = atoi(e) != 0;
 		if (const char* e = getenv("RNB_ENCODE_DEPTH")) { const int d = atoi(e); k.encode_depth = (d == 0 || d == 2 || d == 4 || d == 7) ? d : 4; }
 		if (const char* e = getenv("RNB_DEBUG_SCATTER_LEVELS")) { int lo = -1, hi = -1; if (sscanf(e, "%d,%d", &lo, &hi) == 2 && lo >= 0 && hi > lo) { k.dbg_scatter_lo = lo; k.dbg_scatter_hi = hi; } }
 		if (const char* e = getenv("RNB_SCATTER_C_EARLY")) k.scatter_c_early = atoi(e) != 0;
@@ -1937,7 +1964,7 @@
 	if (c->n_views == 0) return fail(RNB_ERR_INVALID, "no dataset");
 	if (n_rays == 0 || n_rays > c->cfg.max_rays_per_batch) return fail(RNB_ERR_INVALID, "n_rays out of range");
 	if (max_samples > c->cfg.target_batch_size * 16) return fail(RNB_ERR_INVALID, "max_samples exceeds 16*target_batch_size");
-	c->cin_flow = false;
+	c->cin_flow = false; c->enc_flow = false;
 	return generate_training_samples(c, as_stream(stream), n_rays, n_rays_total, max_samples);
 } RNB_GUARD
 
@@ -1945,13 +1972,13 @@
 	if (!c) return fail(RNB_ERR_INVALID, "null ctx");
 	if (c->n_views == 0) return fail(RNB_ERR_INVALID, "no dataset");
 	if (n_rays == 0 || n_rays > c->cfg.max_rays_per_batch) return fail(RNB_ERR_INVALID, "n_rays out of range");
-	c->cin_flow = false;
+	c->cin_flow = false; c->enc_flow = false;
 	return compute_loss(c, as_stream(stream), n_rays, n_rays_total);
 } RNB_GUARD
 
 int rnb_forward_backward(rnb_ctx* c, void* stream) try {
 	if (!c) return fail(RNB_ERR_INVALID, "null ctx");
-	c->cin_flow = false;
+	c->cin_flow = false; c->enc_flow = false;
 	return forward_backward(c, as_stream(stream));
 } RNB_GUARD
 
@@ -2022,8 +2049,9 @@
 	c->cin_flow = c->rgb_split();
 	if (c->cin_flow) { rc = ensure_rgb_buffers(c); if (rc != RNB_OK) return rc; }
 	half_t* cin_out = c->cin_flow ? c->cin_eval.p : nullptr;
-	if (two_round) rc = launch_forward(c, s, c->coords.p, c->fwd_counts.p, max_inference, c->mlp_out.p, false, c->idx1.p, cin_out);
-	else rc = launch_forward(c, s, c->coords.p, c->counters.p + 3, max_inference, c->mlp_out.p, false, nullptr, cin_out);
+	c->enc_flow = c->enc_mode() && max_inference <= c->cfg.target_batch_size * 16 && ensure_enc_buffers(c);
+	if (two_round) rc = launch_forward(c, s, c->coords.p, c->fwd_counts.p, max_inference, c->mlp_out.p, false, c->idx1.p, cin_out, c->enc_flow);
+	else rc = launch_forward(c, s, c->coords.p, c->counters.p + 3, max_inference, c->mlp_out.p, false, nullptr, cin_out, c->enc_flow);
 	if (rc != RNB_OK) return rc;
 	c->prof.mark(s, P_FORWARD);
 	if (join_rest) HIP_TRY(hipStreamWaitEvent(s, c->ev_march_rest, 0));
@@ -2063,7 +2091,7 @@
 	const bool poll = c->poll_loss();
 	if (poll) { if (++c->rb_seq == 0) ++c->rb_seq; c->loss_polled = false; }
 	LAUNCH_EV(k_reduce_losses_rollover, dim3(1 + 255), dim3(1024), 0, s, poll ? nullptr : c->ev_loss, c->cur_n_rays, c->counters.p, c->loss.p, c->ek_loss, c->mask_loss, c->loss_sums.p, c->fwd_counts.p,
-	          reinterpret_cast<double*>(c->host_rb_dev), tiled ? c->loss_partial.p : nullptr, n_tiles, c->cfg.target_batch_size, c->dloss_dout.p, c->coords_compacted.p, c->cin_flow ? c->src_slot.p : nullptr,
+	          reinterpret_cast<double*>(c->host_rb_dev), tiled ? c->loss_partial.p : nullptr, n_tiles, c->cfg.target_batch_size, c->dloss_dout.p, c->coords_compacted.p, c->flow_slots(),
 	          poll ? c->rb_seq : 0u);
 	c->prof.mark(s, P_REDUCE);
 	HIP_TRY(hipGetLastError());
@@ -2094,7 +2122,7 @@
 	c->cur_step = c->training_step;
 	c->step_stream = s;
 	int rc = step_front(c, s);
-	if (rc != RNB_OK) { c->cin_flow = false; return rc; }
+	if (rc != RNB_OK) { c->cin_flow = false; c->enc_flow = false; return rc; }
 	rc = launch_reduce_losses(c, s);
 	if (rc != RNB_OK) return rc;
 	return step_back(c, s);
```

Result: no change. 52.43 million (median of 6 runs) (+0.6%).
